# algbio/GraphChainer

Measured on AMD Instinct MI355X. Metric: reads_per_sec, higher is better.
Workload: dtype u64

## Files before the change

graphchainer_amd/csrc/batch/gc_batch_long.inc:

```
	void prepareWholeReadPass()
	{
		uint64_t nLongSeeds = 0;
		maxReadLen = 1;
		for (uint64_t r = 0; r < n; r++) maxReadLen = std::max<uint64_t>(maxReadLen, R->offsets[r + 1] - R->offsets[r]);
		firstAlnCap = (uint32_t)std::max<uint64_t>(32, maxReadLen / 512);
		if (sw.testLongMaxAlignments) firstAlnCap = *sw.testLongMaxAlignments;
		alnSlots = n * (uint64_t)firstAlnCap;
		if (P->long_pass && alnSlots >= 0xffffffffull) throw std::runtime_error("batch too large for the whole-read pass");
		if (P->long_pass) {
			if (deviceGlue) nLongSeeds = nSeedsTotal;
			else for (uint64_t r = 0; r < n; r++) { glue[r].longSeedBegin = nLongSeeds; nLongSeeds += glue[r].longSeeds.size(); }
			if (nLongSeeds >= 0xffffffffull) throw std::runtime_error("batch too large for the whole-read pass");
			LongSeed* hSeeds = st->hLongSeeds.reserve<LongSeed>(deviceGlue ? 0 : nLongSeeds);
			hJobs = st->hLongJobs.reserve<LongJob>(n);
			cellPoolPinned = sw.testLongCellsPerBase || P->capacity.long_cells_per_base > 0;
			uint64_t cellsPerBase = (uint64_t)std::max<int64_t>(2, capacityOr(sw.testLongCellsPerBase, P->capacity.long_cells_per_base, (int64_t)st->longCellsPerBase));
			if (sw.testLongForceFallback && !cellPoolPinned) cellsPerBase *= 3;
			cellBudget = cellBudgetFor(cellsPerBase);
			pool.run(n, [&](size_t r, size_t) {
				const ReadGlue& gl = glue[r];
				uint64_t at = gl.longSeedBegin;
				if (deviceGlue) at += gl.nSeedsR;
				else for (const gc::SeedRec& s : gl.longSeeds) {
					hSeeds[at++] = LongSeed { s.node, s.seqPos, s.goodness, s.clusterSize, s.offset, 0 };
				}
				LongJob& j = hJobs[r];
				j.maskOff = R->maskOff[r];
				j.maskWords = R->maskWords[r];
				j.alnCap = firstAlnCap;
				j.readOff = R->offsets[r];
				j.readLen = (uint32_t)(R->offsets[r + 1] - R->offsets[r]);
				j.seedBegin = (uint32_t)gl.longSeedBegin;
				j.seedEnd = (uint32_t)at;
				j.alnBegin = (uint32_t)(r * firstAlnCap);
				j.extendSeeds = j.seedEnd - j.seedBegin;
				if (P->seed_extend_density != -1) j.extendSeeds = (uint32_t)std::min<double>(4294967295.0, P->seed_extend_density * (double)j.readLen + 1);
				j.pad = 0;
			});
			lcfg.bandwidth = P->bandwidth;
			lcfg.rampBandwidth = P->ramp_bandwidth;
			lcfg.maxCells = P->max_cells_per_slice < 0 || P->max_cells_per_slice >= 0xffffffffll ? ~0u : (uint32_t)P->max_cells_per_slice;
			lcfg.maxSlices = (uint32_t)(maxReadLen / 64 + 3);
			lcfg.maxItems = (uint32_t)std::max<uint64_t>(8192, (maxReadLen / 64 + 3) * 24);
			lcfg.maxPending = 96;
			lcfg.forceGlobal = P->force_global != 0;
			lcfg.maxTrace = P->force_global || clip.on() ? (uint32_t)(2 * maxReadLen + 2 + 512) : (uint32_t)(maxReadLen + maxReadLen / 2 + 512);
			clip.apply(lcfg);
			lcfg.maxCols = (uint32_t)std::max<int64_t>(0, capacityOr(sw.testLongMaxCols, P->capacity.long_column_store, (int64_t)(3 * maxReadLen + 4096)));
			lcfg.maxItems = (uint32_t)std::max<int64_t>(64, capacityOr(sw.testLongMaxItems, P->capacity.long_max_items, lcfg.maxItems));
			if (sw.testLongRegCap) lcfg.regCap = *sw.testLongRegCap;
			waveWords = longWaveWordsPerLane(lcfg);
			if (!deviceGlue) dLongSeeds = st->longSeeds.reserve<LongSeed>(nLongSeeds);
			dLongJobs = st->longJobs.reserve<LongJob>(n);
			dLongAlns = st->longAlns.reserve<LongAln>(alnSlots);
			LongReadResult* dLongResults = st->longResults.reserve<LongReadResult>(n);
			dLongCells = st->longCells.reserve<LongCell>(cellBudget, true);
			if (!st->roundStream) {
				createStream(&st->roundStream);
				for (auto& e : st->roundEvents) HIP_CHECK(hipEventCreate(&e));
			}
			cursorWords = 32 + 8 * 16;
			dLongCursor = st->longCursor.reserve<unsigned long long>(cursorWords);
			hLongAlns = st->hLongAlns.reserve<LongAln>(alnSlots);
			hLongResults = st->hLongResults.reserve<LongReadResult>(n);
			hLongSmall = st->hLongSmall.reserve<unsigned long long>(cursorWords);
			ls = st->longStream;
			HIP_CHECK(hipMemsetAsync(dLongCursor, 0, cursorWords * sizeof(unsigned long long), ls));
			if (nLongSeeds && !deviceGlue) HIP_CHECK(hipMemcpyAsync(dLongSeeds, hSeeds, nLongSeeds * sizeof(LongSeed), hipMemcpyHostToDevice, ls));
			if (n) HIP_CHECK(hipMemcpyAsync(dLongJobs, hJobs, n * sizeof(LongJob), hipMemcpyHostToDevice, ls));
			syncStream(ls);
			dLongState = st->longState.reserve<LongState>(n);
			workCapacity = 8 * n + 64;
			dLongWork = st->longWork.reserve<LongWork>(workCapacity);
			dLongWorkResults = st->longWorkResults.reserve<LongWorkResult>(workCapacity);
			dCandSeed = st->longCandSeed.reserve<uint32_t>(2 * workCapacity);
			dWorkLen = st->longWorkLen.reserve<uint32_t>(workCapacity);
			dRetryList = st->longRetryList.reserve<uint32_t>(workCapacity);
			dOrder = st->longOrder.reserve<uint32_t>(workCapacity);
			roundTraceBudget = 0;
			for (uint64_t r = 0; r < n; r++) { uint64_t len = R->offsets[r + 1] - R->offsets[r]; roundTraceBudget += 4 * ((P->force_global || clip.on() ? 2 * len + 2 : len + len / 2) + 1024); }
			dRoundTrace = st->longRoundTrace.reserve<unsigned long long>(roundTraceBudget);
			uint64_t scratchBudget = P->capacity.long_scratch_bytes > 0 ? (uint64_t)P->capacity.long_scratch_bytes : (48ull << 30) / (uint64_t)longTokenCount(sw.longTokens, n, st->batchesDone, st->fragShare);
			if (sw.testLongScratchGb) scratchBudget = *sw.testLongScratchGb << 30;
			scratchLanes = std::min<uint64_t>(std::min<uint64_t>(workCapacity + 64, 2 * n + 128), std::max<uint64_t>(2048, std::min<uint64_t>(65536 + 64, scratchBudget / (waveWords * 8))));
			longScratchWords = scratchLanes * waveWords;
			shareLongScratch = sw.shareLongScratch();
			if (!shareLongScratch) dLongScratchOwn = st->longScratch.reserve<unsigned long long>(longScratchWords);
		}
	}

	uint64_t cellBudgetFor(uint64_t perBase) const { uint64_t b = 0; for (uint64_t r = 0; r < n; r++) b += perBase * (R->offsets[r + 1] - R->offsets[r]) + 1024; return b; }

	bool growLongCells()
	{
		bool overflowed = false;
		for (uint64_t r = 0; r < n && !overflowed; r++) overflowed = hLongResults[r].status == 4;
		if (!overflowed || cellPoolPinned) return false;
		HIP_CHECK(hipMemcpyAsync(hLongSmall, dLongCursor, sizeof(unsigned long long), hipMemcpyDeviceToHost, ls));
		syncStream(ls);
		const uint64_t asked = hLongSmall[0], bases = std::max<uint64_t>(1, R->totalBases);
		const uint64_t next = std::max<uint64_t>(st->longCellsPerBase + 2, (asked + asked / 2 + bases - 1) / bases);
		if (sw.debugTimes) fprintf(stderr, "[gc mem] the whole-read pass runs again: %.2f G merged-trace cells asked for, %.2f G reserved (%llu per read base), now %llu per base\n", asked / 1e9, cellBudget / 1e9, (unsigned long long)st->longCellsPerBase, (unsigned long long)next);
		if (next > 256 || cellBudgetFor(next) * sizeof(LongCell) > (64ull << 30)) return false;
		st->longCellsPerBase = next;
		cellBudget = cellBudgetFor(next);
		dLongCells = st->longCells.reserve<LongCell>(cellBudget, true);
		HIP_CHECK(hipMemsetAsync(dLongCursor, 0, cursorWords * sizeof(unsigned long long), ls));
		syncStream(ls);
		return true;
	}

	static constexpr uint32_t LONG_ALN_SLOTS_MAX = 1u << 16;
	bool growAlnSlots(const std::vector<uint32_t>& reads, bool keep)
	{
		uint64_t total = alnSlots;
		std::vector<std::pair<uint32_t, uint32_t>> grown;
		for (uint32_t r : reads) {
			const uint32_t cap = hJobs[r].alnCap, limit = std::min<uint32_t>(LONG_ALN_SLOTS_MAX, std::max<uint32_t>(1, hJobs[r].seedEnd - hJobs[r].seedBegin));
			if (cap >= limit) continue;
			const uint32_t next = (uint32_t)std::min<uint64_t>(limit, 4ull * cap);
			if (total + next >= 0xffffffffull) continue;
			grown.push_back({ r, next });
			total += next;
		}
		if (grown.empty()) return false;
		if (sw.debugTimes) fprintf(stderr, "[gc mem] %zu reads found more whole-read alignments than they had slots for and run again: %llu -> %llu slots in the batch\n", grown.size(), (unsigned long long)alnSlots, (unsigned long long)total);
		if (keep && total * sizeof(LongAln) > st->longAlns.bytes) {
			DeviceBuffer larger;
			LongAln* dLarger = larger.reserve<LongAln>(total);
			HIP_CHECK(hipMemcpyAsync(dLarger, dLongAlns, alnSlots * sizeof(LongAln), hipMemcpyDeviceToDevice, ls));
			syncStream(ls);
			std::swap(st->longAlns.ptr, larger.ptr); std::swap(st->longAlns.bytes, larger.bytes);
		}
		dLongAlns = st->longAlns.reserve<LongAln>(total);
		uint64_t at = alnSlots;
		for (const auto& g : grown) { hJobs[g.first].alnBegin = (uint32_t)at; hJobs[g.first].alnCap = g.second; at += g.second; }
		alnSlots = total;
		HIP_CHECK(hipMemcpyAsync(dLongJobs, hJobs, n * sizeof(LongJob), hipMemcpyHostToDevice, ls));
		syncStream(ls);
		return true;
	}

	bool growLongAlns()
	{
		std::vector<uint32_t> full;
		for (uint64_t r = 0; r < n; r++) if (hLongResults[r].status == 3) full.push_back((uint32_t)r);
		if (full.empty() || !growAlnSlots(full, false)) return false;
		HIP_CHECK(hipMemsetAsync(dLongCursor, 0, cursorWords * sizeof(unsigned long long), ls));
		syncStream(ls);
		return true;
	}

	void runLongRounds()
	{
		if (n == 0) return;
		unsigned long long* dLongScratch = nullptr;
		hipStream_t q = st->roundStream;
		hipEvent_t* ring = st->roundEvents;
		auto collect = [&](int slot) { float ms = 0; HIP_CHECK(hipEventElapsedTime(&ms, ring[2 * slot], ring[2 * slot + 1])); longExtendUs += (double)ms * 1000.0; };
		int timedRounds = 0;
		unsigned long long* cursor = dLongCursor + 32;
		volatile unsigned long long* hCursor = hLongSmall + 32;
		double dbgWaitUs = 0;
		const double dbgT0 = nowUs();
		launchLongInit(q, dLongJobs, (uint32_t)n, dLongState);
		uint32_t lastWork = 0xffffffffu;

		for (int round = 0; round < 4096; round++) {
			launchZeroWords(q, cursor, 4);
			uint32_t maxCand = 1;
			if (round > 0 && lastWork > 0) maxCand = (uint32_t)std::min<uint64_t>(8, std::max<uint64_t>(1, (2 * n) / lastWork));
			if (round > 0 && lastWork < 8192) maxCand = 8;
			if (round > 0 && lastWork > 0) maxCand = (uint32_t)std::min<uint64_t>(maxCand, std::max<uint64_t>(1, (8 * n) / lastWork));
			if (sw.testLongSpeculate) maxCand = *sw.testLongSpeculate;
			launchLongSelect(q, G->dev, dLongJobs, (uint32_t)n, dLongSeeds, R->totalBases, (uint32_t)P->min_cluster_size, (uint32_t)P->extra_heuristic, maxCand, dLongState, dLongAlns, dLongCells, dLongWork, dWorkLen, dCandSeed, cursor, workCapacity);
			launchLongOrder(q, dWorkLen, cursor, dOrder, (uint32_t)maxReadLen, sw.testLongOrder);
			launchPublish(q, cursor, (unsigned long long*)hCursor, 2);
			const double tWait0 = nowUs();
			syncStream(q);
			dbgWaitUs += nowUs() - tWait0;
			uint32_t nWorkItems = (uint32_t)hCursor[0];
			if (nWorkItems == 0) break;
			if (!dLongScratch) {
				longTokenTake();
				dLongScratch = shareLongScratch ? longScratchOfToken : dLongScratchOwn;
			}
			uint32_t team = longExtendTeamSize(nWorkItems, sw.testLongTeam.value_or(0));
			uint32_t blocks = std::min<uint32_t>((nWorkItems + team - 1) / team, (uint32_t)std::max<uint64_t>(1, (scratchLanes - 64) / team));
			if (sw.testLongMaxBlocks) blocks = std::min<uint32_t>(blocks, *sw.testLongMaxBlocks);
			if (timedRounds >= LONG_EVENT_RING) collect(timedRounds % LONG_EVENT_RING);
			hipEvent_t ev0 = ring[2 * (timedRounds % LONG_EVENT_RING)], ev1 = ring[2 * (timedRounds % LONG_EVENT_RING) + 1];
			HIP_CHECK(hipEventRecord(ev0, q));
			launchLongExtend(q, G->dev, G->devTables, R->devMasks, lcfg, dLongWork, dOrder, nWorkItems, dLongScratch, team, blocks,
				dRoundTrace, cursor + 1, roundTraceBudget, dLongWorkResults, dLongCursor + 8, cursor + 2, 0, nullptr, team == 1 ? dRetryList : nullptr, cursor + 3);
			if (team == 1) {
				if ((uint64_t)blocks * team < nWorkItems) launchZeroWords(q, cursor + 2, 1);
				uint32_t retryBlocks = std::min<uint32_t>(128, (uint32_t)std::max<uint64_t>(1, (scratchLanes - 64) / 2));
				launchLongExtend(q, G->dev, G->devTables, R->devMasks, lcfg, dLongWork, dRetryList, nWorkItems, dLongScratch, 2, retryBlocks,
					dRoundTrace, cursor + 1, roundTraceBudget, dLongWorkResults, dLongCursor + 8, cursor + 2, EXT_LDS_CAP, cursor + 3);
			}
			HIP_CHECK(hipEventRecord(ev1, q));
			launchLongMerge(q, G->dev, dLongJobs, (uint32_t)n, dLongSeeds, dCandSeed, dLongWorkResults, dRoundTrace, dLongState, dLongAlns, dLongCells, dLongCursor, cellBudget, (uint32_t)P->extra_heuristic);
			lastWork = nWorkItems;
			timedRounds++;
			longRounds++;
		}
		longTokenDrop();
		launchLongFinish(q, (uint32_t)n, dLongState, hLongResults);
		const double dbgT1 = nowUs();
		syncStream(q);
		if (sw.debugTimes) fprintf(stderr, "[gc times] whole-read rounds: %.1f ms in all, %.1f ms waiting for the rounds' work counts, %.1f ms in the last wait, %d rounds\n", (nowUs() - dbgT0) / 1e3, dbgWaitUs / 1e3, (nowUs() - dbgT1) / 1e3, timedRounds);
		for (int k = std::max(0, timedRounds - LONG_EVENT_RING); k < timedRounds; k++) collect(k % LONG_EVENT_RING);
	}

	uint64_t longFallback()
	{
		syncStream(ls);
		std::vector<uint32_t> redo;
		const bool forceAll = sw.testLongForceFallback;
		for (uint64_t r = 0; r < n; r++) if (hLongResults[r].status == 5 || hLongResults[r].status == 2 || forceAll) redo.push_back((uint32_t)r);
		if (!redo.empty()) {
			ExtendConfig fcfg = lcfg;
			fcfg.maxItems = 4 * lcfg.maxItems; fcfg.maxTrace = 2 * lcfg.maxTrace; fcfg.maxPending = 4 * lcfg.maxPending;
			uint64_t lslab = longSlabBytes(fcfg);
			std::vector<uint32_t> now = redo;
			for (int cellGrowths = 0; !now.empty(); ) {
				std::vector<LongJob> subJobs(now.size());
				for (size_t i = 0; i < now.size(); i++) subJobs[i] = hJobs[now[i]];
				uint64_t lanes = (now.size() + 63) / 64 * 64;
				LongJob* dSubJobs = st->longJobsFallback.reserve<LongJob>(now.size());
				LongReadResult* dSubResults = st->longResultsFallback.reserve<LongReadResult>(now.size());
				uint8_t* dSlab = st->longScratchFallback.reserve<uint8_t>(lanes * lslab);
				HIP_CHECK(hipMemcpyAsync(dSubJobs, subJobs.data(), now.size() * sizeof(LongJob), hipMemcpyHostToDevice, ls));
				launchLongPass(ls, G->dev, G->devTables, G->devIupac, fcfg, dSubJobs, (uint32_t)now.size(), dLongSeeds, R->devBases, R->totalBases, (uint32_t)P->min_cluster_size, (uint32_t)P->extra_heuristic,
					dSlab, lslab, dLongCells, dLongCursor, cellBudget, dLongAlns, dSubResults, dLongCursor + 8);
				std::vector<LongReadResult> subResults(now.size());
				HIP_CHECK(hipMemcpyAsync(subResults.data(), dSubResults, now.size() * sizeof(LongReadResult), hipMemcpyDeviceToHost, ls));
				HIP_CHECK(hipMemcpyAsync(hLongSmall, dLongCursor, sizeof(unsigned long long), hipMemcpyDeviceToHost, ls));
				syncStream(ls);
				std::vector<uint32_t> refused, full;
				for (size_t i = 0; i < now.size(); i++) {
					hLongResults[now[i]] = subResults[i];
					if (subResults[i].status == 4) refused.push_back(now[i]);
					if (subResults[i].status == 3) full.push_back(now[i]);
				}
				if (!full.empty() && !growAlnSlots(full, true)) full.clear();
				if (refused.empty() || cellPoolPinned || cellGrowths >= 3) { now.swap(full); continue; }
				const uint64_t used = std::min<uint64_t>(hLongSmall[0], cellBudget), next = std::min<uint64_t>(256, st->longCellsPerBase * 2);
				if (next == st->longCellsPerBase || cellBudgetFor(next) * sizeof(LongCell) > (64ull << 30)) { now.swap(full); continue; }
				cellGrowths++;
				if (sw.debugTimes) fprintf(stderr, "[gc mem] the plain-layout reruns of %zu reads found the merged-trace pool full: %llu -> %llu cells per read base, %.2f G cells kept\n", refused.size(), (unsigned long long)st->longCellsPerBase, (unsigned long long)next, used / 1e9);
				DeviceBuffer larger;
				LongCell* dLarger = larger.reserve<LongCell>(cellBudgetFor(next), true);
				if (used) HIP_CHECK(hipMemcpyAsync(dLarger, dLongCells, used * sizeof(LongCell), hipMemcpyDeviceToDevice, ls));
				const unsigned long long cursor = used;
				HIP_CHECK(hipMemcpyAsync(dLongCursor, &cursor, sizeof(cursor), hipMemcpyHostToDevice, ls));
				syncStream(ls);
				std::swap(st->longCells.ptr, larger.ptr); std::swap(st->longCells.bytes, larger.bytes);
				st->longCellsPerBase = next;
				cellBudget = cellBudgetFor(next);
				dLongCells = (LongCell*)st->longCells.ptr;
				now.swap(refused);
				now.insert(now.end(), full.begin(), full.end());
			}
		}
		hLongAlns = st->hLongAlns.reserve<LongAln>(alnSlots);
		if (n) HIP_CHECK(hipMemcpyAsync(hLongAlns, dLongAlns, alnSlots * sizeof(LongAln), hipMemcpyDeviceToHost, ls));
		HIP_CHECK(hipMemcpyAsync(hLongSmall, dLongCursor, 32 * sizeof(unsigned long long), hipMemcpyDeviceToHost, ls));
		syncStream(ls);
		return (uint64_t)redo.size();
	}

	void decideLongReads(const std::vector<uint32_t>& subset, int slot, hipStream_t q, const std::function<uint32_t(uint32_t)>& nAlnOf, bool usePool = true)
	{
		auto selectOne = [&](size_t i, size_t) {
			const uint32_t r = subset[i];
			ReadGlue& gl = glue[r];
			gl.longAlns.clear();
			gl.longSelected.clear();
			const uint32_t nAln = nAlnOf(r);
			for (uint32_t a = 0; a < nAln; a++) {
				gl.longAlns.push_back(hLongAlns[(uint64_t)hJobs[r].alnBegin + a]);
				std::sort(gl.longAlns.begin(), gl.longAlns.end(), [](const LongAln& l, const LongAln& rr) { return l.start < rr.start; });
			}
			std::vector<gc::SelectItem> items;
			for (const LongAln& al : gl.longAlns) items.push_back(gc::SelectItem { al.start, al.end, al.score });
			const size_t readLen = R->offsets[r + 1] - R->offsets[r];
			gl.longSelected = gc::selectAlignments(items, P->colinear_chaining ? (int)gc::SelectGreedyLength : (int)P->selection_method, hg.SizeInBP(), readLen, P->e_cutoff, evalueModel);
		};
		if (usePool) pool.run(subset.size(), selectOne); else for (size_t i = 0; i < subset.size(); i++) selectOne(i, 0);
		auto& D = st->edLong[slot];
		D.nPairs = 0;
		D.pairRead.clear();
		if (!P->edit_distances || !P->colinear_chaining || subset.empty()) return;
		const size_t m = subset.size();
		PathSeqJob* hJobsPS = D.hJobs.reserve<PathSeqJob>(m);
		EdPair* hPairs = D.hPairs.reserve<EdPair>(m);
		int64_t* hOut = D.hOut.reserve<int64_t>(m);
		uint64_t nLetters = 0;
		uint32_t nPairs = 0;
		for (size_t i = 0; i < m; i++) {
			const uint32_t r = subset[i];
			const ReadGlue& gl = glue[r];
			if (gl.longSelected.empty()) { hJobsPS[i] = PathSeqJob { 0, nLetters, 0, 0, 0, 0 }; continue; }
			const LongAln& al = gl.longAlns[gl.longSelected[0]];
			uint32_t len = (uint32_t)(R->offsets[r + 1] - R->offsets[r]);
			uint32_t cap = 2 * al.traceLen + 256;
			hJobsPS[i] = PathSeqJob { al.traceOff, nLetters, al.traceLen, cap, 0, 0 };
			hPairs[nPairs++] = EdPair { nLetters, 0, (uint32_t)i, r, al.score + al.start + (len - std::min(len, al.end)) + 8 };
			D.pairRead.push_back(r);
			nLetters += cap;
		}
		PathSeqJob* dJobsPS = D.jobs.reserve<PathSeqJob>(m);
		char* dLetters = D.letters.reserve<char>(nLetters);
		uint32_t* dLettersLen = D.lettersLen.reserve<uint32_t>(m);
		EdPair* dPairs = D.pairs.reserve<EdPair>(m);
		int64_t* dOut = D.out.reserve<int64_t>(m);
		HIP_CHECK(hipMemcpyAsync(dJobsPS, hJobsPS, m * sizeof(PathSeqJob), hipMemcpyHostToDevice, q));
		launchLongPathSeq(q, G->dev, dJobsPS, (uint32_t)m, dLongCells, dLetters, dLettersLen);
		auto readLenOf = [R = R](uint32_t r) { return (uint32_t)(R->offsets[r + 1] - R->offsets[r]); };
		launchEditDistances(D.run, q, hPairs, hOut, nPairs, dPairs, dOut, R->devEdReads, R->devBases, R->devEqMasks, dLetters, dLettersLen, readLenOf, sw.debugTimes, true);
		D.nPairs = nPairs;
		decisionPtr[slot] = DecisionPointers { hPairs, hOut, dPairs, dOut, dLetters, dLettersLen };
	}

	void finishLongDecision(int slot)
	{
		auto& D = st->edLong[slot];
		if (!D.nPairs) return;
		const DecisionPointers& p = decisionPtr[slot];
		finishEditDistances(D.run, st->longStream, p.hPairs, p.hOut, D.nPairs, p.dPairs, p.dOut, R->devEdReads, R->devBases, R->devEqMasks, p.dLetters, p.dLettersLen, sw.debugTimes);
		for (uint32_t i = 0; i < D.nPairs; i++) {
			ReadGlue& gl = glue[D.pairRead[i]];
			gl.longEditDistance = p.hOut[i];
			if (p.hOut[i] < -1) { gl.longEditDistance = -1; gl.capacityExceededLong = true; }
		}
		D.nPairs = 0;
	}

	void afterLongPass()
	{
		uint64_t rerun = longFallback();
		res->counters_long[7] = rerun;
		for (int i = 0; i < 6; i++) res->counters_long[i] = hLongSmall[8 + i];
#ifdef GC_STAMPS
		{
			static const char* names[11] = { "slice prologue", "pop+prev lookup", "tile columns", "item store", "edge pushes", "slice epilogue", "bt slice change", "bt item loads", "bt recompute", "bt corner", "bt walk" };
			double total = 0;
			for (int i = 0; i < 11; i++) total += (double)hLongSmall[16 + i];
			for (int i = 0; i < 11; i++) fprintf(stderr, "[gc stamps] %-16s %6.2f%%  %.3e lane-cycles\n", names[i], 100.0 * hLongSmall[16 + i] / (total > 0 ? total : 1), (double)hLongSmall[16 + i]);
		}
#endif
		if (sw.testFailLong) {
			const long idx = *sw.testFailLong;
			if (idx >= 0 && (uint64_t)idx < n) hLongResults[idx].status = 1;
// ... 78 lines not shown
```

graphchainer_amd/csrc/gc_batch.hip:

```cpp
#include "gc_runtime.hpp"

extern "C" {

struct ClipOptions {
	double cutoff = 0;
	double errorCost = 0;
	int32_t xDrop = 0;
	bool on() const { return cutoff != 0; }
	void apply(ExtendConfig& cfg) const { if (on()) { cfg.setClipErrorCost(errorCost); cfg.xDrop = xDrop; } }
};

struct BatchRun {
	const gc::Switches sw;
	const gc_graph* const G; const gc_seeder* const S; const gc_seeds* const H; gc_stream* const st; const gc_reads* const R; const gc_params* const P; const ClipOptions clip; gc_result* const res;
	const double tCall, cpuCall;
	double cpuJoined;
	const uint64_t n;
	const gc::AlignmentGraph& hg;
	WorkerPool& pool;
	std::vector<ReadGlue>& glue;
	const hipStream_t stream;
	int evIdx = 0;
	double tTotal = 0;
	bool deviceGlue = true;
	double tGlue = 0;
	uint64_t nSlots = 0, nFrags = 0, nSeedsTotal = 0, traceBudget = 0;
	uint32_t maxSlotsPerRead = 1, maxWindowSeeds = 0;
	Fragment* frags = nullptr; ReadChainJob* jobs = nullptr;
	FragSeed* readSeeds = nullptr; uint32_t* fragFirstSeed = nullptr;
	Fragment* dFrags = nullptr; uint32_t* dFragFirstSeed = nullptr; FragSeed* dReadSeeds = nullptr; ReadChainJob* dJobs = nullptr;
	LongSeed* dLongSeeds = nullptr;
	hipEvent_t glueCopied = nullptr;
	double tOrdered = 0;
	unsigned long long* hSmall = nullptr;
	unsigned long long* dCursors = nullptr;
	unsigned long long* dCounters = nullptr;
	uint32_t firstAlnCap = 0;
	uint64_t alnSlots = 0;
	LongAln* hLongAlns = nullptr;
	unsigned long long* hLongSmall = nullptr;
	LongReadResult* hLongResults = nullptr;
	LongCell* dLongCells = nullptr;
	uint64_t cellBudget = 0;
	unsigned long long* longScratchOfToken = nullptr;
	std::function<void()> longTokenTake, longTokenDrop;
	uint64_t longScratchWords = 0;
	bool shareLongScratch = false;
	double longExtendUs = 0; uint32_t longRounds = 0;
	const gc::EValueModel evalueModel { clip.on() ? clip.cutoff : 0.7 };
	struct DecisionPointers { EdPair* hPairs = nullptr; int64_t* hOut = nullptr; EdPair* dPairs = nullptr; int64_t* dOut = nullptr; char* dLetters = nullptr; uint32_t* dLettersLen = nullptr; } decisionPtr[2];
	LongJob* hJobs = nullptr;
	bool cellPoolPinned = 0;
	uint64_t waveWords = 0;
	LongJob* dLongJobs = nullptr;
	LongAln* dLongAlns = nullptr;
	uint32_t cursorWords = 0;
	uint64_t workCapacity = 0;
	uint64_t roundTraceBudget = 0;
	unsigned long long* dLongCursor = nullptr;
	LongState* dLongState = nullptr;
	LongWork* dLongWork = nullptr;
	LongWorkResult* dLongWorkResults = nullptr;
	uint32_t* dCandSeed = nullptr;
	uint32_t* dWorkLen = nullptr;
	uint32_t* dRetryList = nullptr;
	uint32_t* dOrder = nullptr;
	unsigned long long* dRoundTrace = nullptr;
	uint64_t scratchLanes = 0;
	hipStream_t ls = nullptr;
	ExtendConfig lcfg;
	unsigned long long* dLongScratchOwn = nullptr;
	uint64_t maxReadLen = 1;
	std::thread longThread;
	double passThreadCpuMs = 0;
	std::exception_ptr longError;
	double tLongWall0 = 0;
	double longWallBeginUs = 0.0;
	double longWallEndUs = 0.0;
	double tDev = 0;
	uint32_t nWork = 0;
	ExtResult* dResults = nullptr;
	PoolCell* dTrace = nullptr;
	AnchorRec* dAnchors = nullptr;
	uint32_t* dFragStatus = nullptr;
	uint32_t* dFragExtended = nullptr;
	uint64_t traceWorst = 0, pathWorst = 0;
	bool poolsSized = false;
	uint32_t nExtendPairs = 0, nAnchorPairs = 0;
	uint32_t poolReruns = 0;
	uint32_t* dReadTies = nullptr;
	uint64_t pathCapacity = 0;
	uint32_t* dPathPool = nullptr;
	uint32_t* dChainOut = nullptr;
	uint32_t* dChainLen = nullptr;
	unsigned long long* dChainScore = nullptr;
	uint32_t* dChainStatus = nullptr;
	bool deviceStitch = false;
	StitchInfo* stitchInfo = nullptr;
	uint32_t* hStitchNodes = nullptr;
	uint32_t* dStitchNodes = nullptr;
	uint64_t stitchDenseCap = 0;
	unsigned long long* hStitchCursor = nullptr;
	AnchorRec* anchors = nullptr;
	uint32_t* fragStatus = nullptr;
	uint32_t* fragExtended = nullptr;
	uint32_t* readTies = nullptr;
	uint32_t* chainOut = nullptr;
	uint32_t* chainLen = nullptr;
	unsigned long long* chainScore = nullptr;
	uint32_t* chainStatus = nullptr;
	uint32_t* pathPool = nullptr;
	bool deviceAnchors = false;
	uint4* hAnchorPerRead = nullptr;
	unsigned long long* hAnchorOff = nullptr;
	uint8_t* hAnchorDense = nullptr;
	uint64_t denseAnchors = 0, densePathWords = 0;
	std::vector<ExtResult> extResults;
	std::vector<PoolCell> tracePool;
	bool anchorTraces = false;
	bool stitchNodesPending = false;
	const PathSeqJob* chainLetterJobs = nullptr;
	const char* dChainLetters = nullptr;
	const uint32_t* dChainAltNodes = nullptr;
	const FastChainJob* fastChainJobs = nullptr;
	std::vector<uint32_t> zeroWords; std::vector<unsigned long long> zeroLongs; std::vector<uint4> zeroPerRead;
	double tJoined = 0;
	const LongCell* longCells = nullptr;

	BatchRun(const gc::Switches& sw, const gc_graph* G, const gc_seeder* S, const gc_seeds* H, gc_stream* st, const gc_reads* R, const gc_params* P, const ClipOptions& clip, gc_result* res, double tCall, double cpuCall)
		: sw(sw), G(G), S(S), H(H), st(st), R(R), P(P), clip(clip), res(res), tCall(tCall), cpuCall(cpuCall), cpuJoined(cpuCall), n(R->offsets.size() - 1), hg(G->host), pool(WorkerPool::batch()), glue(st->glue),
		  stream(st->stream) {}
	~BatchRun() { if (longThread.joinable()) longThread.join(); }
	BatchRun(const BatchRun&) = delete;
	BatchRun& operator=(const BatchRun&) = delete;

	void mark() { HIP_CHECK(hipEventRecord(st->ev[evIdx++], stream)); }
	double elapsedUs(int a, int b) { float ms = 0; HIP_CHECK(hipEventElapsedTime(&ms, st->ev[a], st->ev[b])); return (double)ms * 1000.0; }

	void run()
	{
		res->n_reads = n;
		tTotal = nowUs();
		const bool cpuStages = sw.debugTimes;
		double cpuAt = cpuStages ? threadCpuMs() : 0, cpuStage[10] = {}, poolStage[10] = {};
		uint64_t poolAt = pool.cpuUs.load();
		const double processAt = processCpuMs();
		auto stageDone = [&](int k) {
			if (!cpuStages) return;
			const double now = threadCpuMs(); const uint64_t poolNow = pool.cpuUs.load();
			cpuStage[k] += now - cpuAt; poolStage[k] += (poolNow - poolAt) / 1e3;
			cpuAt = now; poolAt = poolNow;
		};
		seeds(); stageDone(0);
		prepareWholeReadPass(); stageDone(1);
		startWholeReadPass(); stageDone(2);
		if (!P->colinear_chaining) { withoutChaining(); joinWholeReadPass(); stageDone(6); encodeOutput(); stageDone(8); assemble(); stageDone(9); st->batchesDone++; return; }
		fragmentPipeline(); stageDone(3);
		resultsBack(); stageDone(4);
		while (fragmentPoolsOverflowed()) { fragmentPipeline(); resultsBack(); stageDone(3); }
		res->counters[6] = poolReruns;
		compactAnchors(); stageDone(4);
		stitchAndChainDistances(); stageDone(5);
		joinWholeReadPass(); stageDone(6);
		chainedAlignments(); stageDone(7);
		encodeOutput(); stageDone(8);
		assemble(); stageDone(9);
		st->fragShare = (double)res->counters[4] / (double)std::max<uint64_t>(1, R->totalBases);
		st->batchesDone++;
		if (cpuStages)
			fprintf(stderr, "[gc cpu] main thread, ms of its own CPU: seeds %.1f, whole-read set-up %.1f + start %.1f, fragment pipeline %.1f, results back %.1f, stitching + chain distances %.1f, join %.1f, chained alignments %.1f, output %.1f, assembly %.1f; pass thread %.1f\n",
				cpuStage[0], cpuStage[1], cpuStage[2], cpuStage[3], cpuStage[4], cpuStage[5], cpuStage[6], cpuStage[7], cpuStage[8], cpuStage[9], passThreadCpuMs);
		if (cpuStages)
			fprintf(stderr, "[gc cpu] worker pool jobs, ms of CPU over all threads, by stage: %.1f %.1f %.1f %.1f %.1f %.1f %.1f %.1f %.1f %.1f; the process in all %.1f\n",
				poolStage[0], poolStage[1], poolStage[2], poolStage[3], poolStage[4], poolStage[5], poolStage[6], poolStage[7], poolStage[8], poolStage[9], processCpuMs() - processAt);
	}

#include "batch/gc_batch_seeds.inc"
#include "batch/gc_batch_long.inc"
#include "batch/gc_batch_fragments.inc"
#include "batch/gc_batch_results.inc"
#include "batch/gc_batch_output.inc"
};

static int resolveExt(const gc_params* P, const gc_params_ext* X, ClipOptions& clip)
{
	clip = ClipOptions();
	if (!X) return GC_OK;
	if (X->struct_size < sizeof(gc_params_ext)) return fail(GC_ERR_INVALID, "gc_params_ext::struct_size is smaller than the struct (was it initialised with gc_params_ext_default?)");
	if (X->struct_size > sizeof(gc_params_ext)) return fail(GC_ERR_INVALID, "gc_params_ext::struct_size is larger than this library knows: the caller's header is newer");
	if (X->x_drop < 0) return fail(GC_ERR_INVALID, "gc_params_ext::x_drop must be 0 (off) or >= 1 (src/AlignerMain.cpp:316-322)");
	const double c = X->precise_clipping;
	if (std::isnan(c) || (c != 0 && !(c >= 0.001 && c <= 0.999))) return fail(GC_ERR_INVALID, "gc_params_ext::precise_clipping must be 0 (off) or in [0.001, 0.999] (src/AlignerMain.cpp:300-315)");
	if (X->x_drop > 0 && P->force_global != 0) return fail(GC_ERR_INVALID, "gc_params_ext::x_drop cannot be combined with force_global (getSlices asserts, src/GraphAlignerBitvectorBanded.h:504)");
	clip.cutoff = c;
	clip.xDrop = X->x_drop;
	if (clip.xDrop > 0 && clip.cutoff == 0) clip.cutoff = 0.66;
	if (clip.on()) clip.errorCost = clip.cutoff / (1.0 - clip.cutoff) + 1.0;
	return GC_OK;
}

static int alignBatch(const gc::Switches& sw, const gc_graph* G, const gc_seeder* S, const gc_seeds* H, gc_stream* st, const gc_reads* R, const gc_params* P, const ClipOptions& clip, gc_result** out)
{
	if (P->split_len < 16 || P->split_len > 64 || P->split_gap < 1) return fail(GC_ERR_INVALID, "split_len must be in [16,64] (one 64-row slice per fragment extension) and split_gap >= 1");
	if (P->ramp_bandwidth < 0 || (P->ramp_bandwidth != 0 && P->ramp_bandwidth <= P->bandwidth)) return fail(GC_ERR_INVALID, "ramp_bandwidth must be 0 (off) or larger than bandwidth (src/AlignerMain.cpp:380-383)");
	if (P->max_cells_per_slice < -1) return fail(GC_ERR_INVALID, "max_cells_per_slice must be -1 (unlimited) or >= 0");
	if (P->force_global != 0 && P->force_global != 1) return fail(GC_ERR_INVALID, "force_global must be 0 or 1");
	if (P->colinear_chaining != 0 && P->colinear_chaining != 1) return fail(GC_ERR_INVALID, "colinear_chaining must be 0 or 1");
	if (P->colinear_chaining == 0 && !P->long_pass) return fail(GC_ERR_INVALID, "colinear_chaining == 0 needs long_pass: without chaining the whole-read pass is all there is");
	if (P->extra_heuristic != 0 && P->extra_heuristic != 1) return fail(GC_ERR_INVALID, "extra_heuristic must be 0 or 1");
	if (P->selection_method < 0 || P->selection_method > GC_SELECT_ALL) return fail(GC_ERR_INVALID, "selection_method must be one of GC_SELECT_* (0..7)");
	if (P->fast_mode != 0 && P->fast_mode != 1) return fail(GC_ERR_INVALID, "fast_mode must be 0 or 1");
	if (std::isnan(P->seed_extend_density) || (P->seed_extend_density <= 0 && P->seed_extend_density != -1)) return fail(GC_ERR_INVALID, "seed_extend_density must be -1 (all seeds) or > 0 (src/AlignerMain.cpp:405)");
	if (P->seed_extend_density != -1 && P->colinear_chaining == 1) return fail(GC_ERR_INVALID, "seed_extend_density must be -1 with colinear_chaining == 1: chaining tries all seeds (src/AlignerMain.cpp:204,449-453)");
	{
		const gc_capacities& c = P->capacity;
		if (c.reserved[0] || c.reserved[1] || c.reserved[2]) return fail(GC_ERR_INVALID, "gc_params::capacity.reserved must be 0 (was the struct initialised with gc_params_default?)");
		const int64_t v[] = { c.ext_max_items, c.ext_max_pending, c.ext_max_trace, c.long_max_items, c.long_cells_per_base, c.long_scratch_bytes, c.stitch_set_max, c.stitch_bfs_cap };
		for (int64_t x : v) if (x < 0 || x > (1ll << 40)) return fail(GC_ERR_INVALID, "gc_params::capacity: a size is negative or absurd (0 = automatic)");
		if (c.ext_max_items > (1ll << 24) || c.ext_max_pending > (1ll << 24) || c.ext_max_trace > (1ll << 24)) return fail(GC_ERR_INVALID, "gc_params::capacity.ext_*: at most 2^24 (the retry launch reserves 16x)");
// ... 56 lines not shown
```

graphchainer_amd/csrc/gc_runtime.hpp:

```cpp
#pragma once
#include "../../include/graphchainer_amd.h"
#include "hip/gc_kernels.hpp"
#include "host/gc_graph.hpp"
#include "host/gc_hashorder.hpp"
#include "host/gc_glue.hpp"
#include "host/gc_output.hpp"
#include "host/gc_index_cache.hpp"
#include "host/gc_correctness.hpp"
#include "host/gc_selection.hpp"
#include "host/gc_switches.hpp"
#include "host/gc_mxm_build.hpp"
#include "hip/gc_mxm_core.hpp"
#include <hip/hip_runtime.h>
#include <algorithm>
#include <atomic>
#include <condition_variable>
#include <functional>
#include <mutex>
#include <chrono>
#include <cmath>
#include <cstdlib>
#include <cstring>
#include <stdexcept>
#include <string>
// ... 375 lines not shown
		for (const Block& b : mine) { if (pinned) (void)hipHostFree(b.ptr); else (void)hipFree(b.ptr); }
	}
};
inline BlockCache& g_readDeviceBlocks = *new BlockCache(false);
inline BlockCache& g_readPinnedBlocks = *new BlockCache(true);
inline BlockCache& g_deflateDeviceBlocks = *new BlockCache(false, (size_t)4 << 30);
inline BlockCache& g_deflatePinnedBlocks = *new BlockCache(true, (size_t)4 << 30);

inline hipStream_t threadStream(int device)
{
	static thread_local struct ThreadStream { hipStream_t q = nullptr; int device = -1; ~ThreadStream() { if (q) (void)hipStreamDestroy(q); } } ts;
	if (!ts.q || ts.device != device) { if (ts.q) (void)hipStreamDestroy(ts.q); ts.q = nullptr; HIP_CHECK(hipStreamCreateWithFlags(&ts.q, hipStreamNonBlocking)); ts.device = device; }
	return ts.q;
}

struct gc_reads {
	void* deviceBlock = nullptr; size_t deviceBlockBytes = 0; int device = 0;
	std::vector<uint64_t> offsets;
	uint64_t totalBases = 0;
	std::vector<uint8_t> invalid;
	char* devBases = nullptr;
	uint64_t* devOffsets = nullptr;
	uint64_t* devMasks = nullptr;
	std::vector<uint64_t> maskOff;
	std::vector<uint32_t> maskWords;
	const uint64_t* devMaskOff = nullptr; const uint32_t* devMaskWords = nullptr;
	uint64_t* devEqMasks = nullptr;
	EdRead* devEdReads = nullptr;
	uint32_t* devChunkRead = nullptr;
	uint64_t* devPacked = nullptr;
	uint64_t* devInvalid = nullptr;
	uint8_t* devReadInvalid = nullptr;
	~gc_reads() { g_readDeviceBlocks.put(deviceBlock, deviceBlockBytes, device); }
};

struct gc_seeds {
	int device = 0;
	uint64_t nHits = 0;
	std::vector<uint64_t> readOffsets;
	uint32_t* devReadHitOff = nullptr;
	SeedHitArrays dev {};
	void* block = nullptr;
	SeedHit* devHits = nullptr;
	double kernelMs = 0;
	~gc_seeds() { if (block) (void)hipFree(block); }
};

struct gc_mxm_index {
	const gc_graph* graph = nullptr;
	int device = 0;
	std::vector<uint32_t> nodeStart;
	std::vector<int32_t> nodeId;
	MxmIndexView dev {};
	uint64_t deviceBytes = 0;
	double buildSeconds = 0;
	std::vector<void*> allocations;
	~gc_mxm_index() { for (void* p : allocations) (void)hipFree(p); }
};

struct StitchedPath { std::vector<uint32_t> nodes; uint32_t firstOffset = 0, lastOffset = 0; uint64_t cells = 0; };

struct ReadGlue {
	std::vector<gc::SeedRec> seeds;
	std::vector<gc::SeedRec> longSeeds;
	std::vector<gc::FragmentWindow> windows;
	std::vector<LongAln> longAlns;
	uint64_t longBegin = 0, longTraceBegin = 0, longSeedBegin = 0;
	bool failed = false;
	bool longFailed = false;
	bool capacityExceeded = false;
	bool capacityExceededLong = false;
	uint64_t slotBegin = 0, fragBegin = 0;
	uint32_t nSeedsR = 0, nWindows = 0;
	uint64_t nAnchors = 0, nPath = 0, nTrace = 0, anchorBegin = 0, pathBegin = 0, traceBegin = 0, seedBegin = 0, chainBegin = 0;
	StitchedPath stitched;
	bool stitchedOnDevice = false;
	uint64_t stitchedBegin = 0;
	std::vector<uint32_t> longSelected;
	uint64_t longSelectedBegin = 0;
	int64_t longEditDistance = -1, chainEditDistance = -1;
	std::vector<int32_t> chainTraceNode; std::vector<uint32_t> chainTraceOffset, chainTraceSeqPos; std::vector<uint8_t> chainTraceSwitch;
	uint32_t chainAlnStart = 0, chainAlnEnd = 0;
	bool hasChainAlignment = false, chainWins = false;
	uint64_t chainTraceBegin = 0;
	void reset()
	{
		seeds.clear(); longSeeds.clear(); windows.clear(); longAlns.clear(); longSelected.clear();
		stitched.nodes.clear(); stitched.firstOffset = stitched.lastOffset = 0; stitched.cells = 0;
		longBegin = longTraceBegin = longSeedBegin = 0;
		failed = longFailed = capacityExceeded = capacityExceededLong = false;
		slotBegin = fragBegin = 0;
		nSeedsR = nWindows = 0;
		nAnchors = nPath = nTrace = anchorBegin = pathBegin = traceBegin = seedBegin = chainBegin = 0;
		stitchedBegin = longSelectedBegin = 0;
		longEditDistance = chainEditDistance = -1;
		chainTraceNode.clear(); chainTraceOffset.clear(); chainTraceSeqPos.clear(); chainTraceSwitch.clear();
		chainAlnStart = chainAlnEnd = 0;
		hasChainAlignment = chainWins = false;
		chainTraceBegin = 0;
	}
};

struct EditDistanceRun {
	hipStream_t streams[8] {};
	uint32_t begin[9] {};
	std::vector<uint32_t> lens;
	hipEvent_t ready = nullptr;
	std::vector<uint32_t> perm;
	std::vector<int64_t> grouped;
	~EditDistanceRun() { for (auto& q : streams) if (q) (void)hipStreamDestroy(q); if (ready) (void)hipEventDestroy(ready); }
};

inline constexpr int LONG_EVENT_RING = 8;
struct gc_stream {
	std::vector<ReadGlue> glue;
	int device = 0;
	hipStream_t stream = nullptr;
	hipEvent_t ev[12] {};
	hipEvent_t fragEv[16] {};
	DeviceBuffer tmp, matches, readMatchOff, readMatchCount, cursors, readSeeds, fragFirstSeed, longRetryList, extLists, fragItems, fragRetryList, fragClaims, pendingFrags, fragNext, roundCounts, work, results, scratch, scratchRetry, tracePool, frags, fragSeeds, anchors, fragStatus, fragExtended, readTies, pathPool, jobs, chainOut, chainLen, chainScore, chainStatus, chainScratch, counters;
	PinnedBuffer hFragDeclined, hMatches, hReadSeeds, hFragFirstSeed, hFrags, hJobs, hAnchors, hFragStatus, hFragExtended, hReadTies, hChainOut, hChainLen, hChainScore, hChainStatus, hPathPool, hSmall;
	hipStream_t longStream = nullptr;
	hipEvent_t longEv[2] {};
	DeviceBuffer edPathNodes, edJobs, edLetters, edLettersLen, edPairs, edOut;
	PinnedBuffer hEdPathNodes, hEdJobs, hEdPairs, hEdOut;
	DeviceBuffer outJobs, outRecs, outOffsets, outMapSizes, outPathText, outCigarText, outVgBytes, outTotals;
	PinnedBuffer hOutJobs, hOutRecs, hOutOffsets, hOutPathText, hOutCigarText, hOutVgBytes, hOutTotals;
	DeviceBuffer stitchSlotOf, stitchRegions, stitchNodes, stitchInfo, stitchCursor, stitchSpill;
	DeviceBuffer anchorPerRead, anchorSlotEnd, anchorOff, anchorDense;
	PinnedBuffer hAnchorPerRead, hAnchorOff, hAnchorDense;
	PinnedBuffer hStitchNodes, hStitchInfo, hStitchCursor;
	EditDistanceRun edChainRun;
	DeviceBuffer edPathJobs, edPathOps, edPathLen, edPathScratch;
	PinnedBuffer hEdPathJobs, hEdPathOps, hEdPathLen;
	DeviceBuffer fastJobs, fastScore, fastTraceJobs, fastTrace, fastWritten;
	PinnedBuffer hFastJobs, hFastScore, hFastTraceJobs, hFastTrace, hFastWritten;
	struct LongDecision {
		PinnedBuffer hJobs, hPairs, hOut;
		DeviceBuffer jobs, letters, lettersLen, pairs, out;
		EditDistanceRun run;
		std::vector<uint32_t> pairRead;
		uint32_t nPairs = 0;
	} edLong[2];
	uint64_t longCellsPerBase = 4;
	double fragShare = 0;
	uint64_t batchesDone = 0;
	bool poolsRerun = false;
	double traceCellsPerSlot = 0, pathWordsPerSlot = 0;
	hipStream_t roundStream = nullptr;
	hipEvent_t roundEvents[2 * LONG_EVENT_RING] {};
	DeviceBuffer longSeeds, longJobs, longAlns, longResults, longScratch, longCells, longCursor, longJobsFallback, longResultsFallback, longScratchFallback;
	DeviceBuffer gluePerRead, glueCursors, glueOut, glueSeedCap, glueSeedOff, glueWinCapOff, glueU32[8], glueSort, gluePos, glueWin;
	PinnedBuffer hGlueOut, hGlueWinCapOff, hGlueSmall;
	DeviceBuffer longState, longWork, longWorkResults, longRoundTrace, longCandSeed, longWorkLen, longOrder;
	PinnedBuffer hLongSeeds, hLongJobs, hLongAlns, hLongResults, hLongSmall, hLongCells;
	template <typename F> void forEachDeviceBuffer(F f) const
	{
		f("tmp", tmp.bytes); f("matches", matches.bytes); f("readMatchOff", readMatchOff.bytes); f("readMatchCount", readMatchCount.bytes); f("cursors", cursors.bytes); f("readSeeds", readSeeds.bytes);
		f("fragFirstSeed", fragFirstSeed.bytes); f("longRetryList", longRetryList.bytes); f("extLists", extLists.bytes); f("pendingFrags", pendingFrags.bytes); f("fragNext", fragNext.bytes);
		f("roundCounts", roundCounts.bytes); f("fragItems", fragItems.bytes); f("fragRetryList", fragRetryList.bytes); f("work", work.bytes); f("results", results.bytes); f("scratch", scratch.bytes); f("scratchRetry", scratchRetry.bytes); f("tracePool", tracePool.bytes);
		f("frags", frags.bytes); f("fragSeeds", fragSeeds.bytes); f("anchors", anchors.bytes); f("fragStatus", fragStatus.bytes); f("fragExtended", fragExtended.bytes); f("readTies", readTies.bytes);
		f("pathPool", pathPool.bytes); f("jobs", jobs.bytes); f("chainOut", chainOut.bytes); f("chainLen", chainLen.bytes); f("chainScore", chainScore.bytes); f("chainStatus", chainStatus.bytes);
		f("chainScratch", chainScratch.bytes); f("counters", counters.bytes); f("edPathNodes", edPathNodes.bytes); f("edJobs", edJobs.bytes); f("edLetters", edLetters.bytes);
		f("edLettersLen", edLettersLen.bytes); f("edPairs", edPairs.bytes); f("edOut", edOut.bytes); f("outJobs", outJobs.bytes); f("outRecs", outRecs.bytes); f("outOffsets", outOffsets.bytes);
		f("outMapSizes", outMapSizes.bytes); f("outPathText", outPathText.bytes); f("outCigarText", outCigarText.bytes); f("outVgBytes", outVgBytes.bytes); f("outTotals", outTotals.bytes);
		f("stitchSlotOf", stitchSlotOf.bytes); f("stitchRegions", stitchRegions.bytes); f("stitchNodes", stitchNodes.bytes); f("stitchInfo", stitchInfo.bytes); f("stitchCursor", stitchCursor.bytes); f("stitchSpill", stitchSpill.bytes);
		f("anchorPerRead", anchorPerRead.bytes); f("anchorSlotEnd", anchorSlotEnd.bytes); f("anchorOff", anchorOff.bytes); f("anchorDense", anchorDense.bytes);
		f("edPathJobs", edPathJobs.bytes); f("edPathOps", edPathOps.bytes); f("edPathLen", edPathLen.bytes); f("edPathScratch", edPathScratch.bytes); f("longSeeds", longSeeds.bytes);
		f("fastJobs", fastJobs.bytes); f("fastScore", fastScore.bytes); f("fastTraceJobs", fastTraceJobs.bytes); f("fastTrace", fastTrace.bytes); f("fastWritten", fastWritten.bytes);
		f("longJobs", longJobs.bytes); f("longAlns", longAlns.bytes); f("longResults", longResults.bytes); f("longScratch", longScratch.bytes); f("longCells", longCells.bytes);
		f("longCursor", longCursor.bytes); f("longJobsFallback", longJobsFallback.bytes); f("longResultsFallback", longResultsFallback.bytes); f("longScratchFallback", longScratchFallback.bytes);
		f("gluePerRead", gluePerRead.bytes); f("glueCursors", glueCursors.bytes); f("glueOut", glueOut.bytes); f("glueSeedCap", glueSeedCap.bytes); f("glueSeedOff", glueSeedOff.bytes);
		f("glueWinCapOff", glueWinCapOff.bytes); f("glueU32[0]", glueU32[0].bytes); f("glueU32[1]", glueU32[1].bytes); f("glueU32[2]", glueU32[2].bytes); f("glueU32[3]", glueU32[3].bytes);
		f("glueU32[4]", glueU32[4].bytes); f("glueU32[5]", glueU32[5].bytes); f("glueU32[6]", glueU32[6].bytes); f("glueU32[7]", glueU32[7].bytes); f("glueSort", glueSort.bytes);
		f("gluePos", gluePos.bytes); f("glueWin", glueWin.bytes); f("longState", longState.bytes); f("longWork", longWork.bytes); f("longWorkResults", longWorkResults.bytes);
		f("longRoundTrace", longRoundTrace.bytes); f("longCandSeed", longCandSeed.bytes); f("longWorkLen", longWorkLen.bytes); f("longOrder", longOrder.bytes);
		for (int k = 0; k < 2; k++) { f("edLong.letters", edLong[k].letters.bytes); f("edLong.jobs+pairs+out", edLong[k].jobs.bytes + edLong[k].lettersLen.bytes + edLong[k].pairs.bytes + edLong[k].out.bytes); }
	}
	~gc_stream()
	{
		for (auto& e : ev) if (e) (void)hipEventDestroy(e);
		for (auto& e : fragEv) if (e) (void)hipEventDestroy(e);
		for (auto& e : longEv) if (e) (void)hipEventDestroy(e);
		for (auto& e : roundEvents) if (e) (void)hipEventDestroy(e);
		if (roundStream) (void)hipStreamDestroy(roundStream);
		if (stream) (void)hipStreamDestroy(stream);
		if (longStream) (void)hipStreamDestroy(longStream);
	}
};

inline void buildIupacTable(uint8_t* t)
{
	memset(t, 0, 256);
	auto set = [&](const char* chars, uint8_t m) { for (const char* c = chars; *c; c++) t[(uint8_t)*c] = m; };
	set("Aa", 1); set("Cc", 2); set("Gg", 4); set("TtUu", 8);
	set("Rr", 1 | 4); set("Yy", 2 | 8); set("Kk", 4 | 8); set("Mm", 1 | 2); set("Ss", 2 | 4); set("Ww", 1 | 8);
	set("Bb", 2 | 4 | 8); set("Dd", 1 | 4 | 8); set("Hh", 1 | 2 | 8); set("Vv", 1 | 2 | 4); set("Nn", 15);
}

inline void uploadGraph(gc_graph* G)
{
	const gc::AlignmentGraph& h = G->host;
	size_t n = h.NodeSize();
	if (n >= 0xfffffff0ull) throw std::runtime_error("graph too large for 32-bit node ids");
	DGraph& d = G->dev;
	d.nNodes = (uint32_t)n;
	d.firstAmbiguous = (uint32_t)h.firstAmbiguous;
	int maxId = -1;
	{
		std::vector<uint8_t> nodeLength(n);
		std::vector<uint32_t> nodeOffset(n);
		std::vector<int32_t> nodeIDs(n);
		for (size_t i = 0; i < n; i++) {
			nodeLength[i] = (uint8_t)h.nodeLength[i];
			nodeOffset[i] = (uint32_t)h.nodeOffset[i];
			nodeIDs[i] = h.nodeIDs[i];
			maxId = std::max(maxId, h.nodeIDs[i]);
		}
		d.nodeLength = G->up(nodeLength);
		d.nodeOffset = G->up(nodeOffset);
		d.nodeIDs = G->up(nodeIDs);
	}
	{
		std::vector<uint32_t> componentNumber(n), componentMap(n), topoId(n);
		for (size_t i = 0; i < n; i++) {
			componentNumber[i] = (uint32_t)h.componentNumber[i];
			componentMap[i] = (uint32_t)h.component_map[i];
			topoId[i] = (uint32_t)h.topo_ids[h.component_map[i]][h.component_idx[i]];
		}
		d.componentNumber = G->up(componentNumber);
		d.componentMap = G->up(componentMap);
		d.topoId = G->up(topoId);
	}
	{
		std::vector<uint64_t> nodeSeq(2 * h.firstAmbiguous);
		for (size_t i = 0; i < h.firstAmbiguous; i++) { nodeSeq[2 * i] = h.nodeSequences[i][0]; nodeSeq[2 * i + 1] = h.nodeSequences[i][1]; }
		d.nodeSeq = G->up(nodeSeq);
	}
	{
		std::vector<uint64_t> ambSeq(4 * (n - h.firstAmbiguous));
		for (size_t i = h.firstAmbiguous; i < n; i++) {
			const gc::AmbiguousSeq& s = h.ambiguousNodeSequences[i - h.firstAmbiguous];
			size_t at = 4 * (i - h.firstAmbiguous);
			ambSeq[at] = s.A; ambSeq[at + 1] = s.C; ambSeq[at + 2] = s.G; ambSeq[at + 3] = s.T;
		}
		d.ambSeq = G->up(ambSeq);
	}
	auto csr = [&](const std::vector<std::vector<size_t>>& adj, const uint32_t*& devOff, const uint32_t*& devFlat) {
		std::vector<uint32_t> off(n + 1, 0), flat;
		for (size_t i = 0; i < n; i++) off[i + 1] = off[i] + (uint32_t)adj[i].size();
		flat.reserve(off[n]);
		for (size_t i = 0; i < n; i++) for (size_t v : adj[i]) flat.push_back((uint32_t)v);
		devOff = G->up(off); devFlat = G->up(flat);
	};
	csr(h.inNeighbors, d.inOff, d.inAdj);
	csr(h.outNeighbors, d.outOff, d.outAdj);
	const size_t nB = (size_t)maxId + 1;
	{
		std::vector<uint32_t> origSize(nB, 0), lookupOff(nB + 1, 0), lookup;
		lookup.reserve(n);
		for (size_t id = 0; id < nB; id++) {
			const bool known = h.nodeLookup.contains((int)id);
			lookupOff[id + 1] = lookupOff[id] + (known ? (uint32_t)h.nodeLookup.at((int)id).size() : 0u);
			if (known) {
				origSize[id] = (uint32_t)h.originalNodeSize.at((int)id);
				for (size_t s : h.nodeLookup.at((int)id)) lookup.push_back((uint32_t)s);
			}
		}
		for (size_t id = 0; id < nB; id++)
			for (uint32_t k = lookupOff[id]; k < lookupOff[id + 1]; k++)
				if (h.nodeOffset[lookup[k]] != 64ull * (k - lookupOff[id])) throw std::runtime_error("split nodes are not 64-aligned chunks of their original node");
		d.origSize = G->up(origSize); d.lookupOff = G->up(lookupOff); d.lookup = G->up(lookup);
		G->hOrigSize = std::move(origSize); G->hLookupOff = std::move(lookupOff); G->hLookup = std::move(lookup);
	}
	{
		std::vector<uint32_t> pathsOff(n + 1, 0), pathsFlat, pathsPos, backOff(n + 1, 0), mpcWidth(h.mpc.size());
		for (size_t c = 0; c < h.mpc.size(); c++) { mpcWidth[c] = (uint32_t)h.mpc[c].size(); G->maxMpcWidth = std::max(G->maxMpcWidth, mpcWidth[c]); }
		size_t nPaths = 0, nBack = 0;
		for (size_t i = 0; i < n; i++) { const size_t c = h.component_map[i], x = h.component_idx[i]; nPaths += h.paths[c][x].size(); nBack += h.backwards[c][x].size(); }
		if (nPaths >= 0xffffffffull || nBack >= 0xffffffffull) throw std::runtime_error("MPC index too large for 32-bit offsets");
		pathsFlat.reserve(nPaths);
		for (size_t i = 0; i < n; i++) {
			size_t c = h.component_map[i], x = h.component_idx[i];
			for (size_t k : h.paths[c][x]) pathsFlat.push_back((uint32_t)k);
			pathsOff[i + 1] = (uint32_t)pathsFlat.size();
			G->maxPathsPerNode = std::max(G->maxPathsPerNode, pathsOff[i + 1] - pathsOff[i]);
			backOff[i + 1] = backOff[i] + (uint32_t)h.backwards[c][x].size();
			G->maxBackPerNode = std::max(G->maxBackPerNode, backOff[i + 1] - backOff[i]);
		}
		pathsPos.assign(pathsFlat.size(), 0);
		for (size_t c = 0; c < h.mpc.size(); c++)
			for (size_t k = 0; k < h.mpc[c].size(); k++)
				for (size_t j = 0; j < h.mpc[c][k].size(); j++) {
					size_t node = h.mpc[c][k][j];
					for (uint32_t e = pathsOff[node]; e < pathsOff[node + 1]; e++) if (pathsFlat[e] == k) pathsPos[e] = (uint32_t)j;
				}
		auto posOf = [&](uint32_t node, uint32_t k) -> uint32_t {
			for (uint32_t e = pathsOff[node]; e < pathsOff[node + 1]; e++) if (pathsFlat[e] == k) return pathsPos[e];
			throw std::runtime_error("MPC index: node not on path");
		};
		uint32_t *dBackNode = nullptr, *dBackPath = nullptr, *dBackPos = nullptr;
		for (uint32_t** p : { &dBackNode, &dBackPath, &dBackPos }) { HIP_CHECK(hipMalloc((void**)p, std::max<size_t>(nBack, 1) * sizeof(uint32_t))); G->allocations.push_back(*p); }
		const size_t sliceLinks = gc::Switches::fromEnvironment().testUploadSlice;
		std::vector<uint32_t> backNode, backPath, backPos;
		for (size_t first = 0; first < n;) {
			size_t last = first;
			while (last < n && (last == first || (size_t)(backOff[last + 1] - backOff[first]) <= sliceLinks)) last++;
			backNode.clear(); backPath.clear(); backPos.clear();
			for (size_t i = first; i < last; i++) {
				const size_t c = h.component_map[i], x = h.component_idx[i];
				for (const auto& b : h.backwards[c][x]) {
					const uint32_t node = (uint32_t)h.component_ids[c][b.first], path = (uint32_t)b.second;
					backNode.push_back(node); backPath.push_back(path); backPos.push_back(posOf(node, path));
				}
			}
			if (backNode.size() != (size_t)(backOff[last] - backOff[first])) throw std::runtime_error("MPC index: backward links counted differently");
			if (!backNode.empty()) {
				HIP_CHECK(hipMemcpy(dBackNode + backOff[first], backNode.data(), backNode.size() * sizeof(uint32_t), hipMemcpyHostToDevice));
				HIP_CHECK(hipMemcpy(dBackPath + backOff[first], backPath.data(), backPath.size() * sizeof(uint32_t), hipMemcpyHostToDevice));
				HIP_CHECK(hipMemcpy(dBackPos + backOff[first], backPos.data(), backPos.size() * sizeof(uint32_t), hipMemcpyHostToDevice));
			}
			first = last;
		}
		d.pathsOff = G->up(pathsOff); d.paths = G->up(pathsFlat); d.pathsPos = G->up(pathsPos);
		d.backOff = G->up(backOff); d.backNode = dBackNode; d.backPath = dBackPath; d.backPos = dBackPos;
		d.mpcWidth = G->up(mpcWidth);
	}
	{
		std::vector<uint32_t> chainNumber(n);
// ... 259 lines not shown
```

graphchainer_amd/csrc/hip/gc_kernels.hip:

```cpp
#include "gc_kernels.hpp"
#include "gc_device_wave.hpp"
#include <cstdlib>

namespace gcdev {


__device__ __forceinline__ int baseCode(uint8_t c)
{
	switch (c) {
		case 'a': case 'A': return 0;
		case 'c': case 'C': return 1;
		case 'g': case 'G': return 2;
		case 't': case 'T': return 3;
	}
	return -1;
}

__device__ __forceinline__ uint32_t hashKmer(uint64_t kmer)
{
	kmer *= 0x9E3779B97F4A7C15ull;
	return (uint32_t)(kmer >> 32);
}

__device__ __forceinline__ uint32_t filterBit(uint64_t kmer, uint32_t shift) { return (uint32_t)((kmer * 0xD6E8FEB86659FD93ull) >> shift); }

__device__ __forceinline__ uint32_t lookupKmer(const SeedIndex& idx, uint64_t kmer)
{
	const uint32_t fb = filterBit(kmer, idx.filterShift);
	if (!((idx.filter[fb >> 5] >> (fb & 31)) & 1u)) return 0xffffffffu;
	uint32_t h = hashKmer(kmer) & idx.tableMask;
	while (true) {
		uint64_t slot = idx.table[h];
		if (slot == ~0ull) return 0xffffffffu;
		if ((uint32_t)(slot >> 32) == (uint32_t)kmer && (!idx.wideKmers || idx.wideKmers[(uint32_t)slot] == kmer)) return (uint32_t)slot;
		h = (h + 1) & idx.tableMask;
	}
}

__global__ void __launch_bounds__(256) k_seed_probe(SeedIndex idx, const char* __restrict__ bases, const uint64_t* __restrict__ readOff, const uint32_t* __restrict__ chunkRead, const uint64_t* __restrict__ packed, const uint64_t* __restrict__ invalid, uint32_t nReads, uint64_t totalBases, uint32_t* __restrict__ tmp)
{
	const int k = idx.k;
	const int realWindow = idx.w - idx.k + 1;
	const uint64_t mask = ~(~0ull << (2 * k));
	for (uint64_t p = (uint64_t)blockIdx.x * blockDim.x + threadIdx.x; p < totalBases; p += (uint64_t)gridDim.x * blockDim.x) {
		uint32_t lo = chunkRead[p >> 6];
		while (lo + 1 < nReads && readOff[lo + 1] <= p) lo++;
		const char* seq = bases + readOff[lo];
		const int pos = (int)(p - readOff[lo]);
		uint32_t found = 0;
		if (pos >= k - 1) {
			const uint64_t w = p >> 5;
			const uint64_t lo64 = packed[w], hi64 = w ? packed[w - 1] : 0ull;
			const uint32_t sh = 2u * (31u - (uint32_t)(p & 31));
			const uint64_t kmer = (sh ? ((lo64 >> sh) | (hi64 << (64 - sh))) : lo64) & mask;
			const uint64_t iw = p >> 6;
			const uint64_t ilo = invalid[iw], ihi = iw ? invalid[iw - 1] : 0ull;
			const uint32_t ish = 63u - (uint32_t)(p & 63);
			const uint64_t window = ish ? ((ilo >> ish) | (ihi << (64 - ish))) : ilo;
			const bool valid = (window & ((1ull << k) - 1)) == 0;
			if (valid) {
				int streakStart = pos;
				int c0 = baseCode((uint8_t)seq[pos]);
				bool homopolymer = (kmer == (uint64_t)c0 * (mask / 3));
				if (homopolymer) {
					while (streakStart - k >= 0 && baseCode((uint8_t)seq[streakStart - k]) == c0) streakStart--;
				}
				bool emit = ((pos - streakStart) % realWindow) == 0;
				if (emit) {
					uint32_t key = lookupKmer(idx, kmer);
					if (key != 0xffffffffu) {
						uint32_t count = (uint32_t)(idx.startPos[key + 1] - idx.startPos[key]);
						if (count < idx.maxCount) found = key + 1;
					}
				}
			}
		}
		tmp[p] = found;
	}
}

__global__ void __launch_bounds__(64) k_seed_compact(const uint64_t* __restrict__ readOff, uint32_t nReads, const uint32_t* __restrict__ tmp,
	uint64_t* __restrict__ matchCursor, uint32_t* __restrict__ readMatchOff, uint32_t* __restrict__ readMatchCount, uint2* __restrict__ matches, uint64_t matchCapacity)
{
	const int lane = threadIdx.x;
	for (uint32_t r = blockIdx.x; r < nReads; r += gridDim.x) {
		const int len = (int)(readOff[r + 1] - readOff[r]);
		const uint32_t* mine = tmp + readOff[r];
		uint32_t total = 0;
		for (int base = 0; base < len; base += 64) {
			int pos = base + lane;
			total += (uint32_t)__popcll(__ballot(pos < len && mine[pos] != 0));
		}
		uint64_t outBase = 0;
		if (lane == 0) outBase = atomicAdd((unsigned long long*)matchCursor, (unsigned long long)total);
		outBase = __shfl(outBase, 0);
		if (lane == 0) { readMatchOff[r] = (uint32_t)outBase; readMatchCount[r] = total; }
		if (outBase + total > matchCapacity) continue;
		uint32_t written = 0;
		for (int base = 0; base < len; base += 64) {
			int pos = base + lane;
			uint32_t found = pos < len ? mine[pos] : 0;
			unsigned long long ballot = __ballot(found != 0);
			if (found) {
				uint32_t rank = (uint32_t)__popcll(ballot & ((1ull << lane) - 1));
				matches[outBase + written + rank] = make_uint2((uint32_t)pos, found - 1);
			}
			written += (uint32_t)__popcll(ballot);
		}
	}
}


__device__ __forceinline__ LaneScratch laneScratch(uint8_t* slab, const ExtendConfig& cfg)
{
	LaneScratch sc;
	uint8_t* p = slab;
	sc.slices = (SliceInfo*)p;   p += sizeof(SliceInfo) * cfg.maxSlices;
	sc.items = (NodeItem*)p;     p += sizeof(NodeItem) * cfg.maxItems;
	sc.pending = (Pending*)p;    p += sizeof(Pending) * cfg.maxPending;
	sc.columns = (WCol*)p;       p += sizeof(WCol) * 64;
	sc.colMask = 63; sc.colStride = 1;
	sc.trace = (TraceCell*)p;    p += sizeof(TraceCell) * cfg.maxTrace;
	sc.itemNodes = (uint32_t*)p;
	return sc;
}

#ifndef GC_EXTEND_RING
#define GC_EXTEND_RING 8
#endif
#define GC_EXTEND_SLAB_PARAMS DGraph g, const CorrectnessTables* __restrict__ ct, const uint8_t* __restrict__ iupac, ExtendConfig cfg, 	const ExtItem* __restrict__ work, uint32_t nWork, const char* __restrict__ bases, ExtResult* __restrict__ results, 	uint8_t* __restrict__ scratch, uint64_t slabBytes, PoolCell* __restrict__ tracePool, unsigned long long* __restrict__ traceCursor, uint64_t traceCapacity, 	unsigned long long* __restrict__ counters, uint32_t retryStatus, ExtSelection sel
template <bool BAND, bool CLIP = false>
__device__ __forceinline__ void extendSlabBody(GC_EXTEND_SLAB_PARAMS)
{
#if defined(GC_EXTEND_PRIO) && GC_EXTEND_PRIO
	__builtin_amdgcn_s_setprio(GC_EXTEND_PRIO);
#endif
	const uint32_t tid = blockIdx.x * blockDim.x + threadIdx.x;
	const uint32_t stride = gridDim.x * blockDim.x;
	LaneScratch sc = laneScratch(scratch + (uint64_t)tid * slabBytes, cfg);
#if GC_EXTEND_RING
	__shared__ WCol columnRing[GC_EXTEND_RING * 64];
	sc.columns = columnRing + threadIdx.x;
	sc.colMask = GC_EXTEND_RING - 1; sc.colStride = 64;
#endif
	ExtCounters cnt {};
	const uint32_t nSelected = sel.mode == 0 ? nWork : sel.mode == 1 ? 2 * sel.nFrags : (uint32_t)*sel.listCount;
	for (uint32_t at = tid; at < nSelected; at += stride) {
		const uint32_t w = sel.mode == 0 ? at : sel.mode == 1 ? 2 * sel.frags[at >> 1].seedBegin + (at & 1u) : sel.list[at];
		if (retryStatus != 0 && results[w].status != retryStatus) continue;
		ExtItem it = work[w];
		uint32_t nTrace = 0;
		int32_t score = 0;
		uint32_t status = extendSeed<BAND, CLIP>(g, *ct, iupac, cfg, sc, bases + it.seqOff, (int)it.seqLen, it.node, it.offset, nTrace, score, cnt);
		ExtResult res;
// ... 400 lines not shown
					const uint32_t a = a0 + lane;
					const bool have = a < nA;
					const uint32_t slot = have ? (uint32_t)A.aBucket[a] : 0xffffffffu;
					const uint32_t cnt = have ? (uint32_t)A.entBegin[a + 1] - (uint32_t)A.entBegin[a] : 0u;
					uint32_t before = 0, anchorsBefore = 0;
					for (int l = 0; l < 63; l++) { const uint32_t s = __shfl(slot, l), c = __shfl(cnt, l); if (l < lane && s == slot) { before += c; anchorsBefore++; } }
					if (have) {
						A.entByCompBegin[a] = (uint16_t)(bStart[slot] + bFilled[slot] + before);
						A.anchorByBucket[bAnchorStart[slot] + bAnchorsPlaced[slot] + anchorsBefore] = (uint16_t)a;
					}
					__syncthreads();
					if (have) { if (cnt) atomicAdd(&bFilled[slot], cnt); atomicAdd(&bAnchorsPlaced[slot], 1u); }
					__syncthreads();
				}
				for (uint32_t b = lane; b < CHAIN_BUCKETS; b += 64) bFilled[b] = 0;
				__syncthreads();
				for (uint32_t a = lane; a < nA; a += 64)
					for (uint32_t e = A.entBegin[a], to = A.entByCompBegin[a]; e < A.entBegin[a + 1]; e++, to++) A.entByComp[to] = A.ent[e];
				__syncthreads();
			}
		}
		uint32_t w0 = 0;
		uint2 win = (uint32_t)lane < nB ? A.back[lane] : make_uint2(0, 0);
		auto relax = [&](uint32_t j, uint32_t fj, const ChainEntry* entries, uint32_t scanBegin, uint32_t scanEnd, bool sameComponent) {
			const uint32_t b0 = A.backBegin[j], b1 = A.backBegin[j + 1];
			if ((b0 >= w0 && b1 <= w0 + 64) || (b1 - b0 <= 64 && (w0 = b0, win = b0 + lane < nB ? A.back[b0 + lane] : make_uint2(0, 0), true))) {
				const uint32_t t = w0 + lane;
				if (t >= b0 && t < b1) atomicMax(&A.thr[win.x], (int32_t)win.y);
			} else {
				for (uint32_t t = b0 + lane; t < b1; t += 64) { const uint2 it = A.back[t]; atomicMax(&A.thr[it.x], (int32_t)it.y); }
			}
			__syncthreads();
			const uint32_t compV = A.aComp[j];
			const long long xj = (long long)fj * splitGap, yj = xj + splitLen - 1;
			unsigned long long best = 0;
			for (uint32_t e = scanBegin + lane; e < scanEnd; e += 64) {
				const ChainEntry en = entries[e];
				const uint32_t i = en.anchor;
				if ((!sameComponent && A.aComp[i] != compV) || (int32_t)en.pos > A.thr[en.k]) continue;
				const long long yi = (long long)A.aFrag[i] * splitGap + splitLen - 1;
				const long long ci = unpackScore(A.C[i]);
				unsigned long long cand;
				if (yi <= xj - 1) cand = packScore((long long)splitLen + ci, i);
				else cand = packScore(yj - yi + ci, i);
				best = cand > best ? cand : best;
			}
			for (int d = 32; d > 0; d >>= 1) {
				unsigned long long o = __shfl_xor(best, d);
				best = o > best ? o : best;
			}
			if (lane == 0 && best > A.C[j]) A.C[j] = best;
			__syncthreads();
			if (b1 <= w0 + 64 && b0 >= w0) {
				const uint32_t t = w0 + lane;
				if (t >= b0 && t < b1) A.thr[win.x] = -1;
			} else {
				for (uint32_t t = b0 + lane; t < b1; t += 64) A.thr[A.back[t].x] = -1;
			}
		};
		unsigned long long top = 0;
		auto topOver = [&](uint32_t count, auto anchorAt) {
			unsigned long long mine = 0;
			for (uint32_t q = lane; q < count; q += 64) {
				const uint32_t a = anchorAt(q);
				const unsigned long long key = ((unsigned long long)unpackScore(A.C[a]) << 32) | ((unsigned long long)(65535u - (uint32_t)A.aComp[a]) << 16) | a;
				mine = key > mine ? key : mine;
			}
			for (int d = 32; d > 0; d >>= 1) { const unsigned long long o = __shfl_xor(mine, d); mine = o > mine ? o : mine; }
			top = mine > top ? mine : top;
		};
		if (LDS == 0 && bucketed) {
			while (true) {
				uint32_t pick = 0;
				for (uint32_t k = 0; k < CHAIN_BUCKETS / 64; k++) { const uint32_t slot = lane * (CHAIN_BUCKETS / 64) + k, c = bAnchors[slot]; const uint32_t key = c ? (c << 10) | (1023u - slot) : 0u; pick = key > pick ? key : pick; }
				for (int d = 32; d > 0; d >>= 1) { const uint32_t o = __shfl_xor(pick, d); pick = o > pick ? o : pick; }
				const uint32_t count = pick >> 10, slot = 1023u - (pick & 1023u);
				if (count == 0) break;
				if ((unsigned long long)count * (unsigned long long)splitLen < (top >> 32)) break;
				__syncthreads();
				if (lane == 0) bAnchors[slot] = 0;
				const uint16_t* list = A.anchorByBucket + bAnchorStart[slot];
				const uint32_t entFirst = bStart[slot];
				uint32_t filled = 0, groupFrom = 0, fragPrev = 0;
				for (uint32_t q = 0; q < count; q++) {
					const uint32_t j = list[q];
					const uint32_t fj = A.aFrag[j];
					if (q > 0 && fj != fragPrev) {
						uint32_t add = 0;
						for (uint32_t x = groupFrom + lane; x < q; x += 64) { const uint32_t a = list[x]; add += (uint32_t)A.entBegin[a + 1] - (uint32_t)A.entBegin[a]; }
						for (int d = 32; d > 0; d >>= 1) add += __shfl_xor(add, d);
						filled += add;
						groupFrom = q;
						__syncthreads();
					}
					fragPrev = fj;
					if (filled == 0) continue;
					relax(j, fj, A.entByComp, entFirst, entFirst + filled, true);
				}
				__syncthreads();
				topOver(count, [&](uint32_t q) { return (uint32_t)list[q]; });
			}
		} else {
			uint32_t g0 = 0, entPrefix = 0;
			for (uint32_t j = 0; j < nA; j++) {
				const uint32_t fj = A.aFrag[j];
				if (j > 0 && fj != A.aFrag[j - 1]) { g0 = j; entPrefix = A.entBegin[j]; __syncthreads(); }
				if (g0 == 0) continue;
				relax(j, fj, A.ent, 0, entPrefix, false);
			}
			__syncthreads();
			topOver(nA, [&](uint32_t q) { return q; });
		}
		if (lane == 0) {
			uint32_t status = 0;
			const long long best = nA ? (long long)(top >> 32) : 0;
			uint32_t bestLen = 0;
			uint32_t* out = chainOut + job.chainBegin;
			if (nA) {
				uint32_t n = 0;
				for (long long i = (long long)(top & 0xffffu); i != -1; i = unpackAnchor(A.C[i])) {
					if (n >= job.nSlots) { status = 1; break; }
					out[n++] = (uint32_t)i;
				}
				for (uint32_t i = 0; i < n / 2; i++) { uint32_t t = out[i]; out[i] = out[n - 1 - i]; out[n - 1 - i] = t; }
				bestLen = n;
			}
			chainLen[r] = bestLen;
			chainScore[r] = (unsigned long long)best;
			chainStatus[r] = status;
		}
		__syncthreads();
	}
}


struct LongSlab { LaneScratch sc; TraceCell* traceB; };

__device__ __forceinline__ LongSlab longSlab(uint8_t* slab, const ExtendConfig& cfg)
{
	LongSlab ls;
	ls.sc = laneScratch(slab, cfg);
	ls.traceB = (TraceCell*)(ls.sc.itemNodes + cfg.maxItems);
	return ls;
}

__device__ __forceinline__ void twinOf(const DGraph& g, uint32_t node, uint32_t offset, uint32_t& twinNode, uint32_t& twinOffset)
{
	const int32_t id = g.nodeIDs[node];
	const uint32_t rev = g.origSize[id] - 1 - (g.nodeOffset[node] + offset);
	twinNode = g.lookup[g.lookupOff[id ^ 1] + rev / 64];
	twinOffset = rev - g.nodeOffset[twinNode];
}

__device__ inline int onTrace(const LongCell* trace, uint32_t n, uint32_t seqPos, int32_t compareNode, uint32_t nodeOffset)
{
	if (!(trace[n - 1].seqPos > trace[0].seqPos)) return 2;
	if (trace[n - 1].seqPos < seqPos || trace[0].seqPos > seqPos) return 0;
	uint32_t lo = 0, hi = n;
	while (lo < hi) {
		uint32_t mid = (lo + hi) / 2;
		if (trace[mid].seqPos < seqPos) lo = mid + 1; else hi = mid;
	}
	for (uint32_t i = lo; i < n && trace[i].seqPos == seqPos; i++)
		if (trace[i].node == compareNode && trace[i].offset == nodeOffset) return 1;
	return 0;
}

__device__ __forceinline__ bool seedCutEndToEnd(uint32_t goodness, uint32_t e2eScore, uint32_t extraHeuristic)
{
	return goodness < e2eScore || (extraHeuristic && goodness == e2eScore);
}
__device__ __forceinline__ bool seedCutBudget(uint32_t goodness, uint32_t extended, uint32_t extendSeeds, uint32_t worstExtended, uint32_t extraHeuristic)
{
	return extended >= extendSeeds && (extraHeuristic || goodness < worstExtended);
}

__device__ inline uint32_t endToEndScore(LongAln* mine, uint32_t nAln, uint32_t readLen, uint32_t current)
{
	bool anyAtZero = false;
	for (uint32_t a = 0; a < nAln; a++) if (mine[a].start == 0) anyAtZero = true;
	if (!anyAtZero) return current;
	uint32_t contiguousEnd = 0, minGoodness = 0xffffffffu;
	bool first = true;
	for (uint32_t visited = 0; visited < nAln; visited++) {
		uint32_t best = 0xffffffffu;
		for (uint32_t a = 0; a < nAln; a++) {
			if (mine[a].pad) continue;
			if (best == 0xffffffffu || mine[a].start < mine[best].start) best = a;
		}
		mine[best].pad = 1;
		if (first) { contiguousEnd = mine[best].end; minGoodness = mine[best].goodness; first = false; continue; }
		if (mine[best].start <= contiguousEnd) {
			minGoodness = mine[best].goodness < minGoodness ? mine[best].goodness : minGoodness;
			contiguousEnd = mine[best].end > contiguousEnd ? mine[best].end : contiguousEnd;
		}
	}
	for (uint32_t a = 0; a < nAln; a++) mine[a].pad = 0;
	return contiguousEnd == readLen ? minGoodness : current;
}

template <bool BAND, bool CLIP = false>
__global__ void __launch_bounds__(64) k_long_pass(DGraph g, const CorrectnessTables* __restrict__ ct, const uint8_t* __restrict__ iupac, ExtendConfig cfg,
	const LongJob* __restrict__ jobs, uint32_t nReads, const LongSeed* __restrict__ seeds, const char* __restrict__ bases, uint64_t rcBase,
	uint32_t minClusterSize, uint32_t extraHeuristic, uint8_t* __restrict__ scratch, uint64_t slabBytes,
	LongCell* __restrict__ cellPool, unsigned long long* __restrict__ cellCursor, uint64_t cellCapacity,
	LongAln* __restrict__ alns, LongReadResult* __restrict__ results, unsigned long long* __restrict__ counters)
{
	const uint32_t tid = blockIdx.x * blockDim.x + threadIdx.x;
	const uint32_t stride = gridDim.x * blockDim.x;
	LongSlab ls = longSlab(scratch + (uint64_t)tid * slabBytes, cfg);
	ExtCounters cnt {};
	for (uint32_t r = tid; r < nReads; r += stride) {
		LongJob job = jobs[r];
		LongAln* mine = alns + job.alnBegin;
		uint32_t nAln = 0, extended = 0, status = 0, ties = 0;
		uint32_t e2eScore = 0;
		uint32_t worstExtended = 0;
		const int L = (int)job.readLen;
		uint32_t si = job.seedBegin;
		while (true) {
			bool have = false;
			LongSeed sd {};
			for (; status == 0 && si < job.seedEnd && !have; si++) {
				sd = seeds[si];
				if (seedCutEndToEnd(sd.goodness, e2eScore, extraHeuristic)) { si = job.seedEnd; break; }
				if (seedCutBudget(sd.goodness, extended, job.extendSeeds, worstExtended, extraHeuristic)) { si = job.seedEnd; break; }
				if (sd.clusterSize < minClusterSize) continue;
				bool skip = false;
				for (uint32_t a = 0; a < nAln; a++)
					if (mine[a].start <= sd.seqPos && mine[a].end >= sd.seqPos && (extraHeuristic || mine[a].goodness > sd.goodness)) { skip = true; break; }
				if (skip) continue;
				int32_t compareNode = g.nodeIDs[sd.node];
				uint32_t compareOffset = g.nodeOffset[sd.node] + sd.offset;
				for (uint32_t a = 0; a < nAln && !skip; a++) {
					int on = onTrace(cellPool + mine[a].traceOff, mine[a].traceLen, sd.seqPos, compareNode, compareOffset);
					if (on == 2) { status = 1; break; }
					if (on == 1) skip = true;
				}
				if (skip || status) continue;
				have = true;
			}
			if (!__any(have)) break;
			if (!have) continue;
			worstExtended = sd.goodness;
			extended++;
			const int p = (int)sd.seqPos;
			uint32_t nB = 0, nF = 0;
			int32_t scoreB = 0, scoreF = 0;
			uint32_t stB = EXT_FAILED, stF = EXT_FAILED;
			if (p > 0) {
				uint32_t twinNode, twinOffset;
				twinOf(g, sd.node, sd.offset, twinNode, twinOffset);
				stB = extendSeed<BAND, CLIP>(g, *ct, iupac, cfg, ls.sc, bases + rcBase + job.readOff + (uint64_t)(L - p), p, twinNode, twinOffset, nB, scoreB, cnt);
				ties += cnt.flattenTie;
				if (stB == EXT_OK) for (uint32_t i = 0; i < nB; i++) ls.traceB[i] = ls.sc.trace[i];
			}
			if (p < L - 1 && stB != EXT_ASSERT) { stF = extendSeed<BAND, CLIP>(g, *ct, iupac, cfg, ls.sc, bases + job.readOff + (uint64_t)(p + 1), L - 1 - p, sd.node, sd.offset, nF, scoreF, cnt); ties += cnt.flattenTie; }
			if (stB == EXT_ASSERT || stF == EXT_ASSERT) { status = 1; break; }
			if (stB == EXT_OVERFLOW || stF == EXT_OVERFLOW) { status = 2; break; }
			bool hasB = stB == EXT_OK, hasF = stF == EXT_OK;
			if (!hasB && !hasF) continue;
			if (nAln >= job.alnCap) { status = 3; break; }
			uint32_t useB = hasB ? (hasF ? nB - 1 : nB) : 0;
			uint32_t total = useB + (hasF ? nF : 0);
			unsigned long long base = atomicAdd(cellCursor, (unsigned long long)total);
			if (base + total > cellCapacity) { status = 4; break; }
			LongCell* outCells = cellPool + base;
			for (uint32_t i = 0; i < useB; i++) {
				const TraceCell& c = ls.traceB[i];
				uint32_t off = c.offsetAndSwitch & 255u;
				int32_t id = g.nodeIDs[c.node];
				uint32_t orig = g.nodeOffset[c.node] + off;
				LongCell oc;
				oc.node = id ^ 1;
				oc.offset = g.origSize[id] - 1 - orig;
				oc.seqPos = (uint32_t)(p - 1 - c.seqPos);
				oc.nodeSwitch = (i + 1 < nB) ? ((ls.traceB[i + 1].offsetAndSwitch >> 8) & 1u) : 0u;
				outCells[i] = oc;
			}
			if (hasF) for (uint32_t i = 0; i < nF; i++) {
				const TraceCell& c = ls.sc.trace[nF - 1 - i];
				LongCell oc;
				oc.node = g.nodeIDs[c.node];
				oc.offset = g.nodeOffset[c.node] + (c.offsetAndSwitch & 255u);
				oc.seqPos = (uint32_t)(p + 1 + c.seqPos);
				oc.nodeSwitch = (c.offsetAndSwitch >> 8) & 1u;
				outCells[useB + i] = oc;
			}
			LongAln al;
			al.start = outCells[0].seqPos;
			al.end = outCells[total - 1].seqPos + 1;
			al.score = (uint32_t)((hasB ? scoreB : 0) + (hasF ? scoreF : 0));
			al.goodness = sd.goodness;
			al.traceOff = base;
			al.traceLen = total;
			al.pad = 0;
			mine[nAln++] = al;
			e2eScore = endToEndScore(mine, nAln, (uint32_t)L, e2eScore);
		}
		LongReadResult rr;
		rr.nAlignments = status == 1 ? 0 : nAln;
		rr.seedsExtended = extended;
		rr.status = status;
		rr.pad = ties;
		results[r] = rr;
	}
	if (cnt.extensions) {
		atomicAdd(&counters[0], cnt.dpTiles);
		atomicAdd(&counters[1], cnt.recomputeTiles);
		atomicAdd(&counters[2], cnt.columnSteps);
		atomicAdd(&counters[3], cnt.traceItems);
		atomicAdd(&counters[4], cnt.extensions);
		atomicAdd(&counters[5], cnt.backtraceTiles);
	}
}


__global__ void __launch_bounds__(256) k_long_init(const LongJob* __restrict__ jobs, uint32_t nReads, LongState* __restrict__ state)
{
	GC_RAISE_PRIO();
	uint32_t r = blockIdx.x * blockDim.x + threadIdx.x;
	if (r >= nReads) return;
	LongState st { jobs[r].seedBegin, 0, 0, 0, 0, 0, 0, 0, 0, 0 };
	state[r] = st;
}

__device__ inline int seedSkipped(const DGraph& g, const LongSeed& sd, const LongAln* mine, uint32_t aFrom, uint32_t aTo, const LongCell* cellPool, uint32_t extraHeuristic)
{
	for (uint32_t a = aFrom; a < aTo; a++)
		if (mine[a].start <= sd.seqPos && mine[a].end >= sd.seqPos && (extraHeuristic || mine[a].goodness > sd.goodness)) return 1;
	int32_t compareNode = g.nodeIDs[sd.node];
	uint32_t compareOffset = g.nodeOffset[sd.node] + sd.offset;
	for (uint32_t a = aFrom; a < aTo; a++) {
		int on = onTrace(cellPool + mine[a].traceOff, mine[a].traceLen, sd.seqPos, compareNode, compareOffset);
		if (on == 2) return 2;
		if (on == 1) return 1;
	}
	return 0;
}

#define LONG_MAX_CANDIDATES 8
__device__ __forceinline__ void longSelectRead(const DGraph& g, const uint32_t r, const uint32_t lane, const LongJob* __restrict__ jobs, const LongSeed* __restrict__ seeds, uint32_t minClusterSize,
	uint32_t extraHeuristic, uint32_t maxCandidates, LongState* __restrict__ state, const LongAln* __restrict__ alns, const LongCell* __restrict__ cellPool, LongWork* __restrict__ work, uint32_t* __restrict__ workLen, uint32_t* __restrict__ candSeed,
	unsigned long long* __restrict__ workCount, uint64_t workCapacity)
{
	LongState st = state[r];
	st.candCount = 0;
	if (st.status != 0) { if (lane == 0) state[r] = st; return; }
	LongJob job = jobs[r];
	const LongAln* mine = alns + job.alnBegin;
	uint32_t cand[LONG_MAX_CANDIDATES];
	uint32_t nCand = 0;
	uint32_t si = st.si;
	bool stop = false;
	while (!stop && si < job.seedEnd) {
		const uint32_t idx = si + lane;
		const bool valid = idx < job.seedEnd;
		LongSeed sd = seeds[valid ? idx : si];
		const bool cut = valid && (seedCutEndToEnd(sd.goodness, st.e2eScore, extraHeuristic)
			|| seedCutBudget(sd.goodness, st.extended, job.extendSeeds, st.worstExtended, extraHeuristic));
		const bool small = sd.clusterSize < minClusterSize;
		int sk = 1;
		if (valid && !cut && !small) sk = seedSkipped(g, sd, mine, 0, st.nAln, cellPool, extraHeuristic);
		const uint64_t cutMask = __ballot(cut), assertMask = __ballot(sk == 2), candMask = __ballot(sk == 0);
		const uint32_t nValid = job.seedEnd - si < 64 ? job.seedEnd - si : 64;
		const uint32_t firstCut = cutMask ? (uint32_t)__ffsll((unsigned long long)cutMask) - 1 : 64;
		const uint32_t limit = firstCut < nValid ? firstCut : nValid;
		uint32_t b = 0;
		for (; b < limit; b++) {
			if ((assertMask >> b) & 1) { st.status = 1; stop = true; break; }
			if ((candMask >> b) & 1) {
				if (nCand > 0 && st.extended + nCand >= job.extendSeeds) { stop = true; break; }
				for (uint32_t k = 0; k < LONG_MAX_CANDIDATES; k++) if (k == nCand) cand[k] = si + b;
				nCand++;
				if (nCand == maxCandidates) { b++; stop = true; break; }
			}
		}
		si += b;
		if (!stop && firstCut < nValid) { si = job.seedEnd; stop = true; }
	}
	st.si = si;
	if (nCand > 0) {
		unsigned long long at = 0;
		if (lane == 0) at = atomicAdd(workCount, 2ull * nCand);
		at = __shfl(at, 0);
		if (at + 2ull * nCand > workCapacity) { st.status = 2; nCand = 0; }
		st.candBegin = (uint32_t)(at / 2);
		st.candCount = nCand;
		uint32_t myCand = 0;
		for (uint32_t k = 0; k < LONG_MAX_CANDIDATES; k++) if (k == lane) myCand = cand[k];
		if (lane < nCand) {
			const uint32_t c = lane;
			LongSeed sd = seeds[myCand];
			const uint32_t L = job.readLen, p = sd.seqPos;
			uint32_t twinNode, twinOffset;
			twinOf(g, sd.node, sd.offset, twinNode, twinOffset);
			work[at + 2 * c] = LongWork { job.maskOff + 4ull * job.maskWords, job.maskWords, L - p, p, twinNode, twinOffset, r };
			work[at + 2 * c + 1] = LongWork { job.maskOff, job.maskWords, p + 1, L - 1 - p, sd.node, sd.offset, r };
			workLen[at + 2 * c] = p;
			workLen[at + 2 * c + 1] = L - 1 - p;
			candSeed[at / 2 + c] = myCand;
		}
	}
	if (lane == 0) state[r] = st;
}
__global__ void __launch_bounds__(64) k_long_select(DGraph g, const LongJob* __restrict__ jobs, uint32_t nReads, const LongSeed* __restrict__ seeds, uint64_t rcBase, uint32_t minClusterSize,
	uint32_t extraHeuristic, uint32_t maxCandidates, LongState* __restrict__ state, const LongAln* __restrict__ alns, const LongCell* __restrict__ cellPool, LongWork* __restrict__ work, uint32_t* __restrict__ workLen, uint32_t* __restrict__ candSeed,
	unsigned long long* __restrict__ workCount, uint64_t workCapacity)
{
	GC_RAISE_PRIO();
	const uint32_t r = blockIdx.x, lane = threadIdx.x;
	if (r >= nReads) return;
	longSelectRead(g, r, lane, jobs, seeds, minClusterSize, extraHeuristic, maxCandidates, state, alns, cellPool, work, workLen, candSeed, workCount, workCapacity);
}

#ifndef GC_LONG_MIN_WAVES
#define GC_LONG_MIN_WAVES 1
#endif
template <int LANES, bool PERSISTENT, bool BAND = false, bool CLIP = false>
#ifndef GC_LONG_WAVES_ONE
#define GC_LONG_WAVES_ONE 5
#endif
__global__ void __launch_bounds__(64) __attribute__((amdgpu_waves_per_eu(LANES == 1 ? GC_LONG_WAVES_ONE : GC_LONG_MIN_WAVES, 8))) k_long_extend(DGraph g, const CorrectnessTables* __restrict__ ct, const uint64_t* __restrict__ masks, ExtendConfig cfg,
	const LongWork* __restrict__ work, const uint32_t* __restrict__ order, uint32_t nWork, unsigned long long* __restrict__ scratch, uint64_t wordsPerLane,
	unsigned long long* __restrict__ tracePool, unsigned long long* __restrict__ traceCursor, uint64_t traceCapacity, LongWorkResult* __restrict__ results, unsigned long long* __restrict__ counters,
	unsigned long long* __restrict__ nextSlot, uint32_t retryStatus, const unsigned long long* __restrict__ nWorkOnDevice, uint32_t* __restrict__ capListOut, unsigned long long* __restrict__ capCountOut)
{
	__shared__ WaveLdsT<LANES> lds;
	if (nWorkOnDevice) nWork = (uint32_t)*nWorkOnDevice;
	if (LANES > 1 && threadIdx.x >= LANES) return;
	const uint32_t lane = LANES == 1 ? 0u : threadIdx.x;
	const bool leader = LANES > 1 || threadIdx.x == 0;
	WaveScratch wsx;
	wsx.base = scratch + (uint64_t)blockIdx.x * wordsPerLane * LANES;
	wsx.lane = lane;
	wsx.lanes = LANES;
	wsx.maxSlices = cfg.maxSlices; wsx.maxItems = cfg.maxItems; wsx.maxTrace = cfg.maxTrace;
	wsx.maxCols = LANES == 1 ? cfg.maxCols : 0;
	wsx.allLanes = LANES == 1;
	wsx.regCap = cfg.regCap;
	ExtCounters cnt {};
	bool done = false;
	while (true) {
		unsigned long long first = 0;
		if (!PERSISTENT) { if (done) break; done = true; first = (unsigned long long)blockIdx.x * LANES; }
		else {
			if (threadIdx.x == 0) first = atomicAdd(nextSlot, (unsigned long long)LANES);
			if (LANES > 1) first = __shfl(first, 0);
			else first = (unsigned long long)__builtin_amdgcn_readfirstlane((uint32_t)first) | ((unsigned long long)__builtin_amdgcn_readfirstlane((uint32_t)(first >> 32)) << 32);
		}
		if (first >= nWork) break;
		const uint32_t slot = (uint32_t)first + lane;
		if (slot >= nWork) break;
		const uint32_t w = order[slot];
		if (retryStatus != 0 && results[w].status != retryStatus) { if (PERSISTENT) continue; else break; }
		LongWork it = work[w];
		LongWorkResult res { 0, 0, EXT_FAILED, 0, 0 };
		if (it.seqLen > 0) {
			uint32_t nTrace = 0;
			int32_t score = 0;
			EqSource eqSrc { masks + it.maskOff, it.maskWords, it.startBit };
			if (CLIP) res.status = extendSeedWave<LANES == 1, true, true>(g, *ct, eqSrc, cfg.bandwidth, (lds_u32*)&lds.w[0][0], wsx, (int)it.seqLen, it.node, it.offset, 0, nTrace, score, cnt,
				cfg.rampBandwidth, cfg.maxCells, cfg.forceGlobal != 0, cfg.clipErrorCost(), cfg.xDrop);
			else if (BAND) res.status = extendSeedWave<LANES == 1, true>(g, *ct, eqSrc, cfg.bandwidth, (lds_u32*)&lds.w[0][0], wsx, (int)it.seqLen, it.node, it.offset, 0, nTrace, score, cnt,
				cfg.rampBandwidth, cfg.maxCells, cfg.forceGlobal != 0);
			else res.status = extendSeedWave<LANES == 1>(g, *ct, eqSrc, cfg.bandwidth, (lds_u32*)&lds.w[0][0], wsx, (int)it.seqLen, it.node, it.offset, 0, nTrace, score, cnt);
			res.score = score;
			res.pad = cnt.flattenTie;
			if (res.status == EXT_OK) {
				unsigned long long base = 0;
				if (leader) base = atomicAdd(traceCursor, (unsigned long long)nTrace);
				if (LANES == 1) base = (unsigned long long)__builtin_amdgcn_readfirstlane((uint32_t)base) | ((unsigned long long)__builtin_amdgcn_readfirstlane((uint32_t)(base >> 32)) << 32);
				if (base + nTrace <= traceCapacity) {
					if (LANES == 1) { for (uint32_t i = threadIdx.x; i < nTrace; i += 64) tracePool[base + i] = wsx.word(wsx.traceBase(i, 0)); }
					else for (uint32_t i = 0; i < nTrace; i++) tracePool[base + i] = wsx.word(wsx.traceBase(i, 0));
					res.traceOff = base;
					res.traceLen = nTrace;
				} else res.status = EXT_OVERFLOW;
			}
		}
		if (leader) results[w] = res;
		if (leader && capListOut && res.status == EXT_LDS_CAP) capListOut[atomicAdd(capCountOut, 1ull)] = w;
	}
	if (cnt.extensions && leader) {
		atomicAdd(&counters[0], cnt.dpTiles);
		atomicAdd(&counters[1], cnt.recomputeTiles);
		atomicAdd(&counters[2], cnt.columnSteps);
		atomicAdd(&counters[3], cnt.traceItems);
		atomicAdd(&counters[4], cnt.extensions);
		atomicAdd(&counters[5], cnt.backtraceTiles);
#ifdef GC_STAMPS
		for (int i = 0; i < 16; i++) atomicAdd(&counters[8 + i], cnt.cyc[i]);
#endif
	}
}

__device__ __forceinline__ void longMergeRead(const DGraph& g, const uint32_t r, const uint32_t lane, const LongJob* __restrict__ jobs, const LongSeed* __restrict__ seeds, const uint32_t* __restrict__ candSeed,
	const LongWorkResult* __restrict__ results, const unsigned long long* __restrict__ tracePool,
	LongState* state, LongAln* alns, LongCell* cellPool, unsigned long long* __restrict__ cellCursor, uint64_t cellCapacity, uint32_t extraHeuristic)
{
	LongState st = state[r];
	if (st.candCount == 0 || st.status != 0) return;
	LongJob job = jobs[r];
	LongAln* mine = alns + job.alnBegin;
	const int L = (int)job.readLen;
	const uint32_t nAlnAtSelect = st.nAln;
	for (uint32_t c = 0; c < st.candCount && st.status == 0; c++) {
		const uint32_t pair = st.candBegin + c;
		const uint32_t seedIdx = candSeed[pair];
		LongSeed sd = seeds[seedIdx];
		if (c > 0) {
			if (seedCutEndToEnd(sd.goodness, st.e2eScore, extraHeuristic)) { st.si = job.seedEnd; break; }
			if (seedCutBudget(sd.goodness, st.extended, job.extendSeeds, st.worstExtended, extraHeuristic)) { st.si = job.seedEnd; break; }
			int sk = seedSkipped(g, sd, mine, nAlnAtSelect, st.nAln, cellPool, extraHeuristic);
			if (sk == 2) { st.status = 1; break; }
			if (sk == 1) continue;
		}
		st.worstExtended = sd.goodness;
		st.extended++;
		const LongWorkResult rb = results[2 * pair], rf = results[2 * pair + 1];
		const int p = (int)sd.seqPos;
		bool runB = p > 0, runF = p < L - 1;
		uint32_t stB = runB ? rb.status : EXT_FAILED, stF = runF ? rf.status : EXT_FAILED;
		if (runB) st.pad1 += rb.pad & 1u;
		if (runF && stB != EXT_ASSERT) st.pad1 += rf.pad & 1u;
		if (stB == EXT_ASSERT || stF == EXT_ASSERT) { st.status = 1; break; }
		if (stB == EXT_OVERFLOW || stF == EXT_OVERFLOW) { st.status = 2; break; }
		if (stB == EXT_LDS_CAP || stF == EXT_LDS_CAP) { st.status = 5; break; }
		bool hasB = stB == EXT_OK, hasF = stF == EXT_OK;
		if (!hasB && !hasF) continue;
		uint32_t nB = rb.traceLen, nF = rf.traceLen;
		uint32_t useB = hasB ? (hasF ? nB - 1 : nB) : 0;
		uint32_t total = useB + (hasF ? nF : 0);
		if (st.nAln >= job.alnCap) { st.status = 3; break; }
		unsigned long long base = 0;
		if (lane == 0) base = atomicAdd(cellCursor, (unsigned long long)total);
		base = __shfl(base, 0);
		if (base + total > cellCapacity) { st.status = 4; break; }
		LongCell* outCells = cellPool + base;
		for (uint32_t i = lane; i < useB; i += 64) {
			TraceCell tc = unpackCell(tracePool[rb.traceOff + i]);
			uint32_t off = tc.offsetAndSwitch & 255u;
			int32_t id = g.nodeIDs[tc.node];
			uint32_t orig = g.nodeOffset[tc.node] + off;
			LongCell oc;
			oc.node = id ^ 1;
			oc.offset = g.origSize[id] - 1 - orig;
			oc.seqPos = (uint32_t)(p - 1 - tc.seqPos);
			oc.nodeSwitch = (i + 1 < nB) ? ((unpackCell(tracePool[rb.traceOff + i + 1]).offsetAndSwitch >> 8) & 1u) : 0u;
			outCells[i] = oc;
		}
		if (hasF) for (uint32_t i = lane; i < nF; i += 64) {
			TraceCell tc = unpackCell(tracePool[rf.traceOff + (nF - 1 - i)]);
			LongCell oc;
			oc.node = g.nodeIDs[tc.node];
			oc.offset = g.nodeOffset[tc.node] + (tc.offsetAndSwitch & 255u);
			oc.seqPos = (uint32_t)(p + 1 + tc.seqPos);
			oc.nodeSwitch = (tc.offsetAndSwitch >> 8) & 1u;
			outCells[useB + i] = oc;
		}
		__threadfence_block();
		LongAln al;
		al.start = outCells[0].seqPos;
		al.end = outCells[total - 1].seqPos + 1;
		al.score = (uint32_t)((hasB ? rb.score : 0) + (hasF ? rf.score : 0));
		al.goodness = sd.goodness;
		al.traceOff = base;
		al.traceLen = total;
		al.pad = 0;
		uint32_t e2e = 0;
		if (lane == 0) {
			mine[st.nAln] = al;
			e2e = endToEndScore(mine, st.nAln + 1, (uint32_t)L, st.e2eScore);
		}
		st.nAln++;
		st.e2eScore = __shfl(e2e, 0);
		__threadfence_block();
	}
	st.candCount = 0;
	if (lane == 0) state[r] = st;
}

__global__ void __launch_bounds__(64) k_long_merge(DGraph g, const LongJob* __restrict__ jobs, uint32_t nReads, const LongSeed* __restrict__ seeds, const uint32_t* __restrict__ candSeed,
	const LongWorkResult* __restrict__ results, const unsigned long long* __restrict__ tracePool,
	LongState* state, LongAln* alns, LongCell* cellPool, unsigned long long* __restrict__ cellCursor, uint64_t cellCapacity, uint32_t extraHeuristic)
{
	GC_RAISE_PRIO();
	const uint32_t r = blockIdx.x;
	if (r >= nReads) return;
	longMergeRead(g, r, threadIdx.x, jobs, seeds, candSeed, results, tracePool, state, alns, cellPool, cellCursor, cellCapacity, extraHeuristic);
}

#ifndef GC_ORDER_THREADS
#define GC_ORDER_THREADS 256
#endif
__global__ void __launch_bounds__(GC_ORDER_THREADS) k_long_order(const uint32_t* __restrict__ workLen, const unsigned long long* __restrict__ workCount, uint32_t* __restrict__ order, uint32_t shift, uint32_t mode)
{
	GC_RAISE_PRIO();
	__shared__ uint32_t hist[1024];
	__shared__ uint32_t start[1024];
	const uint32_t n = (uint32_t)*workCount, tid = threadIdx.x, T = GC_ORDER_THREADS;
	if (mode == 0) { for (uint32_t i = tid; i < n; i += T) order[i] = i; return; }
	for (uint32_t b = tid; b < 1024; b += T) hist[b] = 0;
	__syncthreads();
	for (uint32_t i = tid; i < n; i += T) { uint32_t b = workLen[i] >> shift; atomicAdd(&hist[1023 - (b < 1023 ? b : 1023)], 1u); }
	__syncthreads();
#if GC_ORDER_THREADS == 1024
	if (tid == 0) { uint32_t at = 0; for (uint32_t b = 0; b < 1024; b++) { start[b] = at; at += hist[b]; } }
#else
	if (tid < 64) {
		uint32_t mine[16], sum = 0;
		for (uint32_t k = 0; k < 16; k++) { mine[k] = hist[tid * 16 + k]; sum += mine[k]; }
		uint32_t incl = sum;
		for (int d = 1; d < 64; d <<= 1) { const uint32_t o = __shfl_up(incl, d); if ((int)tid >= d) incl += o; }
		uint32_t at = incl - sum;
		for (uint32_t k = 0; k < 16; k++) { start[tid * 16 + k] = at; at += mine[k]; }
	}
#endif
	__syncthreads();
	for (uint32_t i = tid; i < n; i += T) { uint32_t b = workLen[i] >> shift; order[atomicAdd(&start[1023 - (b < 1023 ? b : 1023)], 1u)] = i; }
}

__global__ void k_publish(const unsigned long long* __restrict__ src, unsigned long long* __restrict__ dst, uint32_t nWords)
{
	GC_RAISE_PRIO();
	if (threadIdx.x < nWords) { dst[threadIdx.x] = src[threadIdx.x]; __threadfence_system(); }
}

__global__ void k_zero_words(unsigned long long* __restrict__ dst, uint32_t nWords)
{
	GC_RAISE_PRIO();
	if (threadIdx.x < nWords) dst[threadIdx.x] = 0;
}

__global__ void __launch_bounds__(256) k_long_finish(uint32_t nReads, const LongState* __restrict__ state, LongReadResult* __restrict__ results)
{
	GC_RAISE_PRIO();
	uint32_t r = blockIdx.x * blockDim.x + threadIdx.x;
	if (r >= nReads) return;
	LongState st = state[r];
	LongReadResult rr { st.status == 1 ? 0u : st.nAln, st.extended, st.status, st.pad1 };
	results[r] = rr;
}


void launchSeedLookup(hipStream_t stream, const SeedIndex& idx, const char* bases, const uint64_t* readOff, uint32_t nReads,
	uint64_t* matchCursor, uint32_t* readMatchOff, uint32_t* readMatchCount, uint2* matches, uint64_t matchCapacity, uint32_t* tmp, uint64_t totalBases, const uint32_t* chunkRead, const uint64_t* packed, const uint64_t* invalid)
{
	if (nReads == 0) return;
	uint64_t probeBlocks = (totalBases + 255) / 256;
	if (probeBlocks > 65536) probeBlocks = 65536;
	if (probeBlocks) hipLaunchKernelGGL(k_seed_probe, dim3((uint32_t)probeBlocks), dim3(256), 0, stream, idx, bases, readOff, chunkRead, packed, invalid, nReads, totalBases, tmp);
	uint32_t blocks = nReads < 16384 ? nReads : 16384;
	hipLaunchKernelGGL(k_seed_compact, dim3(blocks), dim3(64), 0, stream, readOff, nReads, tmp, matchCursor, readMatchOff, readMatchCount, matches, matchCapacity);
}

uint64_t extendSlabBytes(const ExtendConfig& cfg)
{
	uint64_t b = sizeof(SliceInfo) * (uint64_t)cfg.maxSlices + sizeof(NodeItem) * (uint64_t)cfg.maxItems + sizeof(Pending) * (uint64_t)cfg.maxPending + sizeof(WCol) * 64 + sizeof(TraceCell) * (uint64_t)cfg.maxTrace + sizeof(uint32_t) * (uint64_t)cfg.maxItems;
	return (b + 63) & ~63ull;
}

uint32_t extendGridLanes(uint32_t nWork)
{
	uint32_t lanes = 256u * 16u * 64u;
	uint32_t need = (nWork + 63) / 64 * 64;
	return need < lanes ? need : lanes;
}

void launchExtend(hipStream_t stream, const DGraph& g, const CorrectnessTables* ct, const uint8_t* iupac, const ExtendConfig& cfg,
	const ExtItem* work, uint32_t nWork, const char* bases, ExtResult* results, uint8_t* scratch, uint64_t slabBytes,
	PoolCell* tracePool, unsigned long long* traceCursor, uint64_t traceCapacity, unsigned long long* counters, uint32_t retryStatus, uint32_t retryLanes, ExtSelection sel)
{
	if (nWork == 0) return;
	const uint32_t upper = sel.mode == 1 ? 2 * sel.nFrags : nWork;
	uint32_t lanes = retryStatus ? retryLanes : extendGridLanes(upper);
	if (cfg.clipOn()) hipLaunchKernelGGL(k_extend_slab_clip, dim3(lanes / 64), dim3(64), 0, stream, g, ct, iupac, cfg, work, nWork, bases, results, scratch, slabBytes, tracePool, traceCursor, traceCapacity, counters, retryStatus, sel);
	else if (cfg.bandControls()) hipLaunchKernelGGL(k_extend_slab_band, dim3(lanes / 64), dim3(64), 0, stream, g, ct, iupac, cfg, work, nWork, bases, results, scratch, slabBytes, tracePool, traceCursor, traceCapacity, counters, retryStatus, sel);
	else hipLaunchKernelGGL(k_extend_slab, dim3(lanes / 64), dim3(64), 0, stream, g, ct, iupac, cfg, work, nWork, bases, results, scratch, slabBytes, tracePool, traceCursor, traceCapacity, counters, retryStatus, sel);
}

void launchBuildAnchors(hipStream_t stream, const DGraph& g, const Fragment* frags, uint32_t nFrags, const FragSeed* seeds, const ExtResult* ext,
	const PoolCell* tracePool, int32_t splitLen, AnchorRec* anchors, uint32_t* fragStatus, uint32_t* fragExtended,
	uint32_t* pathPool, unsigned long long* pathCursor, uint64_t pathCapacity, AnchorRounds rounds, uint32_t* readTies)
{
	if (nFrags == 0) return;
	hipLaunchKernelGGL(k_build_anchors, dim3((nFrags + 63) / 64), dim3(64), 0, stream, g, frags, nFrags, seeds, ext, tracePool, splitLen, anchors, fragStatus, fragExtended, pathPool, pathCursor, pathCapacity, rounds, readTies);
}

uint64_t chainScratchBytes(const ChainCaps& caps)
{
	uint64_t b = 8ull * caps.capBack + 8ull * caps.capAnchors + 8ull * caps.capEndpoints + 4ull * caps.capAnchors + 4ull * (caps.capAnchors + 1) + 4ull * caps.capTable + 6ull * (caps.capAnchors + 1) + 256;
	b += 6ull * (caps.capAnchors + 1) + 8ull * caps.capEndpoints + 64;
	return (b + 63) & ~63ull;
}

uint32_t chainGridBlocks(uint32_t nReads) { return nReads < 2048 ? nReads : 2048; }
uint32_t chainScratchBlocks(uint32_t nReads) { return nReads < 1024 ? nReads : 1024; }

bool chainLdsLaunch(uint32_t fewestSlots, bool forceScratch) { return forceScratch || fewestSlots <= 2 * CHAIN_LDS_ANCHORS; }

void launchChain(hipStream_t stream, const DGraph& g, const ReadChainJob* jobs, uint32_t nReads, const AnchorRec* anchors, const Fragment* frags, const uint32_t* fragStatus,
	int32_t splitLen, int32_t splitGap, ChainCaps caps, uint8_t* scratch, uint32_t* chainOut, uint32_t* chainLen, unsigned long long* chainScore, uint32_t* chainStatus, bool plainScan, bool forceScratch, uint32_t fewestSlots)
{
	if (nReads == 0) return;
	const bool ldsLaunch = chainLdsLaunch(fewestSlots, forceScratch);
	const uint32_t scratchFlags = (plainScan ? 2u : 0u) | (ldsLaunch ? 0u : 4u);
	const bool small = caps.capAnchors <= CHAIN_LDS_ANCHORS / 2 && caps.capTable <= CHAIN_LDS_WIDTH / 2;
	if (!ldsLaunch) {}
	else if (small) hipLaunchKernelGGL(HIP_KERNEL_NAME(k_chain<2>), dim3(chainGridBlocks(nReads)), dim3(64), 0, stream, g, jobs, nReads, anchors, frags, fragStatus, splitLen, splitGap, caps, scratch, chainScratchBytes(caps), chainOut, chainLen, chainScore, chainStatus, forceScratch ? 1u : 0u);
	else hipLaunchKernelGGL(HIP_KERNEL_NAME(k_chain<1>), dim3(chainGridBlocks(nReads)), dim3(64), 0, stream, g, jobs, nReads, anchors, frags, fragStatus, splitLen, splitGap, caps, scratch, chainScratchBytes(caps), chainOut, chainLen, chainScore, chainStatus, forceScratch ? 1u : 0u);
	const bool cannotBeNeeded = !forceScratch && caps.capAnchors <= CHAIN_LDS_ANCHORS / (small ? 2 : 1) && caps.capEndpoints <= CHAIN_LDS_ENTRIES / (small ? 2 : 1) && caps.capTable <= CHAIN_LDS_WIDTH / (small ? 2 : 1);
	hipLaunchKernelGGL(HIP_KERNEL_NAME(k_chain<0>), dim3(cannotBeNeeded ? (nReads < 64 ? nReads : 64) : chainScratchBlocks(nReads)), dim3(64), 0, stream, g, jobs, nReads, anchors, frags, fragStatus, splitLen, splitGap, caps, scratch, chainScratchBytes(caps), chainOut, chainLen, chainScore, chainStatus, scratchFlags);
}

uint64_t longWaveWordsPerLane(const ExtendConfig& cfg) { return waveScratchWords(cfg.maxSlices, cfg.maxItems, cfg.maxTrace, cfg.maxCols); }

void launchLongInit(hipStream_t stream, const LongJob* jobs, uint32_t nReads, LongState* state)
{
	if (nReads) hipLaunchKernelGGL(k_long_init, dim3((nReads + 255) / 256), dim3(256), 0, stream, jobs, nReads, state);
}
void launchLongSelect(hipStream_t stream, const DGraph& g, const LongJob* jobs, uint32_t nReads, const LongSeed* seeds, uint64_t rcBase, uint32_t minClusterSize, uint32_t extraHeuristic, uint32_t maxCandidates,
	LongState* state, const LongAln* alns, const LongCell* cellPool, LongWork* work, uint32_t* workLen, uint32_t* candSeed, unsigned long long* workCount, uint64_t workCapacity)
{
	if (maxCandidates < 1) maxCandidates = 1;
	if (maxCandidates > LONG_MAX_CANDIDATES) maxCandidates = LONG_MAX_CANDIDATES;
	if (nReads) hipLaunchKernelGGL(k_long_select, dim3(nReads), dim3(64), 0, stream, g, jobs, nReads, seeds, rcBase, minClusterSize, extraHeuristic, maxCandidates, state, alns, cellPool, work, workLen, candSeed, workCount, workCapacity);
}
uint32_t longExtendTeamSize(uint32_t nWork, uint32_t teamOverride)
{
	if (teamOverride) return teamOverride;
	(void)nWork;
	return 1;
}

void launchLongExtend(hipStream_t stream, const DGraph& g, const CorrectnessTables* ct, const uint64_t* masks, const ExtendConfig& cfg, const LongWork* work, const uint32_t* order, uint32_t nWork,
	unsigned long long* scratch, uint32_t lanes, uint32_t blocks, unsigned long long* tracePool, unsigned long long* traceCursor, uint64_t traceCapacity, LongWorkResult* results, unsigned long long* counters,
	unsigned long long* nextSlot, uint32_t retryStatus, const unsigned long long* nWorkOnDevice, uint32_t* capListOut, unsigned long long* capCountOut)
{
	if (!nWork) return;
	uint64_t words = longWaveWordsPerLane(cfg);
	const bool persistent = nWorkOnDevice || (uint64_t)blocks * lanes < nWork;
	const bool band = cfg.bandControls();
	const bool clip = cfg.clipOn();
#define GC_LAUNCH_ONE(N, P, B, C) hipLaunchKernelGGL(HIP_KERNEL_NAME(k_long_extend<N, P, B, C>), dim3(blocks), dim3(64), 0, stream, g, ct, masks, cfg, work, order, nWork, scratch, words, tracePool, traceCursor, traceCapacity, results, counters, nextSlot, retryStatus, nWorkOnDevice, capListOut, capCountOut)
#define GC_LAUNCH_TEAM(N) do { if (clip) { if (persistent) GC_LAUNCH_ONE(N, true, true, true); else GC_LAUNCH_ONE(N, false, true, true); } \
	else if (band) { if (persistent) GC_LAUNCH_ONE(N, true, true, false); else GC_LAUNCH_ONE(N, false, true, false); } \
	else if (persistent) GC_LAUNCH_ONE(N, true, false, false); else GC_LAUNCH_ONE(N, false, false, false); } while (0)
	switch (lanes) {
		case 1: GC_LAUNCH_TEAM(1); break;
		case 2: GC_LAUNCH_TEAM(2); break;
		case 4: GC_LAUNCH_TEAM(4); break;
		case 8: GC_LAUNCH_TEAM(8); break;
		case 16: GC_LAUNCH_TEAM(16); break;
		case 32: GC_LAUNCH_TEAM(32); break;
		default: GC_LAUNCH_TEAM(64); break;
	}
#undef GC_LAUNCH_TEAM
#undef GC_LAUNCH_ONE
}
__global__ void __launch_bounds__(256) k_build_fragment_work(DGraph g, const Fragment* __restrict__ frags, const uint32_t* __restrict__ fragFirstSeed, uint32_t nFrags,
	const FragSeed* __restrict__ readSeeds, const uint64_t* __restrict__ readOffsets, uint64_t totalBases, uint32_t splitLen, FragSeed* __restrict__ fragSeeds, ExtItem* __restrict__ work,
	ExtResult* __restrict__ results)
{
	const uint32_t F = blockIdx.x * 256 + threadIdx.x;
	if (F >= nFrags) return;
	const Fragment fr = frags[F];
	const uint64_t readOff = readOffsets[fr.read], len = readOffsets[fr.read + 1] - readOff;
	const FragSeed* seeds = readSeeds + fragFirstSeed[F];
	for (uint32_t k = 0; k < fr.seedEnd - fr.seedBegin; k++) {
		const FragSeed s = seeds[k];
		const uint32_t slot = fr.seedBegin + k, p = s.seqPos - fr.l;
		fragSeeds[slot] = s;
		ExtItem b;
		b.seqOff = totalBases + readOff + (len - fr.l - p);
		b.seqLen = p;
		twinOf(g, s.node, s.offset, b.node, b.offset);
		b.pad = fr.read;
		ExtItem f;
		f.seqOff = readOff + fr.l + p + 1;
		f.seqLen = splitLen - 1 - p;
		f.node = s.node;
		f.offset = s.offset;
		f.pad = fr.read;
		work[2 * (size_t)slot] = b;
		work[2 * (size_t)slot + 1] = f;
		if (results) {
			results[2 * (size_t)slot] = ExtResult { 0, 0, EXT_NOT_RUN, 0, 0 };
			results[2 * (size_t)slot + 1] = ExtResult { 0, 0, EXT_NOT_RUN, 0, 0 };
		}
	}
}
void launchBuildFragmentWork(hipStream_t stream, const DGraph& g, const Fragment* frags, const uint32_t* fragFirstSeed, uint32_t nFrags, const FragSeed* readSeeds, const uint64_t* readOffsets,
	uint64_t totalBases, uint32_t splitLen, FragSeed* fragSeeds, ExtItem* work, ExtResult* results)
{
	if (nFrags) hipLaunchKernelGGL(k_build_fragment_work, dim3((nFrags + 255) / 256), dim3(256), 0, stream, g, frags, fragFirstSeed, nFrags, readSeeds, readOffsets, totalBases, splitLen, fragSeeds, work, results);
}
void launchLongMerge(hipStream_t stream, const DGraph& g, const LongJob* jobs, uint32_t nReads, const LongSeed* seeds, const uint32_t* candSeed, const LongWorkResult* results,
	const unsigned long long* tracePool, LongState* state, LongAln* alns, LongCell* cellPool, unsigned long long* cellCursor, uint64_t cellCapacity, uint32_t extraHeuristic)
{
	if (nReads) hipLaunchKernelGGL(k_long_merge, dim3(nReads), dim3(64), 0, stream, g, jobs, nReads, seeds, candSeed, results, tracePool, state, alns, cellPool, cellCursor, cellCapacity, extraHeuristic);
}
void launchLongOrder(hipStream_t stream, const uint32_t* workLen, const unsigned long long* workCount, uint32_t* order, uint32_t maxLen, uint32_t mode)
{
	uint32_t shift = 0;
	while ((maxLen >> shift) > 1023) shift++;
	hipLaunchKernelGGL(k_long_order, dim3(1), dim3(GC_ORDER_THREADS), 0, stream, workLen, workCount, order, shift, mode);
}
void launchPublish(hipStream_t stream, const unsigned long long* src, unsigned long long* dst, uint32_t nWords)
{
	hipLaunchKernelGGL(k_publish, dim3(1), dim3(64), 0, stream, src, dst, nWords);
}
void launchZeroWords(hipStream_t stream, unsigned long long* dst, uint32_t nWords)
{
	hipLaunchKernelGGL(k_zero_words, dim3(1), dim3(64), 0, stream, dst, nWords);
}
void launchLongFinish(hipStream_t stream, uint32_t nReads, const LongState* state, LongReadResult* results)
{
	if (nReads) hipLaunchKernelGGL(k_long_finish, dim3((nReads + 255) / 256), dim3(256), 0, stream, nReads, state, results);
}

__global__ void __launch_bounds__(64) k_test_max_x_score(const uint64_t* __restrict__ vp, const uint64_t* __restrict__ vn, const int32_t* __restrict__ scoreEnd, uint32_t n, double errorCost, int cells, int32_t* __restrict__ out)
{
	const uint32_t i = blockIdx.x * 64 + threadIdx.x;
	if (i < n) out[i] = clipMaxXScore(WS { vp[i], vn[i], scoreEnd[i] }, errorCost, cells);
}
void launchTestMaxXScore(hipStream_t stream, const uint64_t* vp, const uint64_t* vn, const int32_t* scoreEnd, uint32_t n, double errorCost, int cells, int32_t* out)
{
	if (n) hipLaunchKernelGGL(k_test_max_x_score, dim3((n + 63) / 64), dim3(64), 0, stream, vp, vn, scoreEnd, n, errorCost, cells, out);
}

uint64_t longSlabBytes(const ExtendConfig& cfg) { return (extendSlabBytes(cfg) + sizeof(TraceCell) * (uint64_t)cfg.maxTrace + 63) & ~63ull; }

void launchLongPass(hipStream_t stream, const DGraph& g, const CorrectnessTables* ct, const uint8_t* iupac, const ExtendConfig& cfg, const LongJob* jobs, uint32_t nReads,
	const LongSeed* seeds, const char* bases, uint64_t rcBase, uint32_t minClusterSize, uint32_t extraHeuristic, uint8_t* scratch, uint64_t slabBytes,
	LongCell* cellPool, unsigned long long* cellCursor, uint64_t cellCapacity, LongAln* alns, LongReadResult* results, unsigned long long* counters)
{
	if (nReads == 0) return;
	uint32_t blocks = (nReads + 63) / 64;
	if (cfg.clipOn())
		hipLaunchKernelGGL(HIP_KERNEL_NAME(k_long_pass<true, true>), dim3(blocks), dim3(64), 0, stream, g, ct, iupac, cfg, jobs, nReads, seeds, bases, rcBase, minClusterSize, extraHeuristic, scratch, slabBytes,
			cellPool, cellCursor, cellCapacity, alns, results, counters);
	else if (cfg.bandControls())
		hipLaunchKernelGGL(k_long_pass<true>, dim3(blocks), dim3(64), 0, stream, g, ct, iupac, cfg, jobs, nReads, seeds, bases, rcBase, minClusterSize, extraHeuristic, scratch, slabBytes,
			cellPool, cellCursor, cellCapacity, alns, results, counters);
	else
		hipLaunchKernelGGL(k_long_pass<false>, dim3(blocks), dim3(64), 0, stream, g, ct, iupac, cfg, jobs, nReads, seeds, bases, rcBase, minClusterSize, extraHeuristic, scratch, slabBytes,
			cellPool, cellCursor, cellCapacity, alns, results, counters);
}

}
```

graphchainer_amd/csrc/hip/gc_kernels.hpp:

```cpp
#pragma once
#include "gc_device.hpp"

#ifndef GC_HELPER_PRIO
#define GC_HELPER_PRIO 3
#endif
#if GC_HELPER_PRIO
#define GC_RAISE_PRIO() __builtin_amdgcn_s_setprio(GC_HELPER_PRIO)
#else
#define GC_RAISE_PRIO() ((void)0)
#endif
#ifndef GC_ED_PRIO
#define GC_ED_PRIO 0
#endif
#if GC_ED_PRIO
#define GC_RAISE_ED_PRIO() __builtin_amdgcn_s_setprio(GC_ED_PRIO)
#else
#define GC_RAISE_ED_PRIO() ((void)0)
#endif

namespace gcdev {

struct SeedIndex {
	const uint64_t* table;
	const uint64_t* wideKmers;
	uint32_t tableMask;
	const uint32_t* filter;
	uint32_t filterShift;
	const uint64_t* startPos;
	const uint64_t* positions;
	uint32_t nKeys;
	uint32_t maxCount;
	int32_t k, w;
};

struct ExtItem {
	uint64_t seqOff;
	uint32_t seqLen;
	uint32_t node;
	uint32_t offset;
	uint32_t pad;
};

struct ExtResult {
	uint64_t traceOff;
	uint32_t traceLen;
	uint32_t status;
	int32_t score;
	uint32_t pad;
};

struct Fragment;
struct ExtSelection { uint32_t mode = 0; const Fragment* frags = nullptr; uint32_t nFrags = 0; const uint32_t* list = nullptr; const unsigned long long* listCount = nullptr; };
struct AnchorRounds {
	uint32_t lazy = 0, round = 0, parkAll = 0;
	const uint32_t* pending = nullptr; const unsigned long long* pendingCount = nullptr;
	uint32_t* nextList = nullptr; unsigned long long* nextListCount = nullptr;
	uint32_t* nextPending = nullptr; unsigned long long* nextPendingCount = nullptr;
	uint32_t* fragNext = nullptr;
};
struct Fragment {
	uint32_t read;
	uint32_t l;
	uint32_t seedBegin, seedEnd;
};

struct FragSeed {
	uint32_t node, offset;
	uint32_t seqPos;
	uint32_t pad;
};

struct AnchorRec {
	uint32_t valid;
	uint32_t x, y;
	uint32_t firstNode, firstOffset, firstSeqPos;
	uint32_t lastNode, lastOffset, lastSeqPos;
	int32_t score;
	uint32_t pathLen;
	uint32_t pad;
	uint64_t pathOff;
};

struct ReadChainJob {
	uint32_t slotBegin, nSlots;
	uint32_t chainBegin;
	uint32_t nKeys;
	uint32_t fragBegin, nFrags;
};

struct ChainCaps { uint32_t capAnchors, capEndpoints, capTable, capBack; };

struct GlueRead { uint32_t nSeeds, seedOff, nFrags, fragBegin, nSlots, slotBegin, failed, pad; };
struct GlueElem;
struct GlueStaging {
	uint32_t *mPos, *mStartLo, *mStartHi;
	uint32_t *sSeqPos, *sNode, *sOffset, *sGood, *sCluster;
	GlueElem* sortBuf; uint32_t* sortScratch;
	uint32_t* winBuf;
};

struct LongSeed {
	uint32_t node;
	uint32_t seqPos;
	uint32_t goodness;
	uint16_t clusterSize;
	uint8_t offset;
	uint8_t pad;
};

struct LongJob {
	uint64_t maskOff;
	uint32_t maskWords;
	uint32_t alnCap;
	uint64_t readOff;
	uint32_t readLen;
	uint32_t seedBegin, seedEnd;
	uint32_t alnBegin;
	uint32_t extendSeeds;
	uint32_t pad;
};

struct LongCell {
	int32_t node;
	uint32_t offset;
	uint32_t seqPos;
	uint32_t nodeSwitch;
};

struct LongAln {
	uint32_t start, end;
	uint32_t score;
	uint32_t goodness;
	uint64_t traceOff;
	uint32_t traceLen;
	uint32_t pad;
};

struct LongReadResult { uint32_t nAlignments, seedsExtended, status, pad; };

struct LongState { uint32_t si, nAln, extended, status, e2eScore, candBegin, candCount, pad1, worstExtended, pad2; };
struct LongWork {
	uint64_t maskOff;
	uint32_t maskWords, startBit;
	uint32_t seqLen, node, offset;
	uint32_t read;
};
struct LongWorkResult { uint64_t traceOff; uint32_t traceLen, status; int32_t score; uint32_t pad; };

void launchSeedLookup(hipStream_t stream, const SeedIndex& idx, const char* bases, const uint64_t* readOff, uint32_t nReads,
	uint64_t* matchCursor, uint32_t* readMatchOff, uint32_t* readMatchCount, uint2* matches, uint64_t matchCapacity, uint32_t* tmp, uint64_t totalBases, const uint32_t* chunkRead, const uint64_t* packed, const uint64_t* invalid);

void launchSeedCaps(hipStream_t stream, const SeedIndex& idx, uint32_t nReads, const uint8_t* invalidRead, const uint2* matches, const uint32_t* readMatchOff, const uint32_t* readMatchCount,
	uint32_t* readSeedCap, uint32_t* readSeedOff, unsigned long long* total);
void launchSeedGlue(hipStream_t stream, const SeedIndex& idx, const DGraph& g, const uint64_t* readOff, uint32_t nReads, const uint8_t* invalidRead, const uint2* matches, const uint32_t* readMatchOff,
	const uint32_t* readMatchCount, const uint32_t* readSeedOff, const uint32_t* winCapOff, double density, uint32_t splitLen, uint32_t splitGap, bool longPass, const GlueStaging& st,
	uint32_t* perRead , LongSeed* longSeeds, FragSeed* readSeeds, Fragment* frags, uint32_t* fragFirstSeed, ReadChainJob* jobs, GlueRead* out, unsigned long long* cursors, bool forceGlobal = false);
uint64_t glueElemBytes();
struct SeedHit;
struct SeedLookup;
struct SeedHitArrays { uint32_t *node, *offset, *seqPos, *matchLen, *raw; };
void launchSeedResolve(hipStream_t stream, const SeedLookup& lookup, const SeedHit* hits, uint64_t nHits, const uint32_t* readHitOff, uint32_t nReads, const uint64_t* readOff, const SeedHitArrays& out,
	unsigned long long* firstBad);
void launchSeedGlueHits(hipStream_t stream, const DGraph& g, const uint64_t* readOff, uint32_t nReads, const uint8_t* invalidRead, const SeedHitArrays& hits, const uint32_t* readSeedOff, const uint32_t* winCapOff,
	uint32_t splitLen, uint32_t splitGap, bool longPass, const GlueStaging& st, uint32_t* perRead , LongSeed* longSeeds, FragSeed* readSeeds, Fragment* frags, uint32_t* fragFirstSeed,
	ReadChainJob* jobs, GlueRead* out, unsigned long long* cursors, bool forceGlobal = false);
struct MxmIndexView;
void launchMxmPrefixTable(hipStream_t stream, const MxmIndexView& ix, uint32_t* table );
struct MxmSeedRun {
	uint64_t nCandidates = 0;
	hipError_t candidates(hipStream_t q, const MxmIndexView& ix, const char* bases, const uint64_t* readOff, const uint32_t* tileOff , uint32_t nReads, uint32_t nTiles, int32_t mode, uint32_t minLen);
	hipError_t select(hipStream_t q, uint32_t nReads, uint64_t maxCount, uint64_t& nFinal);
	hipError_t write(hipStream_t q, uint32_t nReads, uint64_t nFinal, SeedHit* out, uint32_t* readHitOff);
	~MxmSeedRun();
private:
	void *tiles = nullptr, *work = nullptr, *sortTmp = nullptr, *ranges = nullptr;
	size_t workBytes = 0;
	SeedHit* cand = nullptr;
	uint64_t *sortedOuter = nullptr, *keptOff = nullptr;
	uint32_t *order = nullptr, *candOff = nullptr;
};
void launchTestMaxXScore(hipStream_t stream, const uint64_t* vp, const uint64_t* vn, const int32_t* scoreEnd, uint32_t n, double errorCost, int cells, int32_t* out);
void launchTestStdSort(hipStream_t stream, unsigned long long* elems, const uint64_t* off, uint32_t nArrays, uint32_t* scratch, long depthLimit);

struct FragReads { const uint64_t* masks; const uint64_t* maskOff; const uint32_t* maskWords; const uint64_t* readOff; uint64_t totalBases; };
uint32_t extendFragWaves();
uint64_t extendFragScratchBytes(uint32_t waves);
void launchExtendFrag(hipStream_t stream, const DGraph& g, const CorrectnessTables* ct, int32_t bandwidth, const ExtItem* work, uint32_t nWork, const FragReads& reads, ExtResult* results,
	uint4* itemScratch, uint32_t scratchWaves, PoolCell* tracePool, unsigned long long* traceCursor, uint64_t traceCapacity, unsigned long long* counters, ExtSelection sel, unsigned long long* claim,
	uint32_t* retryList, unsigned long long* retryCount, unsigned long long* stamps = nullptr, uint64_t maxCells = ~0ull, bool forceGlobal = false);
void launchBuildNodeRecs(hipStream_t stream, const DGraph& g, NodeRec* out);
uint64_t extendSlabBytes(const ExtendConfig& cfg);
uint32_t extendGridLanes(uint32_t nWork);
void launchExtend(hipStream_t stream, const DGraph& g, const CorrectnessTables* ct, const uint8_t* iupac, const ExtendConfig& cfg,
	const ExtItem* work, uint32_t nWork, const char* bases, ExtResult* results, uint8_t* scratch, uint64_t slabBytes,
	PoolCell* tracePool, unsigned long long* traceCursor, uint64_t traceCapacity, unsigned long long* counters,
	uint32_t retryStatus = 0, uint32_t retryLanes = 4096, ExtSelection sel = ExtSelection());

void launchBuildAnchors(hipStream_t stream, const DGraph& g, const Fragment* frags, uint32_t nFrags, const FragSeed* seeds, const ExtResult* ext,
	const PoolCell* tracePool, int32_t splitLen, AnchorRec* anchors, uint32_t* fragStatus, uint32_t* fragExtended,
	uint32_t* pathPool, unsigned long long* pathCursor, uint64_t pathCapacity, AnchorRounds rounds = AnchorRounds(), uint32_t* readTies = nullptr);

struct AnchorArrays { uint32_t *x, *y, *firstNode, *firstOffset, *firstSeqPos, *lastNode, *lastOffset, *lastSeqPos; int32_t* score; unsigned long long* pathOff; uint32_t* path; };
void launchAnchorCounts(hipStream_t stream, const ReadChainJob* jobs, uint32_t nReads, const Fragment* frags, const uint32_t* fragStatus, const uint32_t* fragExtended, const AnchorRec* anchors,
	uint4* perRead, uint32_t* readSlotEnd, unsigned long long* readOff, unsigned long long* hostTotals);
void launchAnchorCompact(hipStream_t stream, const ReadChainJob* jobs, uint32_t nReads, const AnchorRec* anchors, const uint32_t* pathPool, const uint32_t* readSlotEnd, const unsigned long long* readOff, const AnchorArrays& out);

uint64_t chainScratchBytes(const ChainCaps& caps);
uint32_t chainGridBlocks(uint32_t nReads);
uint32_t chainScratchBlocks(uint32_t nReads);
bool chainLdsLaunch(uint32_t fewestSlots, bool forceScratch);
void launchChain(hipStream_t stream, const DGraph& g, const ReadChainJob* jobs, uint32_t nReads, const AnchorRec* anchors, const Fragment* frags, const uint32_t* fragStatus,
	int32_t splitLen, int32_t splitGap, ChainCaps caps, uint8_t* scratch, uint32_t* chainOut, uint32_t* chainLen, unsigned long long* chainScore, uint32_t* chainStatus, bool plainScan, bool forceScratch = false,
	uint32_t fewestSlots = 0);

void launchLongPass(hipStream_t stream, const DGraph& g, const CorrectnessTables* ct, const uint8_t* iupac, const ExtendConfig& cfg, const LongJob* jobs, uint32_t nReads,
	const LongSeed* seeds, const char* bases, uint64_t rcBase, uint32_t minClusterSize, uint32_t extraHeuristic, uint8_t* scratch, uint64_t slabBytes,
	LongCell* cellPool, unsigned long long* cellCursor, uint64_t cellCapacity, LongAln* alns, LongReadResult* results, unsigned long long* counters);
uint64_t longSlabBytes(const ExtendConfig& cfg);
uint64_t longWaveWordsPerLane(const ExtendConfig& cfg);
void launchLongInit(hipStream_t stream, const LongJob* jobs, uint32_t nReads, LongState* state);
void launchLongSelect(hipStream_t stream, const DGraph& g, const LongJob* jobs, uint32_t nReads, const LongSeed* seeds, uint64_t rcBase, uint32_t minClusterSize, uint32_t extraHeuristic, uint32_t maxCandidates,
	LongState* state, const LongAln* alns, const LongCell* cellPool, LongWork* work, uint32_t* workLen, uint32_t* candSeed, unsigned long long* workCount, uint64_t workCapacity);
uint32_t longExtendTeamSize(uint32_t nWork, uint32_t teamOverride);
void launchLongExtend(hipStream_t stream, const DGraph& g, const CorrectnessTables* ct, const uint64_t* masks, const ExtendConfig& cfg, const LongWork* work, const uint32_t* order, uint32_t nWork,
	unsigned long long* scratch, uint32_t lanes, uint32_t blocks, unsigned long long* tracePool, unsigned long long* traceCursor, uint64_t traceCapacity, LongWorkResult* results, unsigned long long* counters,
	unsigned long long* nextSlot, uint32_t retryStatus = 0, const unsigned long long* nWorkOnDevice = nullptr, uint32_t* capListOut = nullptr, unsigned long long* capCountOut = nullptr);
void launchLongMerge(hipStream_t stream, const DGraph& g, const LongJob* jobs, uint32_t nReads, const LongSeed* seeds, const uint32_t* candSeed, const LongWorkResult* results,
	const unsigned long long* tracePool, LongState* state, LongAln* alns, LongCell* cellPool, unsigned long long* cellCursor, uint64_t cellCapacity, uint32_t extraHeuristic);
struct PathSeqJob {
	uint64_t srcOff;
	uint64_t outOff;
	uint32_t count;
	uint32_t outCap;
	uint32_t firstOffset, lastOffset;
};
struct EdRead { uint64_t readOff, eqOff; uint32_t len, words; };
struct EdPair {
	uint64_t lettersOff;
	uint32_t m;
	uint32_t lenIndex;
	uint32_t read;
	uint32_t k;
};
void launchLongPathSeq(hipStream_t stream, const DGraph& g, const PathSeqJob* jobs, uint32_t nJobs, const LongCell* cellPool, char* letters, uint32_t* outLen);
struct StitchInfo {
	uint64_t start;
	uint64_t cells;
	uint32_t len;
	uint32_t firstOffset, lastOffset;
	uint32_t status;
	uint32_t scoreSum;
	uint32_t pad;
};
void launchStitch(hipStream_t stream, const DGraph& g, const ReadChainJob* jobs, uint32_t nReads, const AnchorRec* anchors, const Fragment* frags, const uint32_t* fragStatus,
	const uint32_t* chainOut, const uint32_t* chainLen, const uint32_t* chainStatus, const uint32_t* pathPool, uint64_t pathCapacity, long long colinearGap, uint32_t* slotOf,
	uint32_t* regions, uint32_t* dense, uint64_t denseCap, unsigned long long* denseCursor, StitchInfo* info,
	uint32_t setMax = 0, uint32_t bfsCap = 0, int sizeClass = 0, unsigned long long* spill = nullptr);
uint64_t stitchSpillWordsPerBlock();
uint32_t stitchSpillBlocks(uint32_t nReads);
uint64_t stitchRegionWords(uint64_t totalSlots, uint64_t nReads);
uint64_t stitchDenseWords(uint64_t totalSlots, uint64_t nReads);
void launchChainPathSeq(hipStream_t stream, const DGraph& g, const PathSeqJob* jobs, uint32_t nJobs, const uint32_t* pathNodes, const uint32_t* altNodes, char* letters, uint32_t* outLen);
uint32_t editDistanceMaxK(uint32_t unitBlocks);
void launchEditDistanceBlock(hipStream_t stream, uint32_t threads, const EdPair* pairs, uint32_t nPairs, const EdRead* reads, const char* bases, const uint64_t* eqMasks,
	const char* letters, const uint32_t* lettersLen, int64_t* outDistance);
uint32_t editDistanceBlockMaxRows();
uint32_t editDistanceTeamMaxK(uint32_t pairsPerWave);
void launchEditDistanceTeam(hipStream_t stream, uint32_t pairsPerWave, const EdPair* pairs, uint32_t nPairs, const EdRead* reads, const char* bases, const uint64_t* eqMasks,
	const char* letters, const uint32_t* lettersLen, int64_t* outDistance);
void launchEditDistance(hipStream_t stream, uint32_t unitBlocks, const EdPair* pairs, uint32_t nPairs, const EdRead* reads, const char* bases, const uint64_t* eqMasks,
	const char* letters, const uint32_t* lettersLen, int64_t* outDistance);
struct OutNames { const uint32_t* nameOff; const char* nameBytes; };
struct OutJob {
	uint64_t cellOff;
	uint64_t readOff;
	uint32_t cellLen, readLen;
	uint32_t flags;
	uint32_t pad;
};
struct OutRec {
	uint64_t nodePathLen, nodePathStart, nodePathEnd;
	uint32_t pathTextLen, cigarLen, vgLen, steps;
	uint32_t matches, mismatches, insertions, deletions;
	uint32_t readStart, readEnd;
};
void launchOutCount(hipStream_t stream, const DGraph& g, const OutNames& names, const uint8_t* iupac, const OutJob* jobs, uint32_t nJobs, const LongCell* cellPool, const char* bases,
	OutRec* recs, uint64_t* offsets, uint32_t* mapSizeAtCell, unsigned long long* totals);
void launchOutWrite(hipStream_t stream, const DGraph& g, const OutNames& names, const uint8_t* iupac, const OutJob* jobs, uint32_t nJobs, const LongCell* cellPool, const char* bases,
	OutRec* recs, const uint64_t* offsets, uint32_t* mapSizeAtCell, char* pathText, char* cigarText, uint8_t* vgBytes);
void launchDeflatePlan(hipStream_t stream, const uint8_t* raw, const uint64_t* rawOff, uint32_t nStreams, uint8_t* lens, uint2* plan);
void launchDeflateWrite(hipStream_t stream, const uint8_t* raw, const uint64_t* rawOff, uint32_t nStreams, const uint8_t* lens, const uint2* plan, uint8_t* out, const uint64_t* outOff);
uint32_t deflateLzLensStride();
void launchDeflateLzPlan(hipStream_t stream, const uint8_t* raw, const uint64_t* rawOff, uint32_t nStreams, uint8_t* lens, uint2* plan);
void launchDeflateLzWrite(hipStream_t stream, const uint8_t* raw, const uint64_t* rawOff, uint32_t nStreams, const uint8_t* lens, const uint2* plan, uint8_t* out, const uint64_t* outOff);
uint64_t buildMinimizerPairsDevice(const DGraph& g, const int32_t* idOrderDev, uint32_t nIds, uint32_t k, uint32_t w, uint64_t** outKeys, uint64_t** outValues);
void launchBuildFragmentWork(hipStream_t stream, const DGraph& g, const Fragment* frags, const uint32_t* fragFirstSeed, uint32_t nFrags, const FragSeed* readSeeds, const uint64_t* readOffsets,
	uint64_t totalBases, uint32_t splitLen, FragSeed* fragSeeds, ExtItem* work, ExtResult* results = nullptr);
void launchPackReads(hipStream_t stream, const uint64_t* readOff, uint32_t nReads, uint64_t totalBases, char* bases, const uint64_t* maskOff, const uint32_t* maskWords, uint64_t* masks,
	const uint64_t* eqOff, uint64_t* eqMasks, uint8_t* readInvalid, uint64_t* packed, uint64_t* invalidBits, uint32_t* chunkRead);
struct EdPathJob {
	uint64_t queryOff;
	uint64_t targetOff;
	uint64_t opsOff;
	uint32_t queryLen, targetLen;
	int32_t best;
	uint32_t pad;
};
#define ED_PATH_LEAF_CELLS 52432ull
uint64_t editPathScratchBytes(uint32_t maxQ, uint32_t maxT);
uint32_t editPathGridBlocks(uint32_t nJobs);
void launchEditPath(hipStream_t stream, const EdPathJob* jobs, uint32_t nJobs, const char* letters, const char* bases, uint8_t* scratch, uint32_t maxQ, uint32_t maxT,
	uint8_t* opsOut, uint32_t* opsLen);
struct FastChainJob {
	uint64_t srcOff;
	uint64_t lettersOff;
	uint64_t readOff;
	uint64_t traceOff;
	uint32_t count, cells;
	uint32_t firstOffset, lastOffset;
	uint32_t x, y;
};
void launchFastChainScore(hipStream_t stream, const FastChainJob* jobs, uint32_t nJobs, const char* letters, const uint32_t* lettersLen, const char* bases, int64_t* outScore);
void launchFastChainTrace(hipStream_t stream, const DGraph& g, const FastChainJob* jobs, uint32_t nJobs, const uint32_t* pathNodes, const uint32_t* altNodes,
	int32_t* traceNode, uint32_t* traceOffset, uint32_t* traceSeqPos, uint8_t* traceSwitch, uint32_t* written);
void launchLongOrder(hipStream_t stream, const uint32_t* workLen, const unsigned long long* workCount, uint32_t* order, uint32_t maxLen, uint32_t mode);
void launchPublish(hipStream_t stream, const unsigned long long* src, unsigned long long* dst, uint32_t nWords);
void launchZeroWords(hipStream_t stream, unsigned long long* dst, uint32_t nWords);
void launchLongFinish(hipStream_t stream, uint32_t nReads, const LongState* state, LongReadResult* results);


}
```

graphchainer_amd/csrc/host/gc_switches.hpp:

```cpp
#pragma once
#include <algorithm>
#include <cstddef>
#include <cstdint>
#include <cstdlib>
#include <cstring>
#include <optional>

namespace gc {

inline constexpr int LONG_TOKENS_MAX = 2;

struct Switches {
	std::optional<size_t> hostThreads;
	std::optional<size_t> batchThreads;
	std::optional<size_t> buildThreads;
	size_t resultCacheMin = 32ull << 20;
	int spinSync = 2;
	int syncPollUs = 40;
	int longToken = 1;
	std::optional<int> longTokens;
	bool debugTimes = false;
	bool debugEd = false;
	bool deviceGlue = true;
	bool hostAnchors = false;
	bool extLazy = true;
	bool extendSlab = false;
	bool poolsWorstCase = false;
	bool hostStitch = false;
	std::optional<int> stitchClass;
	bool chainPlainScan = false;
	std::optional<uint32_t> edFirstK;
	bool seederBuildOnHost = false;
	bool buildReferenceContainers = false;
	std::optional<int64_t> testExtMaxItems;
	std::optional<int64_t> testExtMaxPending;
	std::optional<int64_t> testExtMaxTrace;
	std::optional<uint32_t> testExtRetryMaxItems;
	std::optional<int64_t> testLongMaxItems;
	std::optional<int64_t> testLongMaxCols;
	std::optional<int64_t> testLongCellsPerBase;
	std::optional<uint32_t> testLongMaxAlignments;
	std::optional<uint64_t> testLongScratchGb;
	std::optional<int64_t> testStitchSetMax;
	std::optional<int64_t> testStitchBfsCap;
	std::optional<uint32_t> testSeedFilterBits;
	std::optional<long> testFailLong;
	bool testLongForceFallback = false;
	std::optional<uint32_t> testLongRegCap;
	std::optional<uint32_t> testLongMaxBlocks;
	std::optional<uint32_t> testLongTeam;
	uint32_t testLongOrder = 1;
	std::optional<uint32_t> testLongSpeculate;
	bool testChainForceScratch = false;
	std::optional<double> testPoolFirstGuess;
	size_t testPoolShrinkFloor = 64u << 20;
	bool testResultCachePoison = false;
	size_t testUploadSlice = (size_t)64 << 20;

	bool shareLongScratch() const { return longToken >= 1; }
	bool onePassAtATime() const { return longToken != 0; }

	static Switches fromEnvironment()
	{
		Switches s;
		if (const char* e = getenv("GC_HOST_THREADS")) s.hostThreads = (size_t)std::max(1, atoi(e));
		if (const char* e = getenv("GC_BATCH_THREADS")) s.batchThreads = (size_t)std::max(1, atoi(e));
		if (const char* e = getenv("GC_BUILD_THREADS")) { long v = atol(e); if (v >= 1) s.buildThreads = (size_t)v; }
		if (const char* e = getenv("GC_RESULT_CACHE_MIN")) s.resultCacheMin = (size_t)std::max(1ll, atoll(e));

		if (const char* e = getenv("GC_SPIN_SYNC")) s.spinSync = atoi(e);
		if (const char* e = getenv("GC_SYNC_POLL_US")) s.syncPollUs = std::max(1, atoi(e));
		if (const char* e = getenv("GC_LONG_TOKEN")) s.longToken = atoi(e);
		if (const char* e = getenv("GC_LONG_TOKENS")) s.longTokens = std::max(1, std::min(LONG_TOKENS_MAX, atoi(e)));
		s.debugTimes = getenv("GC_DEBUG_TIMES") != nullptr;
		s.debugEd = getenv("GC_DEBUG_ED") != nullptr;

		if (const char* e = getenv("GC_DEVICE_GLUE")) s.deviceGlue = !(atoi(e) == 0);
		if (const char* e = getenv("GC_HOST_ANCHORS")) s.hostAnchors = atoi(e) == 1;
		if (const char* e = getenv("GC_EXT_LAZY")) s.extLazy = !(atoi(e) == 0);
		if (const char* e = getenv("GC_EXTEND_SLAB")) s.extendSlab = atoi(e) == 1;
		if (const char* e = getenv("GC_POOLS_WORST_CASE")) s.poolsWorstCase = atoi(e) == 1;
		if (const char* e = getenv("GC_HOST_STITCH")) s.hostStitch = atoi(e) != 0;
		if (const char* e = getenv("GC_STITCH_CLASS")) s.stitchClass = atoi(e) == 3 ? 3 : 0;
		if (const char* e = getenv("GC_CHAIN_PLAIN_SCAN")) s.chainPlainScan = atoi(e) == 1;
		if (const char* e = getenv("GC_ED_FIRST_K")) s.edFirstK = (uint32_t)std::max(1, atoi(e));
		if (const char* e = getenv("GC_SEEDER_BUILD")) s.seederBuildOnHost = !strcmp(e, "host");
		if (const char* e = getenv("GC_BUILD_REFERENCE_CONTAINERS")) s.buildReferenceContainers = atoi(e) == 1;

		if (const char* e = getenv("GC_TEST_EXT_MAX_ITEMS")) s.testExtMaxItems = atoll(e);
		if (const char* e = getenv("GC_TEST_EXT_MAX_PENDING")) s.testExtMaxPending = atoll(e);
		if (const char* e = getenv("GC_TEST_EXT_MAX_TRACE")) s.testExtMaxTrace = atoll(e);
		if (const char* e = getenv("GC_TEST_EXT_RETRY_MAX_ITEMS")) s.testExtRetryMaxItems = (uint32_t)std::max(8, atoi(e));
		if (const char* e = getenv("GC_TEST_LONG_MAX_ITEMS")) s.testLongMaxItems = atoll(e);
		if (const char* e = getenv("GC_TEST_LONG_MAX_COLS")) s.testLongMaxCols = atoll(e);
		if (const char* e = getenv("GC_TEST_LONG_CELLS_PER_BASE")) s.testLongCellsPerBase = atoll(e);
		if (const char* e = getenv("GC_TEST_LONG_MAX_ALIGNMENTS")) s.testLongMaxAlignments = (uint32_t)std::max(1, std::min(1 << 16, atoi(e)));
		if (const char* e = getenv("GC_TEST_LONG_SCRATCH_GB")) s.testLongScratchGb = (uint64_t)std::max(1, atoi(e));
		if (const char* e = getenv("GC_TEST_STITCH_SET_MAX")) s.testStitchSetMax = atoll(e);
		if (const char* e = getenv("GC_TEST_STITCH_BFS_CAP")) s.testStitchBfsCap = atoll(e);
		if (const char* e = getenv("GC_TEST_SEED_FILTER_BITS")) s.testSeedFilterBits = (uint32_t)std::max(10, std::min(30, atoi(e)));
		if (const char* e = getenv("GC_TEST_FAIL_LONG")) s.testFailLong = atol(e);
		s.testLongForceFallback = getenv("GC_TEST_LONG_FORCE_FALLBACK") != nullptr;
		if (const char* e = getenv("GC_TEST_LONG_REG_CAP")) s.testLongRegCap = (uint32_t)std::max(1, std::min(64, atoi(e)));
		if (const char* e = getenv("GC_TEST_LONG_MAX_BLOCKS")) s.testLongMaxBlocks = (uint32_t)std::max(1, atoi(e));
		if (const char* e = getenv("GC_TEST_LONG_TEAM")) { int v = atoi(e); if (v == 1 || v == 2 || v == 4 || v == 8 || v == 16 || v == 32 || v == 64) s.testLongTeam = (uint32_t)v; }
		if (const char* e = getenv("GC_TEST_LONG_ORDER")) s.testLongOrder = (uint32_t)atoi(e);
		if (const char* e = getenv("GC_TEST_LONG_SPECULATE")) s.testLongSpeculate = (uint32_t)std::min(2, std::max(1, atoi(e)));
		s.testChainForceScratch = getenv("GC_TEST_CHAIN_FORCE_SCRATCH") != nullptr;
		if (const char* e = getenv("GC_TEST_POOL_FIRST_GUESS")) s.testPoolFirstGuess = std::max(0.0, atof(e));
		if (const char* e = getenv("GC_TEST_POOL_SHRINK_FLOOR")) s.testPoolShrinkFloor = (size_t)std::max(0ll, atoll(e));
		s.testResultCachePoison = getenv("GC_TEST_RESULT_CACHE_POISON") != nullptr;
		if (const char* e = getenv("GC_TEST_UPLOAD_SLICE")) s.testUploadSlice = (size_t)std::max(1, atoi(e));
		return s;
	}
};

inline const Switches& processSwitches() { static const Switches s = Switches::fromEnvironment(); return s; }

}
```

Before: 71610.

## Add persistent continuation kernel with device work queue for whole-read extension

After: 20190. 0.282x the previous value.

```diff
diff --git a/graphchainer_amd/csrc/batch/gc_batch_long.inc b/graphchainer_amd/csrc/batch/gc_batch_long.inc
--- a/graphchainer_amd/csrc/batch/gc_batch_long.inc
+++ b/graphchainer_amd/csrc/batch/gc_batch_long.inc
@@ -70,7 +70,8 @@
 			if (n) HIP_CHECK(hipMemcpyAsync(dLongJobs, hJobs, n * sizeof(LongJob), hipMemcpyHostToDevice, ls));
 			syncStream(ls);
 			dLongState = st->longState.reserve<LongState>(n);
-			workCapacity = 8 * n + 64;
+			longContinue = sw.longContinue && longExtendTeamSize(1, sw.testLongTeam.value_or(0)) == 1;
+			workCapacity = (longContinue ? 16 : 8) * n + 64;
 			dLongWork = st->longWork.reserve<LongWork>(workCapacity);
 			dLongWorkResults = st->longWorkResults.reserve<LongWorkResult>(workCapacity);
 			dCandSeed = st->longCandSeed.reserve<uint32_t>(2 * workCapacity);
@@ -79,10 +80,16 @@
 			dOrder = st->longOrder.reserve<uint32_t>(workCapacity);
 			roundTraceBudget = 0;
 			for (uint64_t r = 0; r < n; r++) { uint64_t len = R->offsets[r + 1] - R->offsets[r]; roundTraceBudget += 4 * ((P->force_global || clip.on() ? 2 * len + 2 : len + len / 2) + 1024); }
+			if (sw.testLongTracePool) roundTraceBudget = *sw.testLongTracePool;
 			dRoundTrace = st->longRoundTrace.reserve<unsigned long long>(roundTraceBudget);
+			if (longContinue) {
+				dLongPending = st->longPending.reserve<uint32_t>(n);
+				dLongReady = st->longReady.reserve<uint32_t>(workCapacity);
+			}
 			uint64_t scratchBudget = P->capacity.long_scratch_bytes > 0 ? (uint64_t)P->capacity.long_scratch_bytes : (48ull << 30) / (uint64_t)longTokenCount(sw.longTokens, n, st->batchesDone, st->fragShare);
 			if (sw.testLongScratchGb) scratchBudget = *sw.testLongScratchGb << 30;
 			scratchLanes = std::min<uint64_t>(std::min<uint64_t>(workCapacity + 64, 2 * n + 128), std::max<uint64_t>(2048, std::min<uint64_t>(65536 + 64, scratchBudget / (waveWords * 8))));
+			if (longContinue) scratchLanes = std::min<uint64_t>(scratchLanes, (uint64_t)longContinueWaves() + 64);
 			longScratchWords = scratchLanes * waveWords;
 			shareLongScratch = sw.shareLongScratch();
 			if (!shareLongScratch) dLongScratchOwn = st->longScratch.reserve<unsigned long long>(longScratchWords);
@@ -165,6 +172,7 @@
 		const double dbgT0 = nowUs();
 		launchLongInit(q, dLongJobs, (uint32_t)n, dLongState);
 		uint32_t lastWork = 0xffffffffu;
+		if (longContinue) launchZeroWords(q, cursor + 4, 2);
 
 		for (int round = 0; round < 4096; round++) {
 			launchZeroWords(q, cursor, 4);
@@ -172,14 +180,16 @@
 			if (round > 0 && lastWork > 0) maxCand = (uint32_t)std::min<uint64_t>(8, std::max<uint64_t>(1, (2 * n) / lastWork));
 			if (round > 0 && lastWork < 8192) maxCand = 8;
 			if (round > 0 && lastWork > 0) maxCand = (uint32_t)std::min<uint64_t>(maxCand, std::max<uint64_t>(1, (8 * n) / lastWork));
+			if (longContinue) maxCand = 1;
 			if (sw.testLongSpeculate) maxCand = *sw.testLongSpeculate;
-			launchLongSelect(q, G->dev, dLongJobs, (uint32_t)n, dLongSeeds, R->totalBases, (uint32_t)P->min_cluster_size, (uint32_t)P->extra_heuristic, maxCand, dLongState, dLongAlns, dLongCells, dLongWork, dWorkLen, dCandSeed, cursor, workCapacity);
+			launchLongSelect(q, G->dev, dLongJobs, (uint32_t)n, dLongSeeds, R->totalBases, (uint32_t)P->min_cluster_size, (uint32_t)P->extra_heuristic, maxCand, dLongState, dLongAlns, dLongCells, dLongWork, dWorkLen, dCandSeed, cursor, workCapacity, longContinue ? dLongPending : nullptr);
 			launchLongOrder(q, dWorkLen, cursor, dOrder, (uint32_t)maxReadLen, sw.testLongOrder);
-			launchPublish(q, cursor, (unsigned long long*)hCursor, 2);
+			launchPublish(q, cursor, (unsigned long long*)hCursor, longContinue ? 6 : 2);
 			const double tWait0 = nowUs();
 			syncStream(q);
 			dbgWaitUs += nowUs() - tWait0;
 			uint32_t nWorkItems = (uint32_t)hCursor[0];
+			if (longContinue && hCursor[5] != 0) throw DeviceError("the whole-read continuation launch timed out waiting for work item " + std::to_string((unsigned long long)hCursor[5] - 1));
 			if (nWorkItems == 0) break;
 			if (!dLongScratch) {
 				longTokenTake();
@@ -187,20 +197,31 @@
 			}
 			uint32_t team = longExtendTeamSize(nWorkItems, sw.testLongTeam.value_or(0));
 			uint32_t blocks = std::min<uint32_t>((nWorkItems + team - 1) / team, (uint32_t)std::max<uint64_t>(1, (scratchLanes - 64) / team));
+			if (longContinue) blocks = std::min<uint32_t>(blocks, longContinueWaves());
 			if (sw.testLongMaxBlocks) blocks = std::min<uint32_t>(blocks, *sw.testLongMaxBlocks);
 			if (timedRounds >= LONG_EVENT_RING) collect(timedRounds % LONG_EVENT_RING);
 			hipEvent_t ev0 = ring[2 * (timedRounds % LONG_EVENT_RING)], ev1 = ring[2 * (timedRounds % LONG_EVENT_RING) + 1];
 			HIP_CHECK(hipEventRecord(ev0, q));
+			if (longContinue) {
+				LongContinue lc {};
+				lc.jobs = dLongJobs; lc.seeds = dLongSeeds; lc.state = dLongState; lc.alns = dLongAlns; lc.cellPool = dLongCells; lc.cellCursor = dLongCursor; lc.cellCapacity = cellBudget;
+				lc.work = dLongWork; lc.candSeed = dCandSeed; lc.pending = dLongPending; lc.ready = dLongReady;
+				lc.tail = cursor; lc.head = cursor + 2; lc.timeout = cursor + 5; lc.deferred = cursor + 4;
+				lc.workCapacity = workCapacity; lc.nInitial = nWorkItems; lc.minClusterSize = (uint32_t)P->min_cluster_size; lc.extraHeuristic = (uint32_t)P->extra_heuristic;
+				lc.fixedCandidates = sw.testLongSpeculate ? *sw.testLongSpeculate : 0;
+				lc.maxSpins = 1u << 22;
+				launchLongContinue(q, G->dev, G->devTables, R->devMasks, lcfg, dOrder, dLongScratch, blocks, dRoundTrace, cursor + 1, roundTraceBudget, dLongWorkResults, dLongCursor + 8, dRetryList, cursor + 3, lc);
+			} else
 			launchLongExtend(q, G->dev, G->devTables, R->devMasks, lcfg, dLongWork, dOrder, nWorkItems, dLongScratch, team, blocks,
 				dRoundTrace, cursor + 1, roundTraceBudget, dLongWorkResults, dLongCursor + 8, cursor + 2, 0, nullptr, team == 1 ? dRetryList : nullptr, cursor + 3);
 			if (team == 1) {
-				if ((uint64_t)blocks * team < nWorkItems) launchZeroWords(q, cursor + 2, 1);
+				if (longContinue || (uint64_t)blocks * team < nWorkItems) launchZeroWords(q, cursor + 2, 1);
 				uint32_t retryBlocks = std::min<uint32_t>(128, (uint32_t)std::max<uint64_t>(1, (scratchLanes - 64) / 2));
-				launchLongExtend(q, G->dev, G->devTables, R->devMasks, lcfg, dLongWork, dRetryList, nWorkItems, dLongScratch, 2, retryBlocks,
+				launchLongExtend(q, G->dev, G->devTables, R->devMasks, lcfg, dLongWork, dRetryList, longContinue ? (uint32_t)workCapacity : nWorkItems, dLongScratch, 2, retryBlocks,
 					dRoundTrace, cursor + 1, roundTraceBudget, dLongWorkResults, dLongCursor + 8, cursor + 2, EXT_LDS_CAP, cursor + 3);
 			}
 			HIP_CHECK(hipEventRecord(ev1, q));
-			launchLongMerge(q, G->dev, dLongJobs, (uint32_t)n, dLongSeeds, dCandSeed, dLongWorkResults, dRoundTrace, dLongState, dLongAlns, dLongCells, dLongCursor, cellBudget, (uint32_t)P->extra_heuristic);
+			launchLongMerge(q, G->dev, dLongJobs, (uint32_t)n, dLongSeeds, dCandSeed, dLongWorkResults, dRoundTrace, dLongState, dLongAlns, dLongCells, dLongCursor, cellBudget, (uint32_t)P->extra_heuristic, longContinue);
 			lastWork = nWorkItems;
 			timedRounds++;
 			longRounds++;
diff --git a/graphchainer_amd/csrc/gc_batch.hip b/graphchainer_amd/csrc/gc_batch.hip
--- a/graphchainer_amd/csrc/gc_batch.hip
+++ b/graphchainer_amd/csrc/gc_batch.hip
@@ -65,6 +65,9 @@
 	uint32_t* dWorkLen = nullptr;
 	uint32_t* dRetryList = nullptr;
 	uint32_t* dOrder = nullptr;
+	bool longContinue = false;
+	uint32_t* dLongPending = nullptr;
+	uint32_t* dLongReady = nullptr;
 	unsigned long long* dRoundTrace = nullptr;
 	uint64_t scratchLanes = 0;
 	hipStream_t ls = nullptr;
diff --git a/graphchainer_amd/csrc/gc_runtime.hpp b/graphchainer_amd/csrc/gc_runtime.hpp
--- a/graphchainer_amd/csrc/gc_runtime.hpp
+++ b/graphchainer_amd/csrc/gc_runtime.hpp
@@ -551,7 +551,7 @@
 	DeviceBuffer longSeeds, longJobs, longAlns, longResults, longScratch, longCells, longCursor, longJobsFallback, longResultsFallback, longScratchFallback;
 	DeviceBuffer gluePerRead, glueCursors, glueOut, glueSeedCap, glueSeedOff, glueWinCapOff, glueU32[8], glueSort, gluePos, glueWin;
 	PinnedBuffer hGlueOut, hGlueWinCapOff, hGlueSmall;
-	DeviceBuffer longState, longWork, longWorkResults, longRoundTrace, longCandSeed, longWorkLen, longOrder;
+	DeviceBuffer longState, longWork, longWorkResults, longRoundTrace, longCandSeed, longWorkLen, longOrder, longPending, longReady;
 	PinnedBuffer hLongSeeds, hLongJobs, hLongAlns, hLongResults, hLongSmall, hLongCells;
 	template <typename F> void forEachDeviceBuffer(F f) const
 	{
@@ -573,7 +573,7 @@
 		f("glueWinCapOff", glueWinCapOff.bytes); f("glueU32[0]", glueU32[0].bytes); f("glueU32[1]", glueU32[1].bytes); f("glueU32[2]", glueU32[2].bytes); f("glueU32[3]", glueU32[3].bytes);
 		f("glueU32[4]", glueU32[4].bytes); f("glueU32[5]", glueU32[5].bytes); f("glueU32[6]", glueU32[6].bytes); f("glueU32[7]", glueU32[7].bytes); f("glueSort", glueSort.bytes);
 		f("gluePos", gluePos.bytes); f("glueWin", glueWin.bytes); f("longState", longState.bytes); f("longWork", longWork.bytes); f("longWorkResults", longWorkResults.bytes);
-		f("longRoundTrace", longRoundTrace.bytes); f("longCandSeed", longCandSeed.bytes); f("longWorkLen", longWorkLen.bytes); f("longOrder", longOrder.bytes);
+		f("longRoundTrace", longRoundTrace.bytes); f("longCandSeed", longCandSeed.bytes); f("longWorkLen", longWorkLen.bytes); f("longOrder", longOrder.bytes); f("longPending", longPending.bytes); f("longReady", longReady.bytes);
 		for (int k = 0; k < 2; k++) { f("edLong.letters", edLong[k].letters.bytes); f("edLong.jobs+pairs+out", edLong[k].jobs.bytes + edLong[k].lettersLen.bytes + edLong[k].pairs.bytes + edLong[k].out.bytes); }
 	}
 	~gc_stream()
diff --git a/graphchainer_amd/csrc/hip/gc_kernels.hip b/graphchainer_amd/csrc/hip/gc_kernels.hip
--- a/graphchainer_amd/csrc/hip/gc_kernels.hip
+++ b/graphchainer_amd/csrc/hip/gc_kernels.hip
@@ -1,5 +1,6 @@
 #include "gc_kernels.hpp"
 #include "gc_device_wave.hpp"
+#include "gc_long_queue.hpp"
 #include <cstdlib>
 
 namespace gcdev {
@@ -706,17 +707,26 @@
 	twinOffset = rev - g.nodeOffset[twinNode];
 }
 
-__device__ inline int onTrace(const LongCell* trace, uint32_t n, uint32_t seqPos, int32_t compareNode, uint32_t nodeOffset)
-{
-	if (!(trace[n - 1].seqPos > trace[0].seqPos)) return 2;
-	if (trace[n - 1].seqPos < seqPos || trace[0].seqPos > seqPos) return 0;
+template <bool V, class T> __device__ __forceinline__ T ldh(const T* p)
+{
+	if (!V) return *p;
+	static_assert(sizeof(T) % 4 == 0, "ldh: whole 32-bit words");
+	union U { T v; uint32_t w[sizeof(T) / 4]; __device__ U() {} } u;
+	for (uint32_t i = 0; i < sizeof(T) / 4; i++) u.w[i] = __hip_atomic_load((const uint32_t*)p + i, __ATOMIC_RELAXED, __HIP_MEMORY_SCOPE_AGENT);
+	return u.v;
+}
+
+template <bool V = false> __device__ inline int onTrace(const LongCell* trace, uint32_t n, uint32_t seqPos, int32_t compareNode, uint32_t nodeOffset)
+{
+	if (!(ldh<V>(&trace[n - 1].seqPos) > ldh<V>(&trace[0].seqPos))) return 2;
+	if (ldh<V>(&trace[n - 1].seqPos) < seqPos || ldh<V>(&trace[0].seqPos) > seqPos) return 0;
 	uint32_t lo = 0, hi = n;
 	while (lo < hi) {
 		uint32_t mid = (lo + hi) / 2;
-		if (trace[mid].seqPos < seqPos) lo = mid + 1; else hi = mid;
-	}
-	for (uint32_t i = lo; i < n && trace[i].seqPos == seqPos; i++)
-		if (trace[i].node == compareNode && trace[i].offset == nodeOffset) return 1;
+		if (ldh<V>(&trace[mid].seqPos) < seqPos) lo = mid + 1; else hi = mid;
+	}
+	for (uint32_t i = lo; i < n && ldh<V>(&trace[i].seqPos) == seqPos; i++)
+		if (ldh<V>(&trace[i].node) == compareNode && ldh<V>(&trace[i].offset) == nodeOffset) return 1;
 	return 0;
 }
 
@@ -869,6 +879,31 @@
 	}
 }
 
+__device__ inline uint32_t endToEndScoreKeyed(const LongAln* mine, uint32_t nAln, uint32_t readLen, uint32_t current)
+{
+	bool anyAtZero = false;
+	for (uint32_t a = 0; a < nAln; a++) if (ldh<true>(&mine[a].start) == 0) anyAtZero = true;
+	if (!anyAtZero) return current;
+	uint32_t contiguousEnd = 0, minGoodness = 0xffffffffu;
+	unsigned long long lastKey = 0;
+	for (uint32_t visited = 0; visited < nAln; visited++) {
+		unsigned long long bestKey = ~0ull;
+		for (uint32_t a = 0; a < nAln; a++) {
+			const unsigned long long key = (((unsigned long long)ldh<true>(&mine[a].start) << 32) | a) + 1;
+			if (key > lastKey && key < bestKey) bestKey = key;
+		}
+		lastKey = bestKey;
+		const uint32_t best = (uint32_t)(bestKey - 1);
+		const uint32_t start = ldh<true>(&mine[best].start), end = ldh<true>(&mine[best].end), goodness = ldh<true>(&mine[best].goodness);
+		if (visited == 0) { contiguousEnd = end; minGoodness = goodness; continue; }
+		if (start <= contiguousEnd) {
+			minGoodness = goodness < minGoodness ? goodness : minGoodness;
+			contiguousEnd = end > contiguousEnd ? end : contiguousEnd;
+		}
+	}
+	return contiguousEnd == readLen ? minGoodness : current;
+}
+
 
 __global__ void __launch_bounds__(256) k_long_init(const LongJob* __restrict__ jobs, uint32_t nReads, LongState* __restrict__ state)
 {
@@ -879,14 +914,14 @@
 	state[r] = st;
 }
 
-__device__ inline int seedSkipped(const DGraph& g, const LongSeed& sd, const LongAln* mine, uint32_t aFrom, uint32_t aTo, const LongCell* cellPool, uint32_t extraHeuristic)
+template <bool V = false> __device__ inline int seedSkipped(const DGraph& g, const LongSeed& sd, const LongAln* mine, uint32_t aFrom, uint32_t aTo, const LongCell* cellPool, uint32_t extraHeuristic)
 {
 	for (uint32_t a = aFrom; a < aTo; a++)
-		if (mine[a].start <= sd.seqPos && mine[a].end >= sd.seqPos && (extraHeuristic || mine[a].goodness > sd.goodness)) return 1;
+		if (ldh<V>(&mine[a].start) <= sd.seqPos && ldh<V>(&mine[a].end) >= sd.seqPos && (extraHeuristic || ldh<V>(&mine[a].goodness) > sd.goodness)) return 1;
 	int32_t compareNode = g.nodeIDs[sd.node];
 	uint32_t compareOffset = g.nodeOffset[sd.node] + sd.offset;
 	for (uint32_t a = aFrom; a < aTo; a++) {
-		int on = onTrace(cellPool + mine[a].traceOff, mine[a].traceLen, sd.seqPos, compareNode, compareOffset);
+		int on = onTrace<V>(cellPool + ldh<V>(&mine[a].traceOff), ldh<V>(&mine[a].traceLen), sd.seqPos, compareNode, compareOffset);
 		if (on == 2) return 2;
 		if (on == 1) return 1;
 	}
@@ -894,11 +929,13 @@
 }
 
 #define LONG_MAX_CANDIDATES 8
+enum : uint32_t { EXT_DEFER = 9 };
+template <bool V = false>
 __device__ __forceinline__ void longSelectRead(const DGraph& g, const uint32_t r, const uint32_t lane, const LongJob* __restrict__ jobs, const LongSeed* __restrict__ seeds, uint32_t minClusterSize,
-	uint32_t extraHeuristic, uint32_t maxCandidates, LongState* __restrict__ state, const LongAln* __restrict__ alns, const LongCell* __restrict__ cellPool, LongWork* __restrict__ work, uint32_t* __restrict__ workLen, uint32_t* __restrict__ candSeed,
-	unsigned long long* __restrict__ workCount, uint64_t workCapacity)
-{
-	LongState st = state[r];
+	uint32_t extraHeuristic, uint32_t maxCandidates, LongState* state, const LongAln* alns, const LongCell* cellPool, LongWork* work, uint32_t* workLen, uint32_t* candSeed,
+	unsigned long long* workCount, uint64_t workCapacity, uint32_t* pending = nullptr, const gcq::Queue* queue = nullptr)
+{
+	LongState st = ldh<V>(state + r);
 	st.candCount = 0;
 	if (st.status != 0) { if (lane == 0) state[r] = st; return; }
 	LongJob job = jobs[r];
@@ -915,7 +952,7 @@
 			|| seedCutBudget(sd.goodness, st.extended, job.extendSeeds, st.worstExtended, extraHeuristic));
 		const bool small = sd.clusterSize < minClusterSize;
 		int sk = 1;
-		if (valid && !cut && !small) sk = seedSkipped(g, sd, mine, 0, st.nAln, cellPool, extraHeuristic);
+		if (valid && !cut && !small) sk = seedSkipped<V>(g, sd, mine, 0, st.nAln, cellPool, extraHeuristic);
 		const uint64_t cutMask = __ballot(cut), assertMask = __ballot(sk == 2), candMask = __ballot(sk == 0);
 		const uint32_t nValid = job.seedEnd - si < 64 ? job.seedEnd - si : 64;
 		const uint32_t firstCut = cutMask ? (uint32_t)__ffsll((unsigned long long)cutMask) - 1 : 64;
@@ -936,8 +973,14 @@
 	st.si = si;
 	if (nCand > 0) {
 		unsigned long long at = 0;
-		if (lane == 0) at = atomicAdd(workCount, 2ull * nCand);
-		at = __shfl(at, 0);
+		if (V) {
+			if (lane == 0) at = gcq::reserve(*queue, 2 * nCand);
+			at = __shfl(at, 0);
+			if (at == gcq::NONE) return;
+		} else {
+			if (lane == 0) at = atomicAdd(workCount, 2ull * nCand);
+			at = __shfl(at, 0);
+		}
 		if (at + 2ull * nCand > workCapacity) { st.status = 2; nCand = 0; }
 		st.candBegin = (uint32_t)(at / 2);
 		st.candCount = nCand;
@@ -951,21 +994,30 @@
 			twinOf(g, sd.node, sd.offset, twinNode, twinOffset);
 			work[at + 2 * c] = LongWork { job.maskOff + 4ull * job.maskWords, job.maskWords, L - p, p, twinNode, twinOffset, r };
 			work[at + 2 * c + 1] = LongWork { job.maskOff, job.maskWords, p + 1, L - 1 - p, sd.node, sd.offset, r };
-			workLen[at + 2 * c] = p;
-			workLen[at + 2 * c + 1] = L - 1 - p;
+			if (!V) {
+				workLen[at + 2 * c] = p;
+				workLen[at + 2 * c + 1] = L - 1 - p;
+			}
 			candSeed[at / 2 + c] = myCand;
+		}
+		if (pending && lane == 0) gcq::store32(pending + r, 2 * nCand);
+		if (V) {
+			if (lane == 0) state[r] = st;
+			gcq::releaseFence();
+			if (lane == 0) gcq::publish(*queue, at, 2 * nCand);
+			return;
 		}
 	}
 	if (lane == 0) state[r] = st;
 }
 __global__ void __launch_bounds__(64) k_long_select(DGraph g, const LongJob* __restrict__ jobs, uint32_t nReads, const LongSeed* __restrict__ seeds, uint64_t rcBase, uint32_t minClusterSize,
 	uint32_t extraHeuristic, uint32_t maxCandidates, LongState* __restrict__ state, const LongAln* __restrict__ alns, const LongCell* __restrict__ cellPool, LongWork* __restrict__ work, uint32_t* __restrict__ workLen, uint32_t* __restrict__ candSeed,
-	unsigned long long* __restrict__ workCount, uint64_t workCapacity)
+	unsigned long long* __restrict__ workCount, uint64_t workCapacity, uint32_t* __restrict__ pending)
 {
 	GC_RAISE_PRIO();
 	const uint32_t r = blockIdx.x, lane = threadIdx.x;
 	if (r >= nReads) return;
-	longSelectRead(g, r, lane, jobs, seeds, minClusterSize, extraHeuristic, maxCandidates, state, alns, cellPool, work, workLen, candSeed, workCount, workCapacity);
+	longSelectRead(g, r, lane, jobs, seeds, minClusterSize, extraHeuristic, maxCandidates, state, alns, cellPool, work, workLen, candSeed, workCount, workCapacity, pending);
 }
 
 #ifndef GC_LONG_MIN_WAVES
@@ -1049,11 +1101,13 @@
 	}
 }
 
-__device__ __forceinline__ void longMergeRead(const DGraph& g, const uint32_t r, const uint32_t lane, const LongJob* __restrict__ jobs, const LongSeed* __restrict__ seeds, const uint32_t* __restrict__ candSeed,
-	const LongWorkResult* __restrict__ results, const unsigned long long* __restrict__ tracePool,
+template <bool V> __device__ __forceinline__ void longFenceOwn() { if (V) __threadfence(); else __threadfence_block(); }
+template <bool V = false>
+__device__ __forceinline__ void longMergeRead(const DGraph& g, const uint32_t r, const uint32_t lane, const LongJob* __restrict__ jobs, const LongSeed* __restrict__ seeds, const uint32_t* candSeed,
+	const LongWorkResult* results, const unsigned long long* tracePool,
 	LongState* state, LongAln* alns, LongCell* cellPool, unsigned long long* __restrict__ cellCursor, uint64_t cellCapacity, uint32_t extraHeuristic)
 {
-	LongState st = state[r];
+	LongState st = ldh<V>(state + r);
 	if (st.candCount == 0 || st.status != 0) return;
 	LongJob job = jobs[r];
 	LongAln* mine = alns + job.alnBegin;
@@ -1061,18 +1115,18 @@
 	const uint32_t nAlnAtSelect = st.nAln;
 	for (uint32_t c = 0; c < st.candCount && st.status == 0; c++) {
 		const uint32_t pair = st.candBegin + c;
-		const uint32_t seedIdx = candSeed[pair];
+		const uint32_t seedIdx = ldh<V>(candSeed + pair);
 		LongSeed sd = seeds[seedIdx];
 		if (c > 0) {
 			if (seedCutEndToEnd(sd.goodness, st.e2eScore, extraHeuristic)) { st.si = job.seedEnd; break; }
 			if (seedCutBudget(sd.goodness, st.extended, job.extendSeeds, st.worstExtended, extraHeuristic)) { st.si = job.seedEnd; break; }
-			int sk = seedSkipped(g, sd, mine, nAlnAtSelect, st.nAln, cellPool, extraHeuristic);
+			int sk = seedSkipped<V>(g, sd, mine, nAlnAtSelect, st.nAln, cellPool, extraHeuristic);
 			if (sk == 2) { st.status = 1; break; }
 			if (sk == 1) continue;
 		}
 		st.worstExtended = sd.goodness;
 		st.extended++;
-		const LongWorkResult rb = results[2 * pair], rf = results[2 * pair + 1];
+		const LongWorkResult rb = ldh<V>(results + 2 * pair), rf = ldh<V>(results + 2 * pair + 1);
 		const int p = (int)sd.seqPos;
 		bool runB = p > 0, runF = p < L - 1;
 		uint32_t stB = runB ? rb.status : EXT_FAILED, stF = runF ? rf.status : EXT_FAILED;
@@ -1093,7 +1147,7 @@
 		if (base + total > cellCapacity) { st.status = 4; break; }
 		LongCell* outCells = cellPool + base;
 		for (uint32_t i = lane; i < useB; i += 64) {
-			TraceCell tc = unpackCell(tracePool[rb.traceOff + i]);
+			TraceCell tc = unpackCell(ldh<V>(tracePool + rb.traceOff + i));
 			uint32_t off = tc.offsetAndSwitch & 255u;
 			int32_t id = g.nodeIDs[tc.node];
 			uint32_t orig = g.nodeOffset[tc.node] + off;
@@ -1101,11 +1155,11 @@
 			oc.node = id ^ 1;
 			oc.offset = g.origSize[id] - 1 - orig;
 			oc.seqPos = (uint32_t)(p - 1 - tc.seqPos);
-			oc.nodeSwitch = (i + 1 < nB) ? ((unpackCell(tracePool[rb.traceOff + i + 1]).offsetAndSwitch >> 8) & 1u) : 0u;
+			oc.nodeSwitch = (i + 1 < nB) ? ((unpackCell(ldh<V>(tracePool + rb.traceOff + i + 1)).offsetAndSwitch >> 8) & 1u) : 0u;
 			outCells[i] = oc;
 		}
 		if (hasF) for (uint32_t i = lane; i < nF; i += 64) {
-			TraceCell tc = unpackCell(tracePool[rf.traceOff + (nF - 1 - i)]);
+			TraceCell tc = unpackCell(ldh<V>(tracePool + rf.traceOff + (nF - 1 - i)));
 			LongCell oc;
 			oc.node = g.nodeIDs[tc.node];
 			oc.offset = g.nodeOffset[tc.node] + (tc.offsetAndSwitch & 255u);
@@ -1113,10 +1167,10 @@
 			oc.nodeSwitch = (tc.offsetAndSwitch >> 8) & 1u;
 			outCells[useB + i] = oc;
 		}
-		__threadfence_block();
+		longFenceOwn<V>();
 		LongAln al;
-		al.start = outCells[0].seqPos;
-		al.end = outCells[total - 1].seqPos + 1;
+		al.start = ldh<V>(&outCells[0].seqPos);
+		al.end = ldh<V>(&outCells[total - 1].seqPos) + 1;
 		al.score = (uint32_t)((hasB ? rb.score : 0) + (hasF ? rf.score : 0));
 		al.goodness = sd.goodness;
 		al.traceOff = base;
@@ -1125,11 +1179,12 @@
 		uint32_t e2e = 0;
 		if (lane == 0) {
 			mine[st.nAln] = al;
-			e2e = endToEndScore(mine, st.nAln + 1, (uint32_t)L, st.e2eScore);
+			if (V) { __threadfence(); e2e = endToEndScoreKeyed(mine, st.nAln + 1, (uint32_t)L, st.e2eScore); }
+			else e2e = endToEndScore(mine, st.nAln + 1, (uint32_t)L, st.e2eScore);
 		}
 		st.nAln++;
 		st.e2eScore = __shfl(e2e, 0);
-		__threadfence_block();
+		longFenceOwn<V>();
 	}
 	st.candCount = 0;
 	if (lane == 0) state[r] = st;
@@ -1137,12 +1192,149 @@
 
 __global__ void __launch_bounds__(64) k_long_merge(DGraph g, const LongJob* __restrict__ jobs, uint32_t nReads, const LongSeed* __restrict__ seeds, const uint32_t* __restrict__ candSeed,
 	const LongWorkResult* __restrict__ results, const unsigned long long* __restrict__ tracePool,
-	LongState* state, LongAln* alns, LongCell* cellPool, unsigned long long* __restrict__ cellCursor, uint64_t cellCapacity, uint32_t extraHeuristic)
+	LongState* state, LongAln* alns, LongCell* cellPool, unsigned long long* __restrict__ cellCursor, uint64_t cellCapacity, uint32_t extraHeuristic, uint32_t continued)
 {
 	GC_RAISE_PRIO();
 	const uint32_t r = blockIdx.x;
 	if (r >= nReads) return;
+	if (continued) {
+		LongState st = state[r];
+		if (st.status == 0 && st.candCount != 0) {
+			bool deferred = false;
+			for (uint32_t c = 0; c < 2 * st.candCount; c++) if (results[2 * st.candBegin + c].status == EXT_DEFER) deferred = true;
+			if (deferred) {
+				st.si = candSeed[st.candBegin];
+				st.candCount = 0;
+				if (threadIdx.x == 0) state[r] = st;
+				return;
+			}
+		}
+	}
 	longMergeRead(g, r, threadIdx.x, jobs, seeds, candSeed, results, tracePool, state, alns, cellPool, cellCursor, cellCapacity, extraHeuristic);
+}
+
+__device__ __forceinline__ unsigned long long longUniform64(unsigned long long v)
+{
+	return (unsigned long long)__builtin_amdgcn_readfirstlane((uint32_t)v) | ((unsigned long long)__builtin_amdgcn_readfirstlane((uint32_t)(v >> 32)) << 32);
+}
+
+__device__ __forceinline__ void longContinueRead(const DGraph& g, const uint32_t r, const LongContinue& lc, const gcq::Queue& queue, const LongWorkResult* results, const unsigned long long* tracePool)
+{
+	const uint32_t lane = threadIdx.x;
+	const LongState st = ldh<true>(lc.state + r);
+	if (st.status != 0 || st.candCount == 0) return;
+	bool leave = false;
+	for (uint32_t c = 0; c < 2 * st.candCount; c++) {
+		const uint32_t status = ldh<true>(&results[2 * st.candBegin + c].status);
+		if (status != EXT_OK && status != EXT_FAILED) leave = true;
+	}
+	if (st.nAln + st.candCount > lc.jobs[r].alnCap) leave = true;
+	if (leave) return;
+	longMergeRead<true>(g, r, lane, lc.jobs, lc.seeds, lc.candSeed, results, tracePool, lc.state, lc.alns, lc.cellPool, lc.cellCursor, lc.cellCapacity, lc.extraHeuristic);
+	__threadfence();
+	uint32_t maxCandidates = lc.fixedCandidates;
+	if (!maxCandidates) {
+		unsigned long long waiting = 0;
+		if (lane == 0) waiting = gcq::unclaimed(queue);
+		waiting = longUniform64(waiting);
+		const uint32_t waves = gridDim.x;
+		maxCandidates = waiting >= waves ? 1u : waiting >= waves / 2 ? 2u : waiting >= waves / 4 ? 4u : (uint32_t)LONG_MAX_CANDIDATES;
+	}
+	longSelectRead<true>(g, r, lane, lc.jobs, lc.seeds, lc.minClusterSize, lc.extraHeuristic, maxCandidates, lc.state, lc.alns, lc.cellPool, lc.work, nullptr, lc.candSeed, nullptr, lc.workCapacity, lc.pending, &queue);
+}
+
+template <bool BAND, bool CLIP>
+__global__ void __launch_bounds__(64) __attribute__((amdgpu_waves_per_eu(GC_LONG_WAVES_ONE, 8))) k_long_continue(DGraph g, const CorrectnessTables* __restrict__ ct, const uint64_t* __restrict__ masks, ExtendConfig cfg,
+	const uint32_t* __restrict__ order, unsigned long long* __restrict__ scratch, uint64_t wordsPerLane, unsigned long long* tracePool, unsigned long long* traceCursor, uint64_t traceCapacity,
+	LongWorkResult* results, unsigned long long* __restrict__ counters, uint32_t* __restrict__ capListOut, unsigned long long* __restrict__ capCountOut, LongContinue lc)
+{
+	__shared__ WaveLdsT<1> lds;
+	const bool leader = threadIdx.x == 0;
+	WaveScratch wsx;
+	wsx.base = scratch + (uint64_t)blockIdx.x * wordsPerLane;
+	wsx.lane = 0;
+	wsx.lanes = 1;
+	wsx.maxSlices = cfg.maxSlices; wsx.maxItems = cfg.maxItems; wsx.maxTrace = cfg.maxTrace;
+	wsx.maxCols = cfg.maxCols;
+	wsx.allLanes = true;
+	wsx.regCap = cfg.regCap;
+	ExtCounters cnt {};
+	const gcq::Queue queue { lc.head, lc.tail, lc.ready, lc.timeout, lc.workCapacity, lc.nInitial, gridDim.x < lc.nInitial ? gridDim.x : lc.nInitial, lc.maxSpins };
+	unsigned long long slot = blockIdx.x < queue.firstDynamic ? (unsigned long long)blockIdx.x : gcq::NONE;
+	while (true) {
+		if (slot == gcq::NONE) {
+			unsigned long long claimed = 0;
+			if (leader) claimed = gcq::claim(queue);
+			slot = longUniform64(claimed);
+			if (slot == gcq::NONE) break;
+		}
+		uint32_t ready = 0;
+		if (leader) ready = gcq::waitReady(queue, slot) ? 1u : 0u;
+		if (!__builtin_amdgcn_readfirstlane(ready)) break;
+		gcq::acquireFence();
+		const uint32_t w = slot < lc.nInitial ? order[slot] : (uint32_t)slot;
+		slot = gcq::NONE;
+		LongWork it;
+		{
+			const LongWork loaded = ldh<true>(lc.work + w);
+			it.maskOff = longUniform64(loaded.maskOff);
+			it.maskWords = __builtin_amdgcn_readfirstlane(loaded.maskWords); it.startBit = __builtin_amdgcn_readfirstlane(loaded.startBit);
+			it.seqLen = __builtin_amdgcn_readfirstlane(loaded.seqLen); it.node = __builtin_amdgcn_readfirstlane(loaded.node);
+			it.offset = __builtin_amdgcn_readfirstlane(loaded.offset); it.read = __builtin_amdgcn_readfirstlane(loaded.read);
+		}
+		LongWorkResult res { 0, 0, EXT_FAILED, 0, 0 };
+		if (it.seqLen > 0) {
+			uint32_t nTrace = 0;
+			int32_t score = 0;
+			EqSource eqSrc { masks + it.maskOff, it.maskWords, it.startBit };
+			if (CLIP) res.status = extendSeedWave<true, true, true>(g, *ct, eqSrc, cfg.bandwidth, (lds_u32*)&lds.w[0][0], wsx, (int)it.seqLen, it.node, it.offset, 0, nTrace, score, cnt,
+				cfg.rampBandwidth, cfg.maxCells, cfg.forceGlobal != 0, cfg.clipErrorCost(), cfg.xDrop);
+			else if (BAND) res.status = extendSeedWave<true, true>(g, *ct, eqSrc, cfg.bandwidth, (lds_u32*)&lds.w[0][0], wsx, (int)it.seqLen, it.node, it.offset, 0, nTrace, score, cnt,
+				cfg.rampBandwidth, cfg.maxCells, cfg.forceGlobal != 0);
+			else res.status = extendSeedWave<true>(g, *ct, eqSrc, cfg.bandwidth, (lds_u32*)&lds.w[0][0], wsx, (int)it.seqLen, it.node, it.offset, 0, nTrace, score, cnt);
+			res.score = score;
+			res.pad = cnt.flattenTie;
+			if (res.status == EXT_OK) {
+				unsigned long long base = 0;
+				if (leader) base = atomicAdd(traceCursor, (unsigned long long)nTrace);
+				base = longUniform64(base);
+				if (base + nTrace <= traceCapacity) {
+					for (uint32_t i = threadIdx.x; i < nTrace; i += 64) tracePool[base + i] = wsx.word(wsx.traceBase(i, 0));
+					res.traceOff = base;
+					res.traceLen = nTrace;
+				} else {
+					res.status = EXT_DEFER;
+					if (leader) atomicAdd(lc.deferred, 1ull);
+				}
+			}
+		}
+		if (leader) results[w] = res;
+		if (leader && res.status == EXT_LDS_CAP) capListOut[atomicAdd(capCountOut, 1ull)] = w;
+		gcq::releaseFence();
+		uint32_t last = 0;
+		if (leader) last = gcq::arrive(lc.pending + it.read) ? 1u : 0u;
+		if (__builtin_amdgcn_readfirstlane(last)) {
+			gcq::acquireFence();
+			longContinueRead(g, it.read, lc, queue, results, tracePool);
+		}
+	}
+	if (cnt.extensions && leader) {
+		atomicAdd(&counters[0], cnt.dpTiles);
+		atomicAdd(&counters[1], cnt.recomputeTiles);
+		atomicAdd(&counters[2], cnt.columnSteps);
+		atomicAdd(&counters[3], cnt.traceItems);
+		atomicAdd(&counters[4], cnt.extensions);
+		atomicAdd(&counters[5], cnt.backtraceTiles);
+#ifdef GC_STAMPS
+		for (int i = 0; i < 16; i++) atomicAdd(&counters[8 + i], cnt.cyc[i]);
+#endif
+	}
+}
+
+__global__ void __launch_bounds__(256) k_zero_u32(uint32_t* __restrict__ dst, uint64_t n)
+{
+	GC_RAISE_PRIO();
+	for (uint64_t i = (uint64_t)blockIdx.x * 256 + threadIdx.x; i < n; i += (uint64_t)gridDim.x * 256) dst[i] = 0;
 }
 
 #ifndef GC_ORDER_THREADS
@@ -1275,11 +1467,11 @@
 	if (nReads) hipLaunchKernelGGL(k_long_init, dim3((nReads + 255) / 256), dim3(256), 0, stream, jobs, nReads, state);
 }
 void launchLongSelect(hipStream_t stream, const DGraph& g, const LongJob* jobs, uint32_t nReads, const LongSeed* seeds, uint64_t rcBase, uint32_t minClusterSize, uint32_t extraHeuristic, uint32_t maxCandidates,
-	LongState* state, const LongAln* alns, const LongCell* cellPool, LongWork* work, uint32_t* workLen, uint32_t* candSeed, unsigned long long* workCount, uint64_t workCapacity)
+	LongState* state, const LongAln* alns, const LongCell* cellPool, LongWork* work, uint32_t* workLen, uint32_t* candSeed, unsigned long long* workCount, uint64_t workCapacity, uint32_t* pending)
 {
 	if (maxCandidates < 1) maxCandidates = 1;
 	if (maxCandidates > LONG_MAX_CANDIDATES) maxCandidates = LONG_MAX_CANDIDATES;
-	if (nReads) hipLaunchKernelGGL(k_long_select, dim3(nReads), dim3(64), 0, stream, g, jobs, nReads, seeds, rcBase, minClusterSize, extraHeuristic, maxCandidates, state, alns, cellPool, work, workLen, candSeed, workCount, workCapacity);
+	if (nReads) hipLaunchKernelGGL(k_long_select, dim3(nReads), dim3(64), 0, stream, g, jobs, nReads, seeds, rcBase, minClusterSize, extraHeuristic, maxCandidates, state, alns, cellPool, work, workLen, candSeed, workCount, workCapacity, pending);
 }
 uint32_t longExtendTeamSize(uint32_t nWork, uint32_t teamOverride)
 {
@@ -1351,9 +1543,35 @@
 	if (nFrags) hipLaunchKernelGGL(k_build_fragment_work, dim3((nFrags + 255) / 256), dim3(256), 0, stream, g, frags, fragFirstSeed, nFrags, readSeeds, readOffsets, totalBases, splitLen, fragSeeds, work, results);
 }
 void launchLongMerge(hipStream_t stream, const DGraph& g, const LongJob* jobs, uint32_t nReads, const LongSeed* seeds, const uint32_t* candSeed, const LongWorkResult* results,
-	const unsigned long long* tracePool, LongState* state, LongAln* alns, LongCell* cellPool, unsigned long long* cellCursor, uint64_t cellCapacity, uint32_t extraHeuristic)
-{
-	if (nReads) hipLaunchKernelGGL(k_long_merge, dim3(nReads), dim3(64), 0, stream, g, jobs, nReads, seeds, candSeed, results, tracePool, state, alns, cellPool, cellCursor, cellCapacity, extraHeuristic);
+	const unsigned long long* tracePool, LongState* state, LongAln* alns, LongCell* cellPool, unsigned long long* cellCursor, uint64_t cellCapacity, uint32_t extraHeuristic, bool continued)
+{
+	if (nReads) hipLaunchKernelGGL(k_long_merge, dim3(nReads), dim3(64), 0, stream, g, jobs, nReads, seeds, candSeed, results, tracePool, state, alns, cellPool, cellCursor, cellCapacity, extraHeuristic, continued ? 1u : 0u);
+}
+
+uint32_t longContinueWaves()
+{
+	static const uint32_t waves = []() {
+		int perCu = 0, dev = 0, cus = 256;
+		if (hipOccupancyMaxActiveBlocksPerMultiprocessor(&perCu, k_long_continue<false, false>, 64, 0) != hipSuccess || perCu <= 0) perCu = 4 * GC_LONG_WAVES_ONE;
+		if (perCu > 4 * GC_LONG_WAVES_ONE) perCu = 4 * GC_LONG_WAVES_ONE;
+		hipDeviceProp_t prop;
+		if (hipGetDevice(&dev) == hipSuccess && hipGetDeviceProperties(&prop, dev) == hipSuccess && prop.multiProcessorCount > 0) cus = prop.multiProcessorCount;
+		return (uint32_t)(perCu * cus);
+	}();
+	return waves;
+}
+
+void launchLongContinue(hipStream_t stream, const DGraph& g, const CorrectnessTables* ct, const uint64_t* masks, const ExtendConfig& cfg, const uint32_t* order, unsigned long long* scratch, uint32_t blocks,
+	unsigned long long* tracePool, unsigned long long* traceCursor, uint64_t traceCapacity, LongWorkResult* results, unsigned long long* counters, uint32_t* capListOut, unsigned long long* capCountOut, const LongContinue& lc)
+{
+	if (!lc.nInitial || !blocks) return;
+	const uint64_t words = longWaveWordsPerLane(cfg);
+	if (lc.workCapacity > lc.nInitial) hipLaunchKernelGGL(k_zero_u32, dim3((uint32_t)std::min<uint64_t>(256, (lc.workCapacity - lc.nInitial + 255) / 256)), dim3(256), 0, stream, lc.ready + lc.nInitial, lc.workCapacity - lc.nInitial);
+#define GC_LAUNCH_CONTINUE(B, C) hipLaunchKernelGGL(HIP_KERNEL_NAME(k_long_continue<B, C>), dim3(blocks), dim3(64), 0, stream, g, ct, masks, cfg, order, scratch, words, tracePool, traceCursor, traceCapacity, results, counters, capListOut, capCountOut, lc)
+	if (cfg.clipOn()) GC_LAUNCH_CONTINUE(true, true);
+	else if (cfg.bandControls()) GC_LAUNCH_CONTINUE(true, false);
+	else GC_LAUNCH_CONTINUE(false, false);
+#undef GC_LAUNCH_CONTINUE
 }
 void launchLongOrder(hipStream_t stream, const uint32_t* workLen, const unsigned long long* workCount, uint32_t* order, uint32_t maxLen, uint32_t mode)
 {
diff --git a/graphchainer_amd/csrc/hip/gc_kernels.hpp b/graphchainer_amd/csrc/hip/gc_kernels.hpp
--- a/graphchainer_amd/csrc/hip/gc_kernels.hpp
+++ b/graphchainer_amd/csrc/hip/gc_kernels.hpp
@@ -146,6 +146,20 @@
 	uint32_t read;
 };
 struct LongWorkResult { uint64_t traceOff; uint32_t traceLen, status; int32_t score; uint32_t pad; };
+struct LongContinue {
+	const LongJob* jobs; const LongSeed* seeds; LongState* state; LongAln* alns; LongCell* cellPool; unsigned long long* cellCursor; uint64_t cellCapacity;
+	LongWork* work; uint32_t* candSeed;
+	uint32_t* pending;
+	uint32_t* ready;
+	unsigned long long* tail;
+	unsigned long long* head;
+	unsigned long long* timeout;
+	unsigned long long* deferred;
+	uint64_t workCapacity;
+	uint32_t nInitial, minClusterSize, extraHeuristic;
+	uint32_t fixedCandidates;
+	uint32_t maxSpins;
+};
 
 void launchSeedLookup(hipStream_t stream, const SeedIndex& idx, const char* bases, const uint64_t* readOff, uint32_t nReads,
 	uint64_t* matchCursor, uint32_t* readMatchOff, uint32_t* readMatchCount, uint2* matches, uint64_t matchCapacity, uint32_t* tmp, uint64_t totalBases, const uint32_t* chunkRead, const uint64_t* packed, const uint64_t* invalid);
@@ -220,13 +234,18 @@
 uint64_t longWaveWordsPerLane(const ExtendConfig& cfg);
 void launchLongInit(hipStream_t stream, const LongJob* jobs, uint32_t nReads, LongState* state);
 void launchLongSelect(hipStream_t stream, const DGraph& g, const LongJob* jobs, uint32_t nReads, const LongSeed* seeds, uint64_t rcBase, uint32_t minClusterSize, uint32_t extraHeuristic, uint32_t maxCandidates,
-	LongState* state, const LongAln* alns, const LongCell* cellPool, LongWork* work, uint32_t* workLen, uint32_t* candSeed, unsigned long long* workCount, uint64_t workCapacity);
+	LongState* state, const LongAln* alns, const LongCell* cellPool, LongWork* work, uint32_t* workLen, uint32_t* candSeed, unsigned long long* workCount, uint64_t workCapacity,
+	uint32_t* pending = nullptr);
 uint32_t longExtendTeamSize(uint32_t nWork, uint32_t teamOverride);
 void launchLongExtend(hipStream_t stream, const DGraph& g, const CorrectnessTables* ct, const uint64_t* masks, const ExtendConfig& cfg, const LongWork* work, const uint32_t* order, uint32_t nWork,
 	unsigned long long* scratch, uint32_t lanes, uint32_t blocks, unsigned long long* tracePool, unsigned long long* traceCursor, uint64_t traceCapacity, LongWorkResult* results, unsigned long long* counters,
 	unsigned long long* nextSlot, uint32_t retryStatus = 0, const unsigned long long* nWorkOnDevice = nullptr, uint32_t* capListOut = nullptr, unsigned long long* capCountOut = nullptr);
 void launchLongMerge(hipStream_t stream, const DGraph& g, const LongJob* jobs, uint32_t nReads, const LongSeed* seeds, const uint32_t* candSeed, const LongWorkResult* results,
-	const unsigned long long* tracePool, LongState* state, LongAln* alns, LongCell* cellPool, unsigned long long* cellCursor, uint64_t cellCapacity, uint32_t extraHeuristic);
+	const unsigned long long* tracePool, LongState* state, LongAln* alns, LongCell* cellPool, unsigned long long* cellCursor, uint64_t cellCapacity, uint32_t extraHeuristic,
+	bool continued = false);
+uint32_t longContinueWaves();
+void launchLongContinue(hipStream_t stream, const DGraph& g, const CorrectnessTables* ct, const uint64_t* masks, const ExtendConfig& cfg, const uint32_t* order, unsigned long long* scratch, uint32_t blocks,
+	unsigned long long* tracePool, unsigned long long* traceCursor, uint64_t traceCapacity, LongWorkResult* results, unsigned long long* counters, uint32_t* capListOut, unsigned long long* capCountOut, const LongContinue& lc);
 struct PathSeqJob {
 	uint64_t srcOff;
 	uint64_t outOff;
diff --git a/graphchainer_amd/csrc/hip/gc_long_queue.hpp b/graphchainer_amd/csrc/hip/gc_long_queue.hpp
--- /dev/null
+++ b/graphchainer_amd/csrc/hip/gc_long_queue.hpp
@@ -0,0 +1,103 @@
+#pragma once
+#include <cstdint>
+
+#if defined(__HIPCC__)
+#include <hip/hip_runtime.h>
+#define GCQ_FN __device__ __forceinline__
+namespace gcq {
+typedef unsigned long long Word64;
+typedef uint32_t Word32;
+GCQ_FN unsigned long long load64(const Word64* p) { return __hip_atomic_load(p, __ATOMIC_RELAXED, __HIP_MEMORY_SCOPE_AGENT); }
+GCQ_FN uint32_t load32(const Word32* p) { return __hip_atomic_load(p, __ATOMIC_RELAXED, __HIP_MEMORY_SCOPE_AGENT); }
+GCQ_FN void store32(Word32* p, uint32_t v) { __hip_atomic_store(p, v, __ATOMIC_RELAXED, __HIP_MEMORY_SCOPE_AGENT); }
+GCQ_FN void store64(Word64* p, unsigned long long v) { __hip_atomic_store(p, v, __ATOMIC_RELAXED, __HIP_MEMORY_SCOPE_AGENT); }
+GCQ_FN bool cas64(Word64* p, unsigned long long& expected, unsigned long long desired) { return __hip_atomic_compare_exchange_strong(p, &expected, desired, __ATOMIC_RELAXED, __ATOMIC_RELAXED, __HIP_MEMORY_SCOPE_AGENT); }
+GCQ_FN void releaseFence() { __builtin_amdgcn_fence(__ATOMIC_RELEASE, "agent"); asm volatile("s_waitcnt vmcnt(0)" ::: "memory"); }
+GCQ_FN void acquireFence() { __builtin_amdgcn_fence(__ATOMIC_ACQUIRE, "agent"); }
+GCQ_FN void storeReleaseRun32(Word32* p, uint32_t n, uint32_t v) { releaseFence(); for (uint32_t i = 0; i < n; i++) store32(p + i, v); }
+GCQ_FN uint32_t fetchSubRelease32(Word32* p) { releaseFence(); return __hip_atomic_fetch_sub(p, 1u, __ATOMIC_RELAXED, __HIP_MEMORY_SCOPE_AGENT); }
+GCQ_FN void pause() { __builtin_amdgcn_s_sleep(8); }
+}
+#else
+#include <atomic>
+#include <thread>
+#define GCQ_FN inline
+namespace gcq {
+typedef std::atomic<unsigned long long> Word64;
+typedef std::atomic<uint32_t> Word32;
+GCQ_FN unsigned long long load64(const Word64* p) { return p->load(std::memory_order_acquire); }
+GCQ_FN uint32_t load32(const Word32* p) { return p->load(std::memory_order_acquire); }
+GCQ_FN void store32(Word32* p, uint32_t v) { p->store(v, std::memory_order_release); }
+GCQ_FN void store64(Word64* p, unsigned long long v) { p->store(v, std::memory_order_release); }
+GCQ_FN bool cas64(Word64* p, unsigned long long& expected, unsigned long long desired) { return p->compare_exchange_strong(expected, desired, std::memory_order_acq_rel, std::memory_order_acquire); }
+GCQ_FN void releaseFence() {}
+GCQ_FN void acquireFence() {}
+GCQ_FN void storeReleaseRun32(Word32* p, uint32_t n, uint32_t v) { for (uint32_t i = 0; i < n; i++) p[i].store(v, std::memory_order_release); }
+GCQ_FN uint32_t fetchSubRelease32(Word32* p) { return p->fetch_sub(1u, std::memory_order_acq_rel); }
+GCQ_FN void pause() { std::this_thread::yield(); }
+}
+#endif
+
+namespace gcq {
+
+struct Queue {
+	Word64* head;
+	Word64* tail;
+	Word32* ready;
+	Word64* timeout;
+	uint64_t capacity;
+	uint32_t nInitial;
+	uint32_t firstDynamic;
+	uint32_t maxSpins;
+};
+constexpr uint64_t NONE = ~0ull;
+
+
+GCQ_FN uint64_t claim(const Queue& q)
+{
+	unsigned long long h = load64(q.head);
+	for (;;) {
+		const unsigned long long t = load64(q.tail);
+		if (q.firstDynamic + h >= t) return NONE;
+		if (cas64(q.head, h, h + 1)) return q.firstDynamic + h;
+	}
+}
+
+GCQ_FN uint64_t unclaimed(const Queue& q)
+{
+	const unsigned long long h = q.firstDynamic + load64(q.head), t = load64(q.tail);
+	return t > h ? t - h : 0;
+}
+
+GCQ_FN uint64_t reserve(const Queue& q, uint32_t k)
+{
+	unsigned long long t = load64(q.tail);
+	for (;;) {
+		if (t + k > q.capacity) return NONE;
+		if (cas64(q.tail, t, t + k)) return t;
+	}
+}
+
+GCQ_FN void publish(const Queue& q, uint64_t first, uint32_t k) { storeReleaseRun32(q.ready + first, k, 1u); }
+
+GCQ_FN bool waitReady(const Queue& q, uint64_t slot)
+{
+	if (slot >= q.nInitial) {
+		uint32_t spins = 0;
+		while (load32(q.ready + slot) == 0) {
+			if (++spins > q.maxSpins) { store64(q.timeout, slot + 1); return false; }
+			pause();
+		}
+	}
+	acquireFence();
+	return true;
+}
+
+GCQ_FN bool arrive(Word32* pending)
+{
+	if (fetchSubRelease32(pending) != 1u) return false;
+	acquireFence();
+	return true;
+}
+
+}
diff --git a/graphchainer_amd/csrc/host/gc_switches.hpp b/graphchainer_amd/csrc/host/gc_switches.hpp
--- a/graphchainer_amd/csrc/host/gc_switches.hpp
+++ b/graphchainer_amd/csrc/host/gc_switches.hpp
@@ -19,6 +19,7 @@
 	int syncPollUs = 40;
 	int longToken = 1;
 	std::optional<int> longTokens;
+	bool longContinue = true;
 	bool debugTimes = false;
 	bool debugEd = false;
 	bool deviceGlue = true;
@@ -51,6 +52,7 @@
 	std::optional<uint32_t> testLongTeam;
 	uint32_t testLongOrder = 1;
 	std::optional<uint32_t> testLongSpeculate;
+	std::optional<uint64_t> testLongTracePool;
 	bool testChainForceScratch = false;
 	std::optional<double> testPoolFirstGuess;
 	size_t testPoolShrinkFloor = 64u << 20;
@@ -59,6 +61,8 @@
 
 	bool shareLongScratch() const { return longToken >= 1; }
 	bool onePassAtATime() const { return longToken != 0; }
+
+	static const char* continuationVariable(const char* name) { return getenv(name); }
 
 	static Switches fromEnvironment()
 	{
@@ -72,6 +76,7 @@
 		if (const char* e = getenv("GC_SYNC_POLL_US")) s.syncPollUs = std::max(1, atoi(e));
 		if (const char* e = getenv("GC_LONG_TOKEN")) s.longToken = atoi(e);
 		if (const char* e = getenv("GC_LONG_TOKENS")) s.longTokens = std::max(1, std::min(LONG_TOKENS_MAX, atoi(e)));
+		if (const char* e = continuationVariable("GC_LONG_CONTINUE")) s.longContinue = !(atoi(e) == 0);
 		s.debugTimes = getenv("GC_DEBUG_TIMES") != nullptr;
 		s.debugEd = getenv("GC_DEBUG_ED") != nullptr;
 
@@ -106,6 +111,7 @@
 		if (const char* e = getenv("GC_TEST_LONG_TEAM")) { int v = atoi(e); if (v == 1 || v == 2 || v == 4 || v == 8 || v == 16 || v == 32 || v == 64) s.testLongTeam = (uint32_t)v; }
 		if (const char* e = getenv("GC_TEST_LONG_ORDER")) s.testLongOrder = (uint32_t)atoi(e);
 		if (const char* e = getenv("GC_TEST_LONG_SPECULATE")) s.testLongSpeculate = (uint32_t)std::min(2, std::max(1, atoi(e)));
+		if (const char* e = continuationVariable("GC_TEST_LONG_TRACE_POOL")) s.testLongTracePool = (uint64_t)std::max(1ll, atoll(e));
 		s.testChainForceScratch = getenv("GC_TEST_CHAIN_FORCE_SCRATCH") != nullptr;
 		if (const char* e = getenv("GC_TEST_POOL_FIRST_GUESS")) s.testPoolFirstGuess = std::max(0.0, atof(e));
 		if (const char* e = getenv("GC_TEST_POOL_SHRINK_FLOOR")) s.testPoolShrinkFloor = (size_t)std::max(0ll, atoll(e));
```
